# ugadiarov-la-phystech-edu/OCRL

Measured on AMD Instinct MI355X. Metric: images/sec (node) SLATE pretrain 128x128, 6 slots, 3 iters, higher is better.
Workload: dtype f32

## Files before the change

include/ocrl_hip.h:

```cpp
#ifndef OCRL_HIP_H
#define OCRL_HIP_H
#include <stddef.h>

#ifdef __cplusplus
extern "C" {
#endif

#define OCRL_ABI_VERSION 5

const char* ocrl_last_error(void);
int ocrl_abi_version(void);

typedef struct ocrl_slate ocrl_slate;
typedef struct ocrl_slate_config {
    int obs_size, obs_channels;
    int vocab_size, d_model;
    int cnn_hidden;
    int num_slots, num_iterations, slot_size, mlp_hidden;
    int num_dec_blocks, num_dec_heads;
    float dropout;
    int max_batch;
    int use_bcdec;
    int hard;
    int num_slot_heads;
// ... 2 lines not shown
size_t ocrl_slate_config_size(void);
int ocrl_slate_create(const ocrl_slate_config* cfg, ocrl_slate** out);
void ocrl_slate_destroy(ocrl_slate* h);

int ocrl_slate_param_count(const ocrl_slate* h);
int ocrl_slate_param_info(const ocrl_slate* h, int i, char* name, int name_cap, int shape[4], int* ndim,
                          long long* offset, long long* numel, int* group);
long long ocrl_slate_flat_size(const ocrl_slate* h);
long long ocrl_slate_group_begin(const ocrl_slate* h, int group);
size_t ocrl_slate_workspace_bytes(const ocrl_slate* h);

int ocrl_slate_bind(ocrl_slate* h, float* params, float* grads, float* adam_m, float* adam_v, void* workspace, size_t workspace_bytes);

int ocrl_slate_forward(ocrl_slate* h, const float* obs, int B, float tau, int train, unsigned long long seed,
                       const float* noise_z, const float* noise_zh, const float* noise_slots, void* stream);
int ocrl_slate_backward(ocrl_slate* h, void* stream);
int ocrl_slate_encode(ocrl_slate* h, const float* obs, int B, unsigned long long seed, const float* noise_slots, void* stream);
int ocrl_slate_encode_backward(ocrl_slate* h, const float* dslots, void* stream);
int ocrl_slate_freeze_weights(ocrl_slate* h, int on);
int ocrl_slate_generate(ocrl_slate* h, void* stream);
int ocrl_slate_clip_adam(ocrl_slate* h, const float lr[3], float clip, int step, float grad_scale, void* stream);
int ocrl_slate_grad_norm(ocrl_slate* h, void* stream);
float* ocrl_slate_metrics(const ocrl_slate* h);
int ocrl_slate_tensor(const ocrl_slate* h, const char* name, float** ptr, long long* count);
int ocrl_slate_soft_z(ocrl_slate* h, void* stream);
int ocrl_slate_dropout_mask(const ocrl_slate* h, unsigned site, long long n, float* out, void* stream);

int ocrl_gemm(const float* A, const float* B, float* C, int M, int N, int K, int lda, int ldb, int ldc, int akc, int bkc,
              float alpha, const float* bias, int relu, const float* mask, int ldmask, const float* resid, int ldr,
              int splitk, float* ws, void* stream);
typedef struct ocrl_gemm_desc {
    const float* A; const float* B; float* C;
    int M, N, K, lda, ldb, ldc;
    int akc, bkc;
    int batch, batch_inner;
    long long sA, sB, sC, sAi, sBi, sCi;
    int splitk; float alpha;
    const float* bias; int relu;
    float drop_p; unsigned long long drop_seed; unsigned drop_site;
    const float* mask; int ldmask; long long sMask; int mask_elu;
    const float* resid; int ldr; long long sR;
    float adrop_p; unsigned adrop_site; int adrop_ld;
    float* bias_out; long long sBias;
    int a_mode, b_mode; const float* x_lse; const int* x_tok; float x_scale;
    int epi_mode; float* stat; float* hstat; int* hidx; const float* e1; const float* e2; unsigned long long e_seed;
    const float* e_lse; const float* e_rowvec; float e_scale;
    int force_tile, force_sb;
} ocrl_gemm_desc;
size_t ocrl_gemm_desc_size(void);
int ocrl_gemm_ex(const ocrl_gemm_desc* d, float* ws, size_t ws_floats, void* stream);
int ocrl_gemm_plan(const ocrl_gemm_desc* d, int out[6]);
int ocrl_conv2d_fwd(const float* x, const float* w, const float* bias, float* y, int B, int H, int W, int cin, int cin_pad, int ks,
                    int relu, float* ws, void* stream);
int ocrl_conv2d_fwd_lowlat(const float* x, const float* w, const float* bias, float* y, int B, int H, int W, int cin, int cin_pad, int ks,
                           int relu, float* ws, void* stream);
size_t ocrl_conv2d_x3_ws_floats(void);
int ocrl_conv2d_fwd_x3(const float* x, const float* w, const float* bias, float* y, int B, int H, int W, int ks, int relu, float* ws, void* stream);
int ocrl_conv2d_bwd_data_x3(const float* dy, const float* w, const float* mask, float* dx, int B, int H, int W, int ks, float* ws, void* stream);
int ocrl_conv2d_bwd_weight_x3(const float* x, const float* dy, float* dw, int B, int H, int W, int ks, float* ws, size_t ws_floats, void* stream);
int ocrl_conv2d_bwd_data(const float* dy, const float* w, const float* mask, float* dx, int B, int H, int W, int ks, float* ws, void* stream);
size_t ocrl_conv2d_wgrad_ws_floats(int B, int H, int W, int ks, int cin_pad);
int ocrl_conv2d_bwd_weight(const float* x, const float* dy, float* dw, float* db, int B, int H, int W, int cin, int cin_pad, int ks,
                           float* ws, size_t ws_floats, void* stream);
typedef struct ocrl_conv_desc {
    const float* x; const float* w; float* y;
    int B, H, W, cin, cin_pad, ks;
    const float* bias; int relu;
    const float* posmap; const float* mask; int mask_elu;
    int transposed, low_latency;
} ocrl_conv_desc;
size_t ocrl_conv_desc_size(void);
int ocrl_conv2d_ex(const ocrl_conv_desc* d, float* ws, size_t ws_floats, void* stream);
typedef struct ocrl_conv_wgrad_desc {
    const float* x; const float* dy; float* dw; float* db;
    int B, H, W, cin, cin_pad, ks;
    int accumulate;
} ocrl_conv_wgrad_desc;
size_t ocrl_conv_wgrad_desc_size(void);
int ocrl_conv2d_bwd_weight_ex(const ocrl_conv_wgrad_desc* d, float* ws, size_t ws_floats, void* stream);
int ocrl_layernorm_fwd(const float* x, const float* gamma, const float* beta, float* y, float* mean, float* rstd, long long R, int F, void* stream);
int ocrl_layernorm_bwd(const float* dy, const float* x, const float* mean, const float* rstd, const float* gamma, float* dx, float* dgb,
                       long long R, int F, float* ws, size_t ws_floats, void* stream);

int ocrl_attention_fwd(const float* q, const float* k, const float* v, float* o, float* lse, int B, int T, int d, int h, int ld,
                       float p, unsigned long long seed, unsigned site, void* stream);
int ocrl_attention_bwd(const float* q, const float* k, const float* v, const float* o, const float* lse, const float* dO,
                       float* dq, float* dk, float* dv, float* delta, int B, int T, int d, int h, int ld,
                       float p, unsigned long long seed, unsigned site, void* stream);

int ocrl_obs_u8_to_f32(const unsigned char* obs_hwc, float* obs_chw, int B, int H, int W, int C, void* stream);

int ocrl_prof_enable(unsigned tag_mask);
int ocrl_prof_collect(double* ms, long long* count, int ntags);

size_t ocrl_slot_attention_ws_floats(int B, int K, int D, int H, int I);
int ocrl_slot_attention_fwd(const float* x, const float* slots0, const float* const* w, float* slots, float* attn, int B, int N, int K, int D,
                            int H, int I, float* ws, size_t ws_floats, void* stream);
int ocrl_slot_attention_bwd(const float* x, const float* dslots, float* dx, float* dslots0, float* const* dw, int B, int N, int K, int D, int H,
                            int I, float* ws, size_t ws_floats, void* stream);
size_t ocrl_slot_attention_mh_ws_floats(int B, int N, int K, int D, int H, int I, int heads);
int ocrl_slot_attention_mh_fwd(const float* x, const float* slots0, const float* const* w, float* slots, float* attn, int B, int N, int K, int D,
                               int H, int I, int heads, float* ws, size_t ws_floats, void* stream);
int ocrl_slot_attention_mh_bwd(const float* x, const float* dslots, float* dx, float* dslots0, float* const* dw, int B, int N, int K, int D, int H,
                               int I, int heads, float* ws, size_t ws_floats, void* stream);

#define OCRL_POOL_MAX_LAYERS 8
size_t ocrl_pool_transformer_ws_floats(int B, int K, int d, int nhead, int ff, int L);
int ocrl_pool_transformer_fwd(const float* slots, const float* const* w, const float* pos, float* out, int B, int K, int Din, int d, int nhead,
                              int ff, int L, float drop_p, unsigned long long seed, float* ws, size_t ws_floats, void* stream);
int ocrl_pool_transformer_bwd(const float* slots, const float* dout, const float* const* w, float* dslots, float* const* dw, int B, int K, int Din,
                              int d, int nhead, int ff, int L, float drop_p, unsigned long long seed, float* ws, size_t ws_floats, void* stream);
int ocrl_pool_transformer_dropout_mask(int layer, int which, long long n, float drop_p, unsigned long long seed, float* out, void* stream);
size_t ocrl_pool_transformer_long_ws_floats(int B, int K, int Din, int d, int nhead, int ff, int L);
int ocrl_pool_transformer_long_fwd(const float* slots, const float* const* w, const float* pos, float* out, int B, int K, int Din, int d, int nhead,
                                   int ff, int L, float drop_p, unsigned long long seed, float* ws, size_t ws_floats, void* stream);
int ocrl_pool_transformer_long_bwd(const float* slots, const float* dout, const float* const* w, float* dslots, float* const* dw, int B, int K,
                                   int Din, int d, int nhead, int ff, int L, float drop_p, unsigned long long seed, float* ws, size_t ws_floats,
                                   void* stream);

#define OCRL_POOL_RN_MAX_LAYERS 16
size_t ocrl_pool_rn_ws_floats(int B, int K, int D, int ng, const int* g_dims, int nf, const int* f_dims);
int ocrl_pool_rn_fwd(const float* slots, const float* const* w, float* out, int B, int K, int D, int ng, const int* g_dims, int nf, const int* f_dims,
                     float* ws, size_t ws_floats, void* stream);
int ocrl_pool_rn_bwd(const float* slots, const float* dout, const float* const* w, float* dslots, float* const* dw, int B, int K, int D, int ng,
                     const int* g_dims, int nf, const int* f_dims, float* ws, size_t ws_floats, void* stream);

#define OCRL_NATURECNN_MAX_GROUPS 16
#define OCRL_NATURECNN_MAX_CONVS 4
size_t ocrl_naturecnn_ws_floats(int B, int H, int W, int cin, int groups, int cnn_feat_size, int use_cnn_feat, int rep_dim);
int ocrl_naturecnn_fwd(const float* obs, const float* const* w, float* out, int B, int H, int W, int cin, int groups, int cnn_feat_size,
                       int use_cnn_feat, int rep_dim, int save, float* ws, size_t ws_floats, void* stream);
int ocrl_naturecnn_bwd(const float* obs, const float* dout, const float* const* w, float* const* dw, int B, int H, int W, int cin, int groups,
                       int cnn_feat_size, int use_cnn_feat, int rep_dim, float* ws, size_t ws_floats, void* stream);

size_t ocrl_pool_cnn_ws_floats(int B, int H, int W, int D, int rep_dim);
int ocrl_pool_cnn_fwd(const float* tokens, const float* const* w, float* out, int B, int H, int W, int D, int rep_dim, int save, float* ws,
                      size_t ws_floats, void* stream);
int ocrl_pool_cnn_bwd(const float* tokens, const float* dout, const float* const* w, float* dtokens, float* const* dw, int B, int H, int W, int D,
                      int rep_dim, float* ws, size_t ws_floats, void* stream);

#define OCRL_VAE_MAX_STAGES 6
size_t ocrl_vae_ws_floats(int B, int obs_size, int obs_channels, int cnn_feat_size, int latent_dim, int use_cnn_feat, int full);
int ocrl_vae_fwd(const float* obs, const float* const* w, const float* eps, float* rep, float* metrics, float* recon, int B, int obs_size,
                 int obs_channels, int cnn_feat_size, int latent_dim, int use_cnn_feat, float kld_weight, int full, float* ws, size_t ws_floats,
                 void* stream);
int ocrl_vae_bwd(const float* obs, const float* eps, const float* const* w, const float* dloss, const float* drep, float* const* dw, int B,
                 int obs_size, int obs_channels, int cnn_feat_size, int latent_dim, int use_cnn_feat, float kld_weight, int full, float* ws,
                 size_t ws_floats, void* stream);

#define OCRL_MAE_MAX_DEPTH 32
size_t ocrl_mae_ws_floats(int B, int obs_size, int patch, int D, int depth, int heads, int Dd, int ddepth, int dheads, int len_keep, int full);
int ocrl_mae_fwd(const float* obs, const float* const* w, const float* noise, float* rep, float* metrics, float* pred, float* mask,
                 int* ids_restore, int B, int obs_size, int patch, int D, int depth, int heads, int Dd, int ddepth, int dheads, int len_keep,
                 int full, float* ws, size_t ws_floats, void* stream);
int ocrl_mae_bwd(const float* obs, const float* const* w, const float* dloss, const float* drep, float* const* dw, int B, int obs_size,
                 int patch, int D, int depth, int heads, int Dd, int ddepth, int dheads, int len_keep, int full, float* ws, size_t ws_floats,
                 void* stream);
int ocrl_mae_rank(const float* noise, int* ids_restore, int* ids_keep, float* mask, int B, int L, int len_keep, void* stream);

#define OCRL_PROBE_MAX_SLOTS 12
#define OCRL_PROBE_MAX_PROPS 8
#define OCRL_PROBE_MAX_LAYERS 8
size_t ocrl_probe_ws_floats(int B, int K, int N, int D, int O, int slot_rows, int nl, const int* dims, int P);
int ocrl_probe_fwd(const float* rows, const float* const* w, const float* y, float* out, float* cost, int* col, float* metrics, int B, int K, int N,
                   int D, int T, int O, int slot_rows, int nl, const int* dims, float slope, int P, const int* tgt_range, const int* out_range,
                   const int* kind, float* ws, size_t ws_floats, void* stream);
// ... 74 lines not shown
```

ocrl_amd/csrc/capi.cpp:

```cpp
#include <stdarg.h>
#include <stdint.h>
#include <string.h>

#include <new>

#include "../../include/ocrl_hip.h"
#include "iodine_model.h"
#include "slate_model.h"

static thread_local char g_err[512] = "";

void ocrl_set_error(const char* fmt, ...) {
    va_list ap;
    va_start(ap, fmt);
    vsnprintf(g_err, sizeof g_err, fmt, ap);
    va_end(ap);
}

template <class M>
struct Handle {
    using Model = M;
    M* m = nullptr;
};
struct ocrl_slate : Handle<SlateModel> {};
// ... 183 lines not shown
}
size_t ocrl_conv2d_x3_ws_floats(void) { return 2 * conv_x3_pack_floats(5); }
int ocrl_conv2d_fwd_x3(const float* x, const float* w, const float* bias, float* y, int B, int H, int W, int ks, int relu, float* ws, void* stream) {
    if (ks != 3 && ks != 5) { ocrl_set_error("ocrl_conv2d_fwd_x3: ks must be 3 or 5"); return 1; }
    if (conv_pack_x3_launch(w, ws, nullptr, ST(stream), ks)) return 1;
    ConvArgs a;
    a.X = x; a.Y = y; a.B = B; a.H = H; a.W = W; a.bias = bias; a.relu = relu;
    return conv_x3_launch(a, ws, ST(stream), ks);
}
int ocrl_conv2d_bwd_data_x3(const float* dy, const float* w, const float* mask, float* dx, int B, int H, int W, int ks, float* ws, void* stream) {
    if (ks != 3 && ks != 5) { ocrl_set_error("ocrl_conv2d_bwd_data_x3: ks must be 3 or 5"); return 1; }
    if (conv_pack_x3_launch(w, ws, ws + conv_x3_pack_floats(5), ST(stream), ks)) return 1;
    ConvArgs a;
    a.X = dy; a.Y = dx; a.B = B; a.H = H; a.W = W; a.mask = mask;
    return conv_x3_launch(a, ws + conv_x3_pack_floats(5), ST(stream), ks);
}
int ocrl_conv2d_bwd_data(const float* dy, const float* w, const float* mask, float* dx, int B, int H, int W, int ks, float* ws, void* stream) {
    float* bw = ws + (size_t)ks * ks * 64 * 64;
    if (conv_pack_launch(w, ws, bw, ks, 64, 64, 64, ST(stream))) return 1;
    ConvArgs a;
    a.X = dy; a.Wp = bw; a.Y = dx; a.B = B; a.H = H; a.W = W; a.mask = mask;
    return conv_fwd_launch(a, ks, 64, 64, ST(stream));
}
size_t ocrl_conv2d_wgrad_ws_floats(int B, int H, int W, int ks, int cin_pad) { return conv_wgrad_ws_floats(B, H, W, ks, cin_pad) + (1 << 16); }
int ocrl_conv2d_bwd_weight(const float* x, const float* dy, float* dw, float* db, int B, int H, int W, int cin, int cin_pad, int ks, float* ws,
                           size_t ws_floats, void* stream) {
    if (ws_floats < ocrl_conv2d_wgrad_ws_floats(B, H, W, ks, cin_pad)) { ocrl_set_error("ocrl_conv2d_bwd_weight: workspace too small"); return 1; }
    WgradArgs a;
    a.X = x; a.dY = dy; a.part = ws; a.B = B; a.H = H; a.W = W;
    if (conv_wgrad_launch(a, ks, cin_pad, 64, cin, dw, 0, ST(stream), 0)) return 1;
    if (db) return colsum_launch(dy, 64, db, (long long)B * H * W, 64, 0, 1.f, ws, ws_floats, ST(stream));
    return 0;
}
int ocrl_conv2d_bwd_weight_x3(const float* x, const float* dy, float* dw, int B, int H, int W, int ks, float* ws, size_t ws_floats, void* stream) {
    if (ks != 3 && ks != 5) { ocrl_set_error("ocrl_conv2d_bwd_weight_x3: ks must be 3 or 5"); return 1; }
    if (ws_floats < ocrl_conv2d_wgrad_ws_floats(B, H, W, ks, 64)) { ocrl_set_error("ocrl_conv2d_bwd_weight_x3: workspace too small"); return 1; }
    WgradArgs a;
    a.X = x; a.dY = dy; a.part = ws; a.B = B; a.H = H; a.W = W;
    return conv_wgrad_launch(a, ks, 64, 64, 64, dw, 0, ST(stream), 1);
}
static bool conv_kernel_built(int ks, int cin_pad) { return (ks == 5 && (cin_pad == 64 || cin_pad == 8)) || (ks == 3 && cin_pad == 64); }
static bool aligned16(const void* p) { return ((uintptr_t)p & 15) == 0; }
size_t ocrl_conv_desc_size(void) { return sizeof(ocrl_conv_desc); }
int ocrl_conv2d_ex(const ocrl_conv_desc* d, float* ws, size_t ws_floats, void* stream) {
    if (!d) { ocrl_set_error("ocrl_conv2d_ex: null descriptor"); return 1; }
    if (!d->x || !d->w || !d->y || !ws || d->B < 1 || d->H < 1 || d->W < 1) { ocrl_set_error("ocrl_conv2d_ex: x, w, y, ws and a non-empty image are required"); return 1; }
    if (!conv_kernel_built(d->ks, d->cin_pad)) { ocrl_set_error("ocrl_conv2d_ex: no kernel for ks=%d cin_pad=%d (built: 5/64, 5/8, 3/64)", d->ks, d->cin_pad); return 1; }
    if (d->cin < 1 || d->cin > d->cin_pad) { ocrl_set_error("ocrl_conv2d_ex: cin %d outside 1 .. cin_pad %d", d->cin, d->cin_pad); return 1; }
    if (d->relu < 0 || d->relu > 2) { ocrl_set_error("ocrl_conv2d_ex: relu must be 0, 1 (ReLU) or 2 (ELU), got %d", d->relu); return 1; }
    if (d->mask_elu && !d->mask) { ocrl_set_error("ocrl_conv2d_ex: mask_elu needs a mask"); return 1; }
    if (d->transposed && (d->cin != 64 || d->cin_pad != 64)) { ocrl_set_error("ocrl_conv2d_ex: the transposed (backward-data) form needs cin = cin_pad = 64"); return 1; }
    if (!aligned16(d->x) || !aligned16(d->y) || !aligned16(ws) || !aligned16(d->bias) || !aligned16(d->posmap) || !aligned16(d->mask)) {
        ocrl_set_error("ocrl_conv2d_ex: x, y, ws, bias, posmap and mask must be 16-byte aligned");
        return 1;
    }
    const size_t pack = (size_t)d->ks * d->ks * d->cin_pad * 64, need = d->transposed ? 2 * pack : pack;
    if (ws_floats < need) { ocrl_set_error("ocrl_conv2d_ex: workspace of %zu floats, %zu needed", ws_floats, need); return 1; }
    float* bw = d->transposed ? ws + pack : nullptr;
    if (conv_pack_launch(d->w, ws, bw, d->ks, d->cin_pad, 64, d->cin, ST(stream))) return 1;
    ConvArgs a;
    a.X = d->x; a.Wp = bw ? bw : ws; a.Y = d->y; a.B = d->B; a.H = d->H; a.W = d->W; a.bias = d->bias; a.relu = d->relu;
    a.posmap = d->posmap; a.mask = d->mask; a.mask_elu = d->mask_elu ? 1 : 0;
    return conv_fwd_launch(a, d->ks, d->cin_pad, 64, ST(stream), d->low_latency ? 1 : 0);
}
size_t ocrl_conv_wgrad_desc_size(void) { return sizeof(ocrl_conv_wgrad_desc); }
int ocrl_conv2d_bwd_weight_ex(const ocrl_conv_wgrad_desc* d, float* ws, size_t ws_floats, void* stream) {
    if (!d) { ocrl_set_error("ocrl_conv2d_bwd_weight_ex: null descriptor"); return 1; }
    if (!d->x || !d->dy || !d->dw || !ws || d->B < 1 || d->H < 1 || d->W < 1) { ocrl_set_error("ocrl_conv2d_bwd_weight_ex: x, dy, dw, ws and a non-empty image are required"); return 1; }
    if (!conv_kernel_built(d->ks, d->cin_pad)) { ocrl_set_error("ocrl_conv2d_bwd_weight_ex: no kernel for ks=%d cin_pad=%d (built: 5/64, 5/8, 3/64)", d->ks, d->cin_pad); return 1; }
    if (d->cin < 1 || d->cin > d->cin_pad) { ocrl_set_error("ocrl_conv2d_bwd_weight_ex: cin %d outside 1 .. cin_pad %d", d->cin, d->cin_pad); return 1; }
    if (!aligned16(d->x) || !aligned16(d->dy) || !aligned16(ws)) { ocrl_set_error("ocrl_conv2d_bwd_weight_ex: x, dy and ws must be 16-byte aligned"); return 1; }
    const size_t need = ocrl_conv2d_wgrad_ws_floats(d->B, d->H, d->W, d->ks, d->cin_pad);
    if (ws_floats < need) { ocrl_set_error("ocrl_conv2d_bwd_weight_ex: workspace of %zu floats, %zu needed", ws_floats, need); return 1; }
    const int acc = d->accumulate ? 1 : 0;
    WgradArgs a;
    a.X = d->x; a.dY = d->dy; a.part = ws; a.B = d->B; a.H = d->H; a.W = d->W;
    if (conv_wgrad_launch(a, d->ks, d->cin_pad, 64, d->cin, d->dw, acc, ST(stream), 0)) return 1;
    if (d->db) return colsum_launch(d->dy, 64, d->db, (long long)d->B * d->H * d->W, 64, acc, 1.f, ws, ws_floats, ST(stream));
    return 0;
}
int ocrl_layernorm_fwd(const float* x, const float* g, const float* b, float* y, float* mean, float* rstd, long long R, int F, void* stream) {
    return layernorm_fwd_launch(x, g, b, y, mean, rstd, R, F, ST(stream));
}
int ocrl_layernorm_bwd(const float* dy, const float* x, const float* mean, const float* rstd, const float* g, float* dx, float* dgb, long long R,
                       int F, float* ws, size_t ws_floats, void* stream) {
    return layernorm_bwd_launch(dy, x, mean, rstd, g, dx, dgb, R, F, 0, 0, ws, ws_floats, ST(stream));
}

int ocrl_attention_fwd(const float* q, const float* k, const float* v, float* o, float* lse, int B, int T, int d, int h, int ld, float p,
                       unsigned long long seed, unsigned site, void* stream) {
    AttnArgs a;
    a.q = q; a.k = k; a.v = v; a.o = o; a.lse = lse; a.B = B; a.T = T; a.d = d; a.h = h; a.ld = ld; a.p = p; a.seed = seed; a.site = site;
    return attn_launch(a, 0, ST(stream));
}
int ocrl_attention_bwd(const float* q, const float* k, const float* v, const float* o, const float* lse, const float* dO, float* dq,
                       float* dk, float* dv, float* delta, int B, int T, int d, int h, int ld, float p, unsigned long long seed,
                       unsigned site, void* stream) {
    AttnArgs a;
    a.q = q; a.k = k; a.v = v; a.o = const_cast<float*>(o); a.lse = const_cast<float*>(lse); a.B = B; a.T = T; a.d = d; a.h = h; a.ld = ld;
    a.p = p; a.seed = seed; a.site = site; a.dO = dO; a.dq = dq; a.dk = dk; a.dv = dv; a.delta = delta;
    return attn_launch(a, 1, ST(stream));
}


int ocrl_iodine_create(const ocrl_iodine_config* c, ocrl_iodine** out) {
    if (!c || !out) { ocrl_set_error("ocrl_iodine_create: null argument"); return 1; }
    if (c->obs_size < 16 || c->obs_size % 16 || c->obs_channels != 3 || c->slot_size < 4 || c->slot_size % 4 || c->slot_size > 256 ||
        c->num_iterations < 1 || c->num_slots < 1 || c->num_slots > 16 || c->ref_mlp_hidden < 64 || c->ref_mlp_hidden % 64 || c->max_batch < 1 ||
        !(c->sigma > 0.f)) {
        ocrl_set_error("ocrl_iodine_create: invalid configuration");
        return 1;
    }
    IodineConfig k;
    k.obs_size = c->obs_size; k.obs_channels = c->obs_channels; k.slot_size = c->slot_size; k.num_iters = c->num_iterations;
    k.num_slots = c->num_slots; k.sigma = c->sigma; k.beta = c->beta; k.layer_norm = c->layer_norm; k.ref_mlp_hidden = c->ref_mlp_hidden;
    k.max_batch = c->max_batch;
    return h_create(k, out);
}
void ocrl_iodine_destroy(ocrl_iodine* h) { h_destroy(h); }
int ocrl_iodine_param_count(const ocrl_iodine* h) { return h_param_count(h); }
int ocrl_iodine_param_info(const ocrl_iodine* h, int i, char* name, int name_cap, int shape[4], int* ndim, long long* offset, long long* numel) {
    return h_param_info(h, i, name, name_cap, shape, ndim, offset, numel, nullptr);
}
long long ocrl_iodine_flat_size(const ocrl_iodine* h) { return h_flat_size(h); }
size_t ocrl_iodine_workspace_bytes(const ocrl_iodine* h) { return h_workspace_bytes(h); }
int ocrl_iodine_bind(ocrl_iodine* h, float* p, float* g, float* m, float* v, void* ws, size_t n) { return h_bind(h, p, g, m, v, ws, n); }
int ocrl_iodine_forward(ocrl_iodine* h, const float* obs, int B, unsigned long long seed, const float* noise, void* stream) {
    GUARD(h);
    return h->m->forward(obs, B, seed, noise, ST(stream));
}
int ocrl_iodine_backward(ocrl_iodine* h, void* stream) { GUARD(h); return h->m->backward(ST(stream)); }
int ocrl_iodine_clip_adam(ocrl_iodine* h, float lr, float clip, int step, float gscale, void* stream) {
    GUARD(h);
    return h->m->clip_adam(lr, clip, step, gscale, ST(stream));
}
int ocrl_iodine_grad_norm(ocrl_iodine* h, void* stream) { GUARD(h); return h->m->grad_norm(ST(stream)); }
float* ocrl_iodine_metrics(const ocrl_iodine* h) { return h_metrics(h); }
int ocrl_iodine_tensor(const ocrl_iodine* h, const char* name, float** ptr, long long* count) { return h_tensor(h, name, ptr, count); }
}
```

ocrl_amd/csrc/elementwise.hip:

```cpp
#include "common.h"
#include "kernels.h"

#define TINYF 1.17549435e-38f

__device__ inline float block_sum(float v, float* red) {
    v = wave_sum(v);
    const int w = threadIdx.x >> 6, nw = blockDim.x >> 6;
    __syncthreads();
    if ((threadIdx.x & 63) == 0) red[w] = v;
    __syncthreads();
    float s = 0.f;
    for (int i = 0; i < nw; ++i) s += red[i];
    return s;
}
__device__ inline float block_max(float v, float* red) {
    v = wave_max(v);
    const int w = threadIdx.x >> 6, nw = blockDim.x >> 6;
    __syncthreads();
    if ((threadIdx.x & 63) == 0) red[w] = v;
    __syncthreads();
    float s = red[0];
    for (int i = 1; i < nw; ++i) s = fmaxf(s, red[i]);
    return s;
}

__global__ void nchw_to_nhwc8_kernel(const float* __restrict__ in, float* __restrict__ out, int B, int C, int H, int W) {
    const long long n = (long long)B * H * W;
    const long long i = (long long)blockIdx.x * blockDim.x + threadIdx.x;
    if (i >= n) return;
    const long long hw = (long long)H * W;
    const long long b = i / hw, r = i % hw;
    float v[8];
#pragma unroll
    for (int c = 0; c < 8; ++c) v[c] = c < C ? in[(b * C + c) * hw + r] : 0.f;
    float4* o = reinterpret_cast<float4*>(out + i * 8);
    o[0] = make_float4(v[0], v[1], v[2], v[3]);
    o[1] = make_float4(v[4], v[5], v[6], v[7]);
}

__global__ void patchify4_kernel(const float* __restrict__ in, float* __restrict__ out, int B, int C, int S) {
    const int E = S / 4;
    const long long n = (long long)B * E * E * C * 4;
    const long long i = (long long)blockIdx.x * blockDim.x + threadIdx.x;
    if (i >= n) return;
    const int ky = i & 3;
    const int c = (i >> 2) % C;
    const long long row = (i >> 2) / C;
    const int ex = row % E, ey = (row / E) % E;
    const long long b = row / ((long long)E * E);
    const float4 v = *reinterpret_cast<const float4*>(in + ((b * C + c) * S + (ey * 4 + ky)) * S + ex * 4);
    *reinterpret_cast<float4*>(out + row * (C * 16) + c * 16 + ky * 4) = v;
}

__global__ void pixel_shuffle_kernel(const float* __restrict__ in, float* __restrict__ out, int B, int h, int w, int Cout, int forward,
                                     const float* __restrict__ mask) {
    const long long n = (long long)B * h * w * Cout;
    const long long i = (long long)blockIdx.x * blockDim.x + threadIdx.x;
    if (i >= n) return;
    const int c = i % Cout;
    long long r = i / Cout;
    const int x = r % w; r /= w;
    const int y = r % h;
    const long long b = r / h;
    const long long u = i * 4;
    const long long s00 = ((b * 2 * h + 2 * y) * (2 * w) + 2 * x) * Cout + c;
    const long long s01 = s00 + Cout, s10 = s00 + (long long)2 * w * Cout, s11 = s10 + Cout;
    if (forward) {
        const float4 v = *reinterpret_cast<const float4*>(in + u);
        out[s00] = v.x; out[s01] = v.y; out[s10] = v.z; out[s11] = v.w;
    } else {
        float4 v = make_float4(in[s00], in[s01], in[s10], in[s11]);
        if (mask) {
            const float4 m = *reinterpret_cast<const float4*>(mask + u);
            v.x = m.x > 0.f ? v.x : 0.f; v.y = m.y > 0.f ? v.y : 0.f; v.z = m.z > 0.f ? v.z : 0.f; v.w = m.w > 0.f ? v.w : 0.f;
        }
        *reinterpret_cast<float4*>(out + u) = v;
    }
}

template <int NPL>
__global__ void layernorm_fwd_kernel(const float* __restrict__ x, const float* __restrict__ g, const float* __restrict__ bta,
                                     float* __restrict__ y, float* __restrict__ mean, float* __restrict__ rstd, long long R) {
    constexpr int F = 64 * NPL;
    const int lane = threadIdx.x & 63;
// ... 166 lines not shown
        const float mu = group16_sum(s) * (1.0f / 192);
        float q = 0.f;
#pragma unroll
        for (int k = 0; k < 3; ++k) {
            v[i][k].x -= mu; v[i][k].y -= mu; v[i][k].z -= mu; v[i][k].w -= mu;
            q += (v[i][k].x * v[i][k].x + v[i][k].y * v[i][k].y) + (v[i][k].z * v[i][k].z + v[i][k].w * v[i][k].w);
        }
        const float rs = rsqrtf(group16_sum(q) * (1.0f / 192) + 1e-5f);
        if (row < R) {
#pragma unroll
            for (int k = 0; k < 3; ++k)
                *reinterpret_cast<float4*>(y + row * 192 + (k * 16 + c4) * 4) = make_float4(v[i][k].x * rs * gg[k].x + bb[k].x, v[i][k].y * rs * gg[k].y + bb[k].y,
                                                                                            v[i][k].z * rs * gg[k].z + bb[k].z, v[i][k].w * rs * gg[k].w + bb[k].w);
            if (c4 == 0) { if (mean) mean[row] = mu; if (rstd) rstd[row] = rs; }
        }
    }
}
__global__ __launch_bounds__(256) void layernorm_bwd192_kernel(const float* __restrict__ dy, const float* __restrict__ x, const float* __restrict__ mean,
                                                               const float* __restrict__ rstd, const float* __restrict__ g, float* __restrict__ dx,
                                                               float* __restrict__ part, long long R, int accumulate) {
    __shared__ float4 red[2][16][48];
    const int lane = threadIdx.x & 63, wv = threadIdx.x >> 6, c4 = lane & 15, rsub = lane >> 4;
    float4 gg[3], dg[3], db[3];
#pragma unroll
    for (int k = 0; k < 3; ++k) { gg[k] = *reinterpret_cast<const float4*>(g + (k * 16 + c4) * 4); dg[k] = make_float4(0.f, 0.f, 0.f, 0.f); db[k] = dg[k]; }
    for (long long grp = blockIdx.x; grp * 32 < R; grp += gridDim.x) {
        const long long row0 = (grp * 4 + wv) * 8 + rsub;
        float4 xv[2][3], yv[2][3];
        float mu[2], rs[2];
#pragma unroll
        for (int i = 0; i < 2; ++i) {
            const long long row = row0 + 4 * i;
            const bool ok = row < R;
#pragma unroll
            for (int k = 0; k < 3; ++k) {
                xv[i][k] = ok ? *reinterpret_cast<const float4*>(x + row * 192 + (k * 16 + c4) * 4) : make_float4(0.f, 0.f, 0.f, 0.f);
                yv[i][k] = ok ? *reinterpret_cast<const float4*>(dy + row * 192 + (k * 16 + c4) * 4) : make_float4(0.f, 0.f, 0.f, 0.f);
            }
            mu[i] = ok ? mean[row] : 0.f;
            rs[i] = ok ? rstd[row] : 0.f;
        }
#pragma unroll
        for (int i = 0; i < 2; ++i) {
            const long long row = row0 + 4 * i;
            float4 xh[3], d4[3];
            float s1 = 0.f, s2 = 0.f;
#pragma unroll
            for (int k = 0; k < 3; ++k) {
                xh[k] = make_float4((xv[i][k].x - mu[i]) * rs[i], (xv[i][k].y - mu[i]) * rs[i], (xv[i][k].z - mu[i]) * rs[i], (xv[i][k].w - mu[i]) * rs[i]);
                const float4 yy = yv[i][k];
                dg[k].x += yy.x * xh[k].x; dg[k].y += yy.y * xh[k].y; dg[k].z += yy.z * xh[k].z; dg[k].w += yy.w * xh[k].w;
                db[k].x += yy.x; db[k].y += yy.y; db[k].z += yy.z; db[k].w += yy.w;
                d4[k] = make_float4(yy.x * gg[k].x, yy.y * gg[k].y, yy.z * gg[k].z, yy.w * gg[k].w);
                s1 += (d4[k].x + d4[k].y) + (d4[k].z + d4[k].w);
                s2 += (d4[k].x * xh[k].x + d4[k].y * xh[k].y) + (d4[k].z * xh[k].z + d4[k].w * xh[k].w);
            }
            s1 = group16_sum(s1) * (1.0f / 192);
            s2 = group16_sum(s2) * (1.0f / 192);
            if (row < R) {
#pragma unroll
                for (int k = 0; k < 3; ++k) {
                    float4 o = make_float4(rs[i] * (d4[k].x - s1 - xh[k].x * s2), rs[i] * (d4[k].y - s1 - xh[k].y * s2), rs[i] * (d4[k].z - s1 - xh[k].z * s2),
                                           rs[i] * (d4[k].w - s1 - xh[k].w * s2));
                    float* dp = dx + row * 192 + (k * 16 + c4) * 4;
                    if (accumulate) { const float4 a = *reinterpret_cast<const float4*>(dp); o.x += a.x; o.y += a.y; o.z += a.z; o.w += a.w; }
                    *reinterpret_cast<float4*>(dp) = o;
                }
            }
        }
    }
#pragma unroll
    for (int k = 0; k < 3; ++k) { red[0][wv * 4 + rsub][k * 16 + c4] = dg[k]; red[1][wv * 4 + rsub][k * 16 + c4] = db[k]; }
    __syncthreads();
    if (threadIdx.x < 96) {
        const int which = threadIdx.x / 48, c = threadIdx.x % 48;
        float4 a = red[which][0][c];
#pragma unroll
        for (int k = 1; k < 16; ++k) { const float4 t = red[which][k][c]; a.x += t.x; a.y += t.y; a.z += t.z; a.w += t.w; }
        *reinterpret_cast<float4*>(part + (size_t)blockIdx.x * 384 + which * 192 + c * 4) = a;
    }
}

__global__ void colsum_kernel(const float* __restrict__ X, long long ld, float* __restrict__ part, long long R, int F, long long rows_per_chunk) {
    __shared__ float red[4][64];
    const int col = blockIdx.x * 64 + (threadIdx.x & 63), rl = threadIdx.x >> 6;
    const long long r0 = (long long)blockIdx.y * rows_per_chunk;
    const long long r1 = min(R, r0 + rows_per_chunk);
    float s = 0.f;
    if (col < F)
        for (long long r = r0 + rl; r < r1; r += 4) s += X[r * ld + col];
    red[rl][threadIdx.x & 63] = s;
    __syncthreads();
    if (rl == 0 && col < F) part[(size_t)blockIdx.y * F + col] = red[0][threadIdx.x] + red[1][threadIdx.x] + red[2][threadIdx.x] + red[3][threadIdx.x];
}
__global__ __launch_bounds__(256) void colsum4_kernel(const float* __restrict__ X, long long ld, float* __restrict__ part, long long R, int F,
                                                      long long rows_per_chunk) {
    __shared__ float4 red[256];
    const int F4 = F >> 2, RL = 256 / F4;
    const int c4 = threadIdx.x % F4, rl = threadIdx.x / F4;
    const long long r0 = (long long)blockIdx.x * rows_per_chunk;
    const long long r1 = min(R, r0 + rows_per_chunk);
    float4 s0 = make_float4(0.f, 0.f, 0.f, 0.f), s1 = s0, s2 = s0, s3 = s0;
    if (rl < RL) {
        const float* base = X + (size_t)c4 * 4;
        long long r = r0 + rl;
        for (; r + 3 * RL < r1; r += 4 * RL) {
            const float4 a = *reinterpret_cast<const float4*>(base + r * ld), b = *reinterpret_cast<const float4*>(base + (r + RL) * ld);
            const float4 c = *reinterpret_cast<const float4*>(base + (r + 2 * RL) * ld), d = *reinterpret_cast<const float4*>(base + (r + 3 * RL) * ld);
            s0.x += a.x; s0.y += a.y; s0.z += a.z; s0.w += a.w;
            s1.x += b.x; s1.y += b.y; s1.z += b.z; s1.w += b.w;
            s2.x += c.x; s2.y += c.y; s2.z += c.z; s2.w += c.w;
            s3.x += d.x; s3.y += d.y; s3.z += d.z; s3.w += d.w;
        }
        for (; r < r1; r += RL) {
            const float4 a = *reinterpret_cast<const float4*>(base + r * ld);
            s0.x += a.x; s0.y += a.y; s0.z += a.z; s0.w += a.w;
        }
    }
    red[threadIdx.x] = make_float4(s0.x + s1.x + s2.x + s3.x, s0.y + s1.y + s2.y + s3.y, s0.z + s1.z + s2.z + s3.z, s0.w + s1.w + s2.w + s3.w);
    __syncthreads();
    if (threadIdx.x < F4) {
        float4 t = red[threadIdx.x];
        for (int k = 1; k < RL; ++k) { const float4 v = red[k * F4 + threadIdx.x]; t.x += v.x; t.y += v.y; t.z += v.z; t.w += v.w; }
        *reinterpret_cast<float4*>(part + (size_t)blockIdx.x * F + threadIdx.x * 4) = t;
    }
}
__global__ __launch_bounds__(256) void colsum_final_kernel(const float* __restrict__ part, float* __restrict__ out, int nchunk, int F, int accumulate, float scale) {
    __shared__ float red[16][16];
    const int cl = threadIdx.x & 15, rl = threadIdx.x >> 4;
    const int c = blockIdx.x * 16 + cl;
    float s0 = 0.f, s1 = 0.f;
    if (c < F) {
        int k = rl;
        for (; k + 16 < nchunk; k += 32) { s0 += part[(size_t)k * F + c]; s1 += part[(size_t)(k + 16) * F + c]; }
        if (k < nchunk) s0 += part[(size_t)k * F + c];
    }
    red[rl][cl] = s0 + s1;
    __syncthreads();
    if (rl == 0 && c < F) {
        float t = 0.f;
#pragma unroll
        for (int k = 0; k < 16; ++k) t += red[k][cl];
        t *= scale;
        out[c] = accumulate ? out[c] + t : t;
    }
}

__global__ void reduce_partials_kernel(const float* __restrict__ part, int n, float* __restrict__ out, float scale, int accumulate) {
    __shared__ float red[4];
    float s = 0.f;
    for (int i = threadIdx.x; i < n; i += blockDim.x) s += part[i];
    s = block_sum(s, red);
    if (threadIdx.x == 0) out[0] = (accumulate ? out[0] : 0.f) + s * scale;
}

__global__ void mse_kernel(const float* __restrict__ obs, const float* __restrict__ recon, float* __restrict__ drecon,
                           float* __restrict__ part, int B, int C, int H, int W, float inv_b) {
    __shared__ float red[4];
    const long long n = (long long)B * H * W, hw = (long long)H * W;
    float s = 0.f;
    for (long long i = (long long)blockIdx.x * blockDim.x + threadIdx.x; i < n; i += (long long)gridDim.x * blockDim.x) {
        const long long b = i / hw, r = i % hw;
        const float4 rc = *reinterpret_cast<const float4*>(recon + i * 4);
        const float rv[4] = {rc.x, rc.y, rc.z, rc.w};
        float d[4] = {0.f, 0.f, 0.f, 0.f};
        for (int c = 0; c < C; ++c) {
            const float e = rv[c] - obs[(b * C + c) * hw + r];
            s += e * e;
            d[c] = 2.f * e * inv_b;
        }
        if (drecon) *reinterpret_cast<float4*>(drecon + i * 4) = make_float4(d[0], d[1], d[2], d[3]);
    }
    s = block_sum(s, red);
    if (threadIdx.x == 0) part[blockIdx.x] = s;
}

#define GS_MAXPT 16
template <int NPT>
__global__ __launch_bounds__(256) void gumbel_softmax_kernel(const float* __restrict__ raw, const float* __restrict__ e1,
                                                             const float* __restrict__ e2, float* __restrict__ z,
                                                             int* __restrict__ tokens, int V, float inv_tau,
                                                             unsigned long long seed, float* __restrict__ zst) {
    __shared__ float red[4];
    __shared__ float redv[4];
    __shared__ int redi[4];
    const long long row = blockIdx.x;
    const float* r = raw + row * V;
    const int npt = NPT ? NPT : V / 256;
    float x[GS_MAXPT];
    float mx = -INFINITY;
#pragma unroll
    for (int i = 0; i < GS_MAXPT; ++i)
        if (i < npt) { x[i] = r[i * 256 + threadIdx.x]; mx = fmaxf(mx, x[i]); }
    mx = block_max(mx, red);
    float s = 0.f;
#pragma unroll
    for (int i = 0; i < GS_MAXPT; ++i)
        if (i < npt) s += __expf(x[i] - mx);
    s = block_sum(s, red);
    const float lse = mx + __logf(s);
    float u[GS_MAXPT];
    float best = -INFINITY;
    int besti = 0;
    float m2 = -INFINITY;
#pragma unroll
    for (int i = 0; i < GS_MAXPT; ++i)
        if (i < npt) {
            const int v = i * 256 + threadIdx.x;
            const float lp = x[i] - lse;
            float ea, eb;
            if (e1) { ea = e1[row * V + v]; eb = e2[row * V + v]; }
            else {
                const uint64_t idx = (uint64_t)row * V + v;
                const uint2 ba = rng_bits4(seed, SITE_GUMBEL_Z, idx);
                ea = -__logf(u01_24(ba.x));
                eb = -__logf(u01_24(ba.y));
            }
            const float g1 = -__logf(ea + TINYF), g2 = -__logf(eb + TINYF);
            u[i] = (lp + g1) * inv_tau;
            m2 = fmaxf(m2, u[i]);
            const float h = (lp + g2) * inv_tau;
            if (h > best) { best = h; besti = v; }
        }
    m2 = block_max(m2, red);
    float s2 = 0.f;
#pragma unroll
    for (int i = 0; i < GS_MAXPT; ++i)
        if (i < npt) { u[i] = __expf(u[i] - m2); s2 += u[i]; }
// ... 805 lines not shown
    float mx = -INFINITY;
    for (int j = tid; j < nk; j += 256) {
        const float* kr = base + (size_t)j * ld + d;
        float a = 0.f;
        for (int c = 0; c < dh; c += 4) {
            const float4 kv = *reinterpret_cast<const float4*>(kr + c);
            a += qs[c] * kv.x + qs[c + 1] * kv.y + qs[c + 2] * kv.z + qs[c + 3] * kv.w;
        }
        sc[j] = a;
        mx = fmaxf(mx, a);
    }
    red[tid] = mx;
    __syncthreads();
    for (int o = 128; o > 0; o >>= 1) { if (tid < o) red[tid] = fmaxf(red[tid], red[tid + o]); __syncthreads(); }
    mx = red[0];
    __syncthreads();
    float sum = 0.f;
    for (int j = tid; j < nk; j += 256) { const float e = __expf(sc[j] - mx); sc[j] = e; sum += e; }
    red[tid] = sum;
    __syncthreads();
    for (int o = 128; o > 0; o >>= 1) { if (tid < o) red[tid] += red[tid + o]; __syncthreads(); }
    const float inv = 1.0f / red[0];
    __syncthreads();
    const int nsl = 256 / dh, c = tid % dh, sl = tid / dh;
    float acc = 0.f;
    if (sl < nsl)
        for (int j = sl; j < nk; j += nsl) acc += sc[j] * base[(size_t)j * ld + 2 * d + c];
    red[tid] = sl < nsl ? acc : 0.f;
    __syncthreads();
    if (tid < dh) {
        float a = 0.f;
        for (int k = 0; k < nsl; ++k) a += red[k * dh + tid];
        out[(size_t)b * d + hd * dh + tid] = a * inv;
    }
}

__global__ void onehot_kernel(const int* __restrict__ tokens, float* __restrict__ z, long long n, int V) {
    const long long i = (long long)blockIdx.x * blockDim.x + threadIdx.x;
    if (i >= n) return;
    z[i] = (int)(i % V) == tokens[i / V] ? 1.f : 0.f;
}

#define GRID1D(n) dim3(cdiv((n), 256)), dim3(256)

int nchw_to_nhwc8_launch(const float* in, float* out, int B, int C, int H, int W, hipStream_t st) {
    OCRL_REQUIRE(C <= 8, "nchw_to_nhwc8: C must be <= 8");
    const long long n = (long long)B * H * W;
    hipLaunchKernelGGL(nchw_to_nhwc8_kernel, GRID1D(n), 0, st, in, out, B, C, H, W);
    OCRL_CHECK_LAUNCH("nchw_to_nhwc8");
    return 0;
}
int patchify4_launch(const float* in, float* out, int B, int C, int S, hipStream_t st) {
    OCRL_REQUIRE(S % 4 == 0, "patchify4: S %% 4 != 0");
    const long long n = (long long)B * (S / 4) * (S / 4) * C * 4;
    hipLaunchKernelGGL(patchify4_kernel, GRID1D(n), 0, st, in, out, B, C, S);
    OCRL_CHECK_LAUNCH("patchify4");
    return 0;
}
int pixel_shuffle_launch(const float* in, float* out, int B, int h, int w, int Cout, int forward, const float* mask, hipStream_t st) {
    const long long n = (long long)B * h * w * Cout;
    hipLaunchKernelGGL(pixel_shuffle_kernel, GRID1D(n), 0, st, in, out, B, h, w, Cout, forward, mask);
    OCRL_CHECK_LAUNCH("pixel_shuffle");
    return 0;
}
int layernorm_fwd_launch(const float* x, const float* g, const float* b, float* y, float* mean, float* rstd, long long R, int F, hipStream_t st) {
    OCRL_REQUIRE(F % 64 == 0 && F >= 64 && F <= 256, "layernorm: F must be 64..256, multiple of 64 (got %d)", F);
    dim3 grid(cdiv(R, 4)), blk(256);
    const bool al16 = (((uintptr_t)x | (uintptr_t)y | (uintptr_t)g | (uintptr_t)b) & 15) == 0;
    switch (F / 64) {
        case 1:
            if (al16) hipLaunchKernelGGL(layernorm_fwd64_kernel, dim3((unsigned)cdiv(R, 64)), blk, 0, st, x, g, b, y, mean, rstd, R);
            else hipLaunchKernelGGL(layernorm_fwd_kernel<1>, grid, blk, 0, st, x, g, b, y, mean, rstd, R);
            break;
        case 2: hipLaunchKernelGGL(layernorm_fwd_kernel<2>, grid, blk, 0, st, x, g, b, y, mean, rstd, R); break;
        case 3:
            if (al16) hipLaunchKernelGGL(layernorm_fwd192_kernel, dim3((unsigned)cdiv(R, 32)), blk, 0, st, x, g, b, y, mean, rstd, R);
            else hipLaunchKernelGGL(layernorm_fwd_kernel<3>, grid, blk, 0, st, x, g, b, y, mean, rstd, R);
            break;
        default: hipLaunchKernelGGL(layernorm_fwd_kernel<4>, grid, blk, 0, st, x, g, b, y, mean, rstd, R); break;
    }
    OCRL_CHECK_LAUNCH("layernorm_fwd");
    return 0;
}
int colsum_launch(const float* X, long long ld, float* out, long long R, int F, int accumulate, float scale, float* ws, size_t ws_floats, hipStream_t st) {
    if (F % 4 == 0 && ld % 4 == 0 && F <= 1024 && F >= 4 && (((uintptr_t)X) & 15) == 0 && R >= 1024) {
        long long nchunk = 2048;
        if (nchunk > R / 8) nchunk = R / 8;
        if ((size_t)nchunk * F > ws_floats) nchunk = (long long)(ws_floats / F);
        if (nchunk >= 16) {
            const long long rpc = (R + nchunk - 1) / nchunk;
            nchunk = (R + rpc - 1) / rpc;
            hipLaunchKernelGGL(colsum4_kernel, dim3((unsigned)nchunk), dim3(256), 0, st, X, ld, ws, R, F, rpc);
            OCRL_CHECK_LAUNCH("colsum4");
            hipLaunchKernelGGL(colsum_final_kernel, dim3(cdiv(F, 16)), dim3(256), 0, st, ws, out, (int)nchunk, F, accumulate, scale);
            OCRL_CHECK_LAUNCH("colsum_final");
            return 0;
        }
    }
    const int cb = cdiv(F, 64);
    long long nchunk = 1024 / cb;
    if (nchunk < 1) nchunk = 1;
    if (nchunk > (R + 63) / 64) nchunk = (R + 63) / 64;
    if (nchunk < 1) nchunk = 1;
    OCRL_REQUIRE((size_t)nchunk * F <= ws_floats, "colsum: workspace too small (%lld x %d)", nchunk, F);
    const long long rpc = (R + nchunk - 1) / nchunk;
    hipLaunchKernelGGL(colsum_kernel, dim3(cb, (int)nchunk), dim3(256), 0, st, X, ld, ws, R, F, rpc);
    OCRL_CHECK_LAUNCH("colsum");
    hipLaunchKernelGGL(colsum_final_kernel, dim3(cdiv(F, 16)), dim3(256), 0, st, ws, out, (int)nchunk, F, accumulate, scale);
    OCRL_CHECK_LAUNCH("colsum_final");
    return 0;
}
int layernorm_bwd_launch(const float* dy, const float* x, const float* mean, const float* rstd, const float* g, float* dx,
                         float* dgb, long long R, int F, int accumulate_dx, int accumulate_dgb, float* ws, size_t ws_floats, hipStream_t st) {
    OCRL_REQUIRE(F % 64 == 0 && F >= 64 && F <= 256, "layernorm bwd: F must be 64..256, multiple of 64 (got %d)", F);
    int nblk = (int)((R + 3) / 4);
    if (nblk > 2048) nblk = 2048;
    while (nblk > 64 && (size_t)nblk * 2 * F * 2 + (size_t)8 * 2 * F > ws_floats) nblk /= 2;
    const size_t need = (size_t)nblk * 2 * F;
    OCRL_REQUIRE(need + (size_t)8 * 2 * F <= ws_floats, "layernorm bwd: workspace too small");
    dim3 grid(nblk), blk(256);
    switch (F / 64) {
        case 1:
            if (((((uintptr_t)x | (uintptr_t)dy | (uintptr_t)dx | (uintptr_t)g) & 15) == 0) && (((uintptr_t)ws) & 15) == 0)
                hipLaunchKernelGGL(layernorm_bwd64_kernel, grid, blk, 0, st, dy, x, mean, rstd, g, dx, ws, R, accumulate_dx);
            else hipLaunchKernelGGL(layernorm_bwd_kernel<1>, grid, blk, 0, st, dy, x, mean, rstd, g, dx, ws, R, accumulate_dx);
            break;
        case 2: hipLaunchKernelGGL(layernorm_bwd_kernel<2>, grid, blk, 0, st, dy, x, mean, rstd, g, dx, ws, R, accumulate_dx); break;
        case 3:
            if (((((uintptr_t)x | (uintptr_t)dy | (uintptr_t)dx | (uintptr_t)g) & 15) == 0) && (((uintptr_t)ws) & 15) == 0)
                hipLaunchKernelGGL(layernorm_bwd192_kernel, grid, blk, 0, st, dy, x, mean, rstd, g, dx, ws, R, accumulate_dx);
            else hipLaunchKernelGGL(layernorm_bwd_kernel<3>, grid, blk, 0, st, dy, x, mean, rstd, g, dx, ws, R, accumulate_dx);
            break;
        default: hipLaunchKernelGGL(layernorm_bwd_kernel<4>, grid, blk, 0, st, dy, x, mean, rstd, g, dx, ws, R, accumulate_dx); break;
    }
    OCRL_CHECK_LAUNCH("layernorm_bwd");
    return colsum_launch(ws, 2 * F, dgb, nblk, 2 * F, accumulate_dgb, 1.f, ws + need, ws_floats - need, st);
}
int reduce_partials_launch(const float* part, int n, float* out, float scale, int accumulate, hipStream_t st) {
    hipLaunchKernelGGL(reduce_partials_kernel, dim3(1), dim3(256), 0, st, part, n, out, scale, accumulate);
    OCRL_CHECK_LAUNCH("reduce_partials");
    return 0;
}
int mse_launch(const float* obs, const float* recon, float* drecon, float* out, int B, int C, int H, int W, float* ws, size_t ws_floats, hipStream_t st) {
    OCRL_REQUIRE(C <= 4, "mse: C must be <= 4");
    const int nblk = 1024;
    OCRL_REQUIRE(ws_floats >= (size_t)nblk, "mse: workspace too small");
    hipLaunchKernelGGL(mse_kernel, dim3(nblk), dim3(256), 0, st, obs, recon, drecon, ws, B, C, H, W, 1.0f / B);
    OCRL_CHECK_LAUNCH("mse");
    return reduce_partials_launch(ws, nblk, out, 1.0f / B, 0, st);
}
int gumbel_softmax_launch(const float* raw, const float* e1, const float* e2, float* z, int* tokens, long long R, int V, float tau,
                          unsigned long long seed, hipStream_t st, float* zst) {
    OCRL_REQUIRE(V % 256 == 0 && V <= 256 * GS_MAXPT, "gumbel_softmax: V must be a multiple of 256, <= %d", 256 * GS_MAXPT);
    OCRL_REQUIRE((e1 == nullptr) == (e2 == nullptr), "gumbel_softmax: give both noise tensors or none");
    switch (V / 256) {
        case 16: hipLaunchKernelGGL(gumbel_softmax_kernel<16>, dim3((unsigned)R), dim3(256), 0, st, raw, e1, e2, z, tokens, V, 1.0f / tau, seed, zst); break;
        case 8: hipLaunchKernelGGL(gumbel_softmax_kernel<8>, dim3((unsigned)R), dim3(256), 0, st, raw, e1, e2, z, tokens, V, 1.0f / tau, seed, zst); break;
        default: hipLaunchKernelGGL(gumbel_softmax_kernel<0>, dim3((unsigned)R), dim3(256), 0, st, raw, e1, e2, z, tokens, V, 1.0f / tau, seed, zst); break;
    }
    OCRL_CHECK_LAUNCH("gumbel_softmax");
    return 0;
}
int softmax_bwd_rows_launch(const float* z, float* d, long long R, int V, float scale, hipStream_t st) {
    OCRL_REQUIRE(V % 256 == 0 && V <= 256 * GS_MAXPT, "softmax_bwd_rows: V must be a multiple of 256, <= %d", 256 * GS_MAXPT);
    if (V == 4096) hipLaunchKernelGGL(softmax_bwd_rows_kernel<16>, dim3((unsigned)R), dim3(256), 0, st, z, d, V, scale);
    else hipLaunchKernelGGL(softmax_bwd_rows_kernel<0>, dim3((unsigned)R), dim3(256), 0, st, z, d, V, scale);
    OCRL_CHECK_LAUNCH("softmax_bwd_rows");
    return 0;
}
int ce_launch(float* pred, const int* tokens, float* out, long long R, int V, int B, int write_grad, float* ws, size_t ws_floats, hipStream_t st) {
    OCRL_REQUIRE(ws_floats >= (size_t)R, "ce: workspace too small");
    OCRL_REQUIRE(V % 256 == 0 && V <= 256 * GS_MAXPT, "ce: V must be a multiple of 256, <= %d", 256 * GS_MAXPT);
    if (V == 4096) hipLaunchKernelGGL(ce_kernel<16>, dim3((unsigned)R), dim3(256), 0, st, pred, tokens, ws, V, 1.0f / B, write_grad);
    else hipLaunchKernelGGL(ce_kernel<0>, dim3((unsigned)R), dim3(256), 0, st, pred, tokens, ws, V, 1.0f / B, write_grad);
    OCRL_CHECK_LAUNCH("ce");
    return reduce_partials_launch(ws, (int)R, out, 1.0f / B, 0, st);
}
int softmax_stat_combine_launch(const float* stat, int nseg, long long R, float* lse, const float* hstat, const int* hidx, int* tokens,
                                const float* pred, int ldp, const int* tok, float* out, float scale, float* ws, size_t ws_floats, hipStream_t st,
                                const float* cdf_scores, int cdf_V, float cdf_tau, unsigned long long cdf_seed) {
    OCRL_REQUIRE(nseg >= 1 && nseg <= 64, "softmax_stat_combine: 1..64 segments (got %d)", nseg);
    const long long nblk = (R + 15) / 16;
    OCRL_REQUIRE(!pred || (tok && out && ws && ws_floats >= (size_t)nblk), "softmax_stat_combine: cross-entropy needs tokens, an output and %lld workspace floats", nblk);
    CdfArgs cdf;
    cdf.scores = cdf_scores; cdf.V = cdf_V; cdf.tau = cdf_tau; cdf.seed = cdf_seed;
    OCRL_REQUIRE(!cdf_scores || (hstat && hidx && tokens && cdf_V > 0 && cdf_V <= nseg * 64), "softmax_stat_combine: inverse-CDF sampling arguments");
    hipLaunchKernelGGL(softmax_stat_combine_kernel, dim3((unsigned)nblk), dim3(1024), 0, st, stat, nseg, R, lse, hstat, hidx, tokens, pred, ldp, tok,
                       pred ? ws : nullptr, cdf);
    OCRL_CHECK_LAUNCH("softmax_stat_combine");
    if (pred) return reduce_partials_launch(ws, (int)nblk, out, scale, 0, st);
    return 0;
}
int exp_rows_launch(const float* y, const float* lse, float* z, long long R, int V, hipStream_t st) {
    OCRL_REQUIRE(V % 4 == 0, "exp_rows: V %% 4 != 0");
    const long long n4 = R * (V / 4);
    hipLaunchKernelGGL(exp_rows_kernel, dim3((unsigned)((n4 + 255) / 256)), dim3(256), 0, st, y, lse, z, n4, V / 4);
    OCRL_CHECK_LAUNCH("exp_rows");
    return 0;
}
int rowdot_bias64_launch(const float* g, const float* act, const float* bias, long long R, float* out, hipStream_t st) {
    OCRL_REQUIRE(((((uintptr_t)g) | ((uintptr_t)act) | ((uintptr_t)bias)) & 15) == 0, "rowdot: operands must be 16-byte aligned");
    hipLaunchKernelGGL(rowdot_bias64_kernel, dim3((unsigned)((R + 15) / 16)), dim3(256), 0, st, g, act, bias, R, out);
    OCRL_CHECK_LAUNCH("rowdot_bias64");
    return 0;
}
int embed_fwd_launch(const int* tokens, const float* dict, const float* bos, const float* pe, float* out, int B, int T, int d, float p,
                     unsigned long long seed, hipStream_t st) {
    OCRL_REQUIRE(d % 4 == 0, "embed: d %% 4 != 0");
    const long long n = (long long)B * T * (d / 4);
    hipLaunchKernelGGL(embed_fwd_kernel, dim3((unsigned)cdiv(n, 1024)), dim3(256), 0, st, tokens, dict, bos, pe, out, B, T, d, p, seed);
    OCRL_CHECK_LAUNCH("embed_fwd");
    return 0;
}
static size_t eb_align(size_t n) { return (n + 63) & ~(size_t)63; }
size_t embed_bwd_ws_floats(long long BT, int V, int d) {
    const size_t nchunk = (size_t)cdiv(BT, EB_CHUNK), nunit = (size_t)cdiv(BT, EB_UNIT);
    return eb_align(nchunk * (V + 1)) + 2 * eb_align((size_t)V + 2) + eb_align((size_t)BT) + eb_align(nunit * 2 * d);
}
// ... 188 lines not shown
```

ocrl_amd/csrc/gemm.hip:

```cpp
#include "common.h"
#include "kernels.h"
#include <stdlib.h>

int gemm_launch_tt(const GemmArgs& a, const GemmPlan& p, hipStream_t st);
int gemm_launch_tn(const GemmArgs& a, const GemmPlan& p, hipStream_t st);
int gemm_launch_nn(const GemmArgs& a, const GemmPlan& p, hipStream_t st);

__global__ __launch_bounds__(256) void splitk_reduce_kernel(const float* __restrict__ part, float* __restrict__ out, long long n4,
                                                            int splits, long long stride, int accumulate) {
    __shared__ float4 red[16][16];
    const int cl = threadIdx.x & 15, sl = threadIdx.x >> 4;
    const long long i = (long long)blockIdx.x * 16 + cl;
    float4 s = make_float4(0.f, 0.f, 0.f, 0.f);
    if (i < n4) {
        int k = sl;
        for (; k + 48 < splits; k += 64) {
            const float4 v0 = *reinterpret_cast<const float4*>(part + (size_t)k * stride + i * 4);
            const float4 v1 = *reinterpret_cast<const float4*>(part + (size_t)(k + 16) * stride + i * 4);
            const float4 v2 = *reinterpret_cast<const float4*>(part + (size_t)(k + 32) * stride + i * 4);
            const float4 v3 = *reinterpret_cast<const float4*>(part + (size_t)(k + 48) * stride + i * 4);
            s.x += (v0.x + v1.x) + (v2.x + v3.x); s.y += (v0.y + v1.y) + (v2.y + v3.y);
            s.z += (v0.z + v1.z) + (v2.z + v3.z); s.w += (v0.w + v1.w) + (v2.w + v3.w);
        }
        for (; k < splits; k += 16) {
            const float4 v = *reinterpret_cast<const float4*>(part + (size_t)k * stride + i * 4);
            s.x += v.x; s.y += v.y; s.z += v.z; s.w += v.w;
        }
    }
    red[sl][cl] = s;
    __syncthreads();
    if (sl == 0 && i < n4) {
        float4 t = accumulate ? *reinterpret_cast<const float4*>(out + i * 4) : make_float4(0.f, 0.f, 0.f, 0.f);
#pragma unroll
        for (int k = 0; k < 16; ++k) { t.x += red[k][cl].x; t.y += red[k][cl].y; t.z += red[k][cl].z; t.w += red[k][cl].w; }
        *reinterpret_cast<float4*>(out + i * 4) = t;
    }
}

static int env_tile() {
    static int v = -1;
    if (v < 0) {
        const char* e = getenv("OCRL_GEMM_TILE");
        v = 0;
        if (e) { int bm = 0, bn = 0; if (sscanf(e, "%dx%d", &bm, &bn) == 2) v = bm * 1000 + bn; }
    }
    return v;
}
static int env_sb() {
    static int v = -1;
    if (v < 0) { const char* e = getenv("OCRL_GEMM_SB"); v = e ? atoi(e) : 0; }
    return v;
}
static bool tile_built(int tile, int akc, int bkc) {
    return tile == 128128 || tile == 128064 || tile == 64128 || tile == 64064 || (tile == 128192 && (akc || !bkc));
}

int gemm_plan(const GemmArgs& a, GemmPlan* plan) {
    OCRL_REQUIRE(a.M > 0 && a.N > 0 && a.K > 0, "gemm: empty problem %d %d %d", a.M, a.N, a.K);
    OCRL_REQUIRE(a.batch >= 1 && a.splitk >= 1, "gemm: bad batch/splitk");
    if (a.akc) OCRL_REQUIRE(a.K % 4 == 0 && a.lda % 4 == 0, "gemm: A k-contiguous needs K,lda %% 4 == 0 (K=%d lda=%d)", a.K, a.lda);
    else OCRL_REQUIRE(a.M % 4 == 0 && a.lda % 4 == 0, "gemm: A m-contiguous needs M,lda %% 4 == 0 (M=%d lda=%d)", a.M, a.lda);
    if (a.bkc) OCRL_REQUIRE(a.K % 4 == 0 && a.ldb % 4 == 0, "gemm: B k-contiguous needs K,ldb %% 4 == 0 (K=%d ldb=%d)", a.K, a.ldb);
    else OCRL_REQUIRE(a.N % 4 == 0 && a.ldb % 4 == 0, "gemm: B n-contiguous needs N,ldb %% 4 == 0 (N=%d ldb=%d)", a.N, a.ldb);
    OCRL_REQUIRE(((uintptr_t)a.A & 15) == 0 && ((uintptr_t)a.B & 15) == 0, "gemm: operands must be 16-byte aligned");
    OCRL_REQUIRE((a.sA % 4) == 0 && (a.sB % 4) == 0 && (a.sAi % 4) == 0 && (a.sBi % 4) == 0, "gemm: batch strides must be multiples of 4");
    OCRL_REQUIRE(a.batch_inner >= 1 && a.batch % a.batch_inner == 0, "gemm: batch must be a multiple of batch_inner");
    OCRL_REQUIRE(a.splitk == 1 || a.batch == 1, "gemm: split-k with batches is not supported");
    if (a.splitk > 1) OCRL_REQUIRE(a.sCsplit >= (long long)(a.M - 1) * a.ldc + a.N, "gemm: split-k slab stride too small");
    if (a.adrop_p > 0.f) OCRL_REQUIRE(a.adrop_ld > 0 && a.adrop_ld % 4 == 0 && a.batch == 1, "gemm: A-dropout needs adrop_ld %% 4 == 0 and no batching");
    if (a.bias_out) OCRL_REQUIRE(!a.akc && (a.splitk == 1 || a.sBias >= a.M), "gemm: fused bias gradient needs the dW form");
    OCRL_REQUIRE(!(a.a_mode || a.b_mode) || (a.batch == 1 && a.adrop_p == 0.f && a.x_lse && (a.a_mode != 3 || a.x_tok) &&
                 (a.a_mode == 0 || a.a_mode == 2 || a.a_mode == 3) && (a.b_mode == 0 || a.b_mode == 2)), "gemm: bad operand transform arguments");
    OCRL_REQUIRE(a.force_sb >= -1 && a.force_sb <= 1, "gemm: force_sb must be -1, 0 or 1 (got %d)", a.force_sb);
    GemmPlan p;
    p.layout = 2 * (a.akc ? 1 : 0) + (a.bkc ? 1 : 0);
    if (a.epi_mode) {
        OCRL_REQUIRE(a.akc && a.batch == 1 && a.splitk == 1 && !a.a_mode && !a.b_mode && a.adrop_p == 0.f && a.relu == 0 && a.drop_p == 0.f && !a.resid,
                     "gemm: soft-max epilogue needs a plain k-contiguous A, no split-k / batches / activation");
        OCRL_REQUIRE((a.N & 3) == 0 && (a.ldc & 3) == 0 && (((uintptr_t)a.C) & 15) == 0 && (!a.bias || (((uintptr_t)a.bias) & 15) == 0),
                     "gemm: soft-max epilogue needs N, ldc multiples of 4 and 16-byte aligned C / bias");
        if (a.epi_mode == 1 || a.epi_mode == 2) {
            OCRL_REQUIRE(a.bkc && a.stat && !a.mask && gemm_stat_segments(a.N) <= 64, "gemm: soft-max statistics need a k-contiguous B, a stat buffer and N <= 4096");
            if (a.epi_mode == 2) {
                OCRL_REQUIRE(a.hstat && a.hidx && (a.e1 == nullptr) == (a.e2 == nullptr) && a.ldc == a.N, "gemm: Gumbel head arguments");
                OCRL_REQUIRE(!a.e1 || ((((uintptr_t)a.e1) | ((uintptr_t)a.e2)) & 15) == 0, "gemm: Gumbel noise must be 16-byte aligned");
            }
        } else {
            OCRL_REQUIRE(a.epi_mode == 3 && !a.bkc && a.mask && a.e_lse && a.e_rowvec && !a.bias && (a.ldmask & 3) == 0 && (((uintptr_t)a.mask) & 15) == 0,
                         "gemm: soft-max backward epilogue arguments");
        }
        OCRL_REQUIRE((a.force_tile == 0 || a.force_tile == 128128) && a.force_sb != 0,
                     "gemm: soft-max epilogue %d is built for single-buffered 128x128 tiles only", a.epi_mode);
        p.bm = 128; p.bn = 128; p.sb = 1; p.epi = a.epi_mode;
        *plan = p;
        return 0;
    }
    if (a.a_mode || a.b_mode) {
        OCRL_REQUIRE(a.akc || !a.bkc, "gemm: operand transforms are not built for akc=0 bkc=1");
        p.xf = 2;
    } else if (a.adrop_p > 0.f) {
        p.xf = 1;
    }
    int tile = 0, sb = -1;
    if (a.force_tile) {
        OCRL_REQUIRE(tile_built(a.force_tile, a.akc, a.bkc), "gemm: tile %dx%d is not built for akc=%d bkc=%d", a.force_tile / 1000,
                     a.force_tile % 1000, a.akc, a.bkc);
        tile = a.force_tile;
    } else if (env_tile() && tile_built(env_tile(), a.akc, a.bkc)) {
        tile = env_tile();
    } else if (a.akc && a.N == 192 && a.K >= 1024 && a.M >= 4096) {
        tile = 128192;
    } else if (!a.akc && !a.bkc && a.N == 192 && a.K >= 4096) {
        tile = 128192;
        sb = 1;
    } else if (a.N % 128 == 0) {
        tile = a.M > 64 ? 128128 : 64128;
    } else {
        tile = a.M > 64 ? 128064 : 64064;
    }
    if (a.force_sb >= 0) {
        sb = a.force_sb;
    } else if (sb < 0) {
        const int mode = env_sb();
        sb = (mode == 1 || (mode == 0 && a.akc)) ? 1 : 0;
    }
    p.bm = tile / 1000; p.bn = tile % 1000; p.sb = sb;
    *plan = p;
    return 0;
}

int gemm_launch(const GemmArgs& a, hipStream_t st) {
    GemmPlan p;
    if (gemm_plan(a, &p)) return 1;
    if (a.akc && a.bkc) return gemm_launch_tt(a, p, st);
    if (a.akc) return gemm_launch_tn(a, p, st);
    return gemm_launch_nn(a, p, st);
}

int splitk_reduce_launch(const float* part, float* out, long long n, int splits, long long stride,
                         int accumulate, hipStream_t st) {
    OCRL_REQUIRE(n % 4 == 0 && stride % 4 == 0, "splitk_reduce: n and stride must be multiples of 4");
    const long long n4 = n / 4;
    hipLaunchKernelGGL(splitk_reduce_kernel, dim3(cdiv(n4, 16)), dim3(256), 0, st, part, out, n4, splits, stride, accumulate);
    OCRL_CHECK_LAUNCH("splitk_reduce");
    return 0;
}

void gemm_splitk_layout(GemmArgs& a, float* ws, long long bslab) {
    const long long slab = (long long)a.M * a.N;
    a.C = ws; a.sCsplit = slab;
    if (a.bias_out) { a.bias_out = ws + a.splitk * slab; a.sBias = bslab; }
}

int gemm_splitk_launch(GemmArgs a, float* ws, long long bslab, int accumulate, hipStream_t st) {
    float* const C = a.C;
    float* const db = a.bias_out;
    gemm_splitk_layout(a, ws, bslab);
    RC(gemm_launch(a, st));
    RC(splitk_reduce_launch(ws, C, a.sCsplit, a.splitk, a.sCsplit, accumulate, st));
    if (db) RC(splitk_reduce_launch(a.bias_out, db, a.M, a.splitk, bslab, 0, st));
    return 0;
}

static void set_xf(GemmArgs& a, const Xf& xf) {
    a.a_mode = xf.a_mode; a.b_mode = xf.b_mode; a.x_lse = xf.lse; a.x_tok = xf.tok; a.x_scale = xf.scale;
}
static void set_adrop(GemmArgs& a, const Drop& dr, int ld) {
    if (dr.p > 0.f) { a.adrop_p = dr.p; a.adrop_site = dr.site; a.adrop_ld = ld; a.drop_seed = dr.seed; }
}

int lin_fwd(const float* x, int ldx, const float* W, const float* b, float* y, int ldy, long long M, int N, int K, int relu, const float* resid,
            int ldr, hipStream_t st, Drop dr) {
    GemmArgs a;
    a.A = x; a.B = W; a.C = y; a.M = (int)M; a.N = N; a.K = K; a.lda = ldx; a.ldb = K; a.ldc = ldy; a.akc = 1; a.bkc = 1;
    a.bias = b; a.relu = relu; a.resid = resid; a.ldr = ldr; a.drop_p = dr.p; a.drop_seed = dr.seed; a.drop_site = dr.site;
    return gemm_launch(a, st);
}

int lin_bwd_x(const float* dy, int ld_dy, const float* W, float* dx, int ldx, long long M, int N_out, int K_in, const float* mask, int ldmask,
              const float* resid, int ldr, hipStream_t st, Drop dr, Xf xf, float alpha) {
    GemmArgs a;
    a.A = dy; a.B = W; a.C = dx; a.M = (int)M; a.N = K_in; a.K = N_out; a.lda = ld_dy; a.ldb = K_in; a.ldc = ldx; a.akc = 1; a.bkc = 0;
    a.alpha = alpha; a.mask = mask; a.ldmask = ldmask; a.resid = resid; a.ldr = ldr;
    set_adrop(a, dr, N_out);
    set_xf(a, xf);
    return gemm_launch(a, st);
}

static int lin_splitk_count(const GemmArgs& a, size_t sk_floats, int max_splits, int* splits) {
    GemmPlan p;
    RC(gemm_plan(a, &p));
    long long s = 1024 / ((long long)cdiv(a.M, p.bm) * cdiv(a.N, p.bn));
    if (s > a.K / 256) s = a.K / 256;
    if (max_splits > 0 && s > max_splits) s = max_splits;
    const long long per = (long long)a.M * a.N + ((a.M + 3) & ~3);
    if (s * per > (long long)sk_floats) s = (long long)sk_floats / per;
    *splits = s > 1 ? (int)s : 1;
    return 0;
}

int lin_bwd_w(const float* dy, int ld_dy, const float* x, int ldx, float* dW, float* db, long long M, int N_out, int K_in, float alpha, float* sk,
              size_t sk_floats, hipStream_t st, Drop dr, Xf xf, int accumulate, int max_splits) {
    OCRL_REQUIRE(!(db && accumulate), "lin_bwd_w: a fused bias gradient is written, not accumulated");
    GemmArgs a;
    a.A = dy; a.B = x; a.C = dW; a.M = N_out; a.N = K_in; a.K = (int)M; a.lda = ld_dy; a.ldb = ldx; a.ldc = K_in; a.akc = 0; a.bkc = 0;
    a.alpha = alpha; a.bias_out = db;
    set_adrop(a, dr, N_out);
    set_xf(a, xf);
    int splits;
    RC(lin_splitk_count(a, sk_floats, max_splits, &splits));
    if (splits > 1) {
        a.splitk = splits;
        return gemm_splitk_launch(a, sk, (N_out + 3) & ~3, accumulate, st);
    }
    if (accumulate) { a.resid = dW; a.ldr = K_in; }
    return gemm_launch(a, st);
}
```

ocrl_amd/csrc/kernels.h:

```cpp
#pragma once
#include "common.h"
#include "../../include/ocrl_hip.h"

enum { PROF_CONV5 = 0, PROF_CONV_OTHER = 1, PROF_WGRAD = 2, PROF_GEMM = 3, PROF_SA_FWD = 4, PROF_SA_BWD = 5, PROF_ATTN_FWD = 6, PROF_ATTN_BWD = 7, PROF_NTAGS = 8 };
int prof_begin(int tag, hipStream_t st);
void prof_end(int idx, hipStream_t st);

struct GemmArgs {
    const float* A = nullptr;
    const float* B = nullptr;
    float* C = nullptr;
    int M = 0, N = 0, K = 0;
    int lda = 0, ldb = 0, ldc = 0;
    int akc = 1, bkc = 1;
    int batch = 1;
    int batch_inner = 1;
    long long sA = 0, sB = 0, sC = 0;
    long long sAi = 0, sBi = 0, sCi = 0;
    int splitk = 1;
    long long sCsplit = 0;
    float alpha = 1.f;
    const float* bias = nullptr;
    int relu = 0;
    float drop_p = 0.f;
    unsigned long long drop_seed = 0;
    unsigned drop_site = 0;
    const float* mask = nullptr; int ldmask = 0; long long sMask = 0;
    int mask_elu = 0;
    const float* resid = nullptr; int ldr = 0; long long sR = 0;
    float adrop_p = 0.f; unsigned adrop_site = 0; int adrop_ld = 0;
    float* bias_out = nullptr; long long sBias = 0;
    int a_mode = 0, b_mode = 0;
    const float* x_lse = nullptr; const int* x_tok = nullptr; float x_scale = 1.f;
    int epi_mode = 0;
    float* stat = nullptr; float* hstat = nullptr; int* hidx = nullptr;
    const float* e1 = nullptr; const float* e2 = nullptr; unsigned long long e_seed = 0;
    const float* e_lse = nullptr; const float* e_rowvec = nullptr; float e_scale = 1.f;
    int force_tile = 0;
    int force_sb = -1;
};
inline int gemm_stat_segments(int N) { return 2 * ((N + 127) / 128); }
struct GemmPlan { int bm = 0, bn = 0, sb = 0, xf = 0, epi = 0, layout = 0; };
int gemm_plan(const GemmArgs& a, GemmPlan* plan);
int gemm_launch(const GemmArgs& a, hipStream_t st);
int splitk_reduce_launch(const float* part, float* out, long long n, int splits, long long stride,
                         int accumulate, hipStream_t st);
void gemm_splitk_layout(GemmArgs& a, float* ws, long long bslab);
int gemm_splitk_launch(GemmArgs a, float* ws, long long bslab, int accumulate, hipStream_t st);

struct Drop { float p = 0.f; unsigned long long seed = 0; unsigned site = 0; };
struct Xf { int a_mode = 0, b_mode = 0; const float* lse = nullptr; const int* tok = nullptr; float scale = 1.f; };
int lin_fwd(const float* x, int ldx, const float* W, const float* b, float* y, int ldy, long long M, int N, int K, int relu, const float* resid,
            int ldr, hipStream_t st, Drop dr = Drop());
int lin_bwd_x(const float* dy, int ld_dy, const float* W, float* dx, int ldx, long long M, int N_out, int K_in, const float* mask, int ldmask,
              const float* resid, int ldr, hipStream_t st, Drop dr = Drop(), Xf xf = Xf(), float alpha = 1.f);
int lin_bwd_w(const float* dy, int ld_dy, const float* x, int ldx, float* dW, float* db, long long M, int N_out, int K_in, float alpha, float* sk,
              size_t sk_floats, hipStream_t st, Drop dr = Drop(), Xf xf = Xf(), int accumulate = 0, int max_splits = 0);

int pool_embed_launch(const float* lin, const float* cls, const float* pos, float* x0, int B, int K, int d, hipStream_t st);
int pool_rows_launch(const float* in, float* out, int B, int K, int d, int mode, hipStream_t st);
int pool_attn_launch(const float* qkv, float* P, float* O, const float* dO, float* dqkv, int B, int S, int d, int h, float p, unsigned long long seed,
                     unsigned site, int backward, hipStream_t st);

int pool_cols_launch(const float* src, int lds, float* dst, int ldd, long long rows, int ncols, int ncopy, hipStream_t st);
int pool_cls_drop_launch(const float* x, const float* resid, int ldr, float* out, int B, int N, int S, float p, unsigned long long seed, unsigned site,
                         hipStream_t st);
int pool_cls_add_launch(float* dX, const float* v, int B, int d, int S, hipStream_t st);
int pool_cls_nchunk(int B, int S, int* chunk);
struct PoolClsArgs {
    const float* X = nullptr;
    const float* Win = nullptr; const float* bin = nullptr;
    const float* q = nullptr;
    float* U = nullptr;
    float* part = nullptr;
    float* z = nullptr;
    float* stat = nullptr;
    float* o = nullptr;
    const float* dO = nullptr;
    float* G = nullptr; float* gD = nullptr;
    float* dX = nullptr;
    float* w = nullptr; float* dq = nullptr;
    const float* x0 = nullptr;
    float* dW = nullptr; float* db = nullptr;
    int B = 0, S = 0, d = 0, h = 0;
    float p = 0.f; unsigned long long seed = 0; unsigned site = 0;
};
int pool_cls_attn_fwd_launch(const PoolClsArgs& a, hipStream_t st);
int pool_cls_attn_bwd_launch(const PoolClsArgs& a, hipStream_t st);
int pool_flash_launch(const float* qkv, float* O, float* lse, const float* dO, float* Dd, float* dqkv, int B, int S, int d, int h, float p,
                      unsigned long long seed, unsigned site, int backward, hipStream_t st);

int rn_pair_fwd_launch(const float* AB, const float* b1, float* h1, int B, int K, int g, hipStream_t st);
int rn_pair_bwd_launch(const float* dh1, float* dAB, int B, int K, int g, hipStream_t st);
int rn_pairsum_fwd_launch(const float* gL, float* y, int B, int P, int g, hipStream_t st);
int rn_pairsum_bwd_launch(const float* dy, const float* gL, float* dgL, int B, int P, int g, hipStream_t st);

struct NcMap { long long sN = 0, sG = 0, sC = 0, sH = 0, sW = 0; };
struct NcFwdArgs {
    const float* X = nullptr; NcMap x;
    float* Y = nullptr; float* Y2 = nullptr; NcMap y;
    const float* w[OCRL_NATURECNN_MAX_GROUPS] = {}; const float* bias[OCRL_NATURECNN_MAX_GROUPS] = {};
    int B = 0, G = 1, cin = 0, cout = 0, H = 0, W = 0, OH = 0, OW = 0, ks = 0, stride = 0;
    int pad = 0;
};
struct NcBwdArgs {
    const float* X = nullptr; NcMap x;
    const float* dY = nullptr; NcMap dy;
    float* dX = nullptr;
    float* part = nullptr;
    int slabs = 1, slab_rows = 0;
    const float* w[OCRL_NATURECNN_MAX_GROUPS] = {};
    int B = 0, G = 1, cin = 0, cout = 0, H = 0, W = 0, OH = 0, OW = 0, ks = 0, stride = 0;
    int pad = 0;
    long long dw_tiles = 0, dx_tiles = 0; int dw_blocks = 0;
};
struct NcReduceLayer { const float* part = nullptr; int slabs = 0, G = 0, cout = 0, K = 0; long long n = 0; };
struct NcReduceArgs {
    NcReduceLayer L[OCRL_NATURECNN_MAX_CONVS];
    float* dw[OCRL_NATURECNN_MAX_CONVS][OCRL_NATURECNN_MAX_GROUPS] = {};
    float* db[OCRL_NATURECNN_MAX_CONVS][OCRL_NATURECNN_MAX_GROUPS] = {};
    int nlayers = 0;
};
int nc_conv_fwd_launch(const NcFwdArgs& a, hipStream_t st);
int nc_conv_bwd_launch(NcBwdArgs a, hipStream_t st);
int nc_dw_reduce_launch(const NcReduceArgs& a, hipStream_t st);
int nc_relu_mask_launch(const float* d, const float* act, float* out, long long n, hipStream_t st);

struct PcGeom {
    int OH = 0, OW = 0, OWT = 0;
    int NG = 0, nchunk = 0;
    size_t wp_floats = 0;
    long long units = 0; int slab_units = 0, slabs = 0; size_t part_floats = 0;
    int passes = 0, nbg = 0, Dp = 0; size_t wd_floats = 0;
    int HB = 0, WB = 0, WT = 0; long long dx_units = 0; int upw = 0;
};
PcGeom pc_geom(int B, int H, int W, int D);
struct PcFwdArgs {
    const float* X = nullptr; const float* Wp = nullptr; const float* bias = nullptr; float* Y = nullptr;
    int B = 0, H = 0, W = 0, D = 0, OH = 0, OW = 0, OWT = 0, nchunk = 0, NG = 0;
};
// ... 5 lines not shown
struct PcDxArgs {
    const float* dY = nullptr; const float* Wd = nullptr; float* dX = nullptr;
    int H = 0, W = 0, D = 0, OH = 0, OW = 0, HB = 0, WT = 0, Dp = 0, passes = 0, upw = 0;
    long long units = 0, groups = 0;
};
int pc_conv1_fwd_launch(const float* X, const float* w, const float* bias, float* Wp, float* Y, int B, int H, int W, int D, hipStream_t st);
int pc_conv1_dw_launch(const float* X, const float* dY, float* part, int B, int H, int W, int D, hipStream_t st);
int pc_conv1_dw_reduce_launch(const float* part, float* dw, float* db, int B, int H, int W, int D, hipStream_t st);
int pc_conv1_dx_launch(const float* dY, const float* w, float* Wd, float* dX, int B, int H, int W, int D, hipStream_t st);

#define PROBE_MAX_SLOTS 12
#define PROBE_MAX_PROPS 8
#define PROBE_MAX_WIDTH 256
struct ProbeSchema { int P; int t[PROBE_MAX_PROPS], a[PROBE_MAX_PROPS], b[PROBE_MAX_PROPS], kind[PROBE_MAX_PROPS]; };
int probe_schema_check(const ProbeSchema& sc, int T, int O);
int probe_match_check(int B, int K, int N, int T, int O);
int probe_match_launch(const float* out, int ld_row, long long ld_img, const float* y, const float* dloss, float* cost, int* col, float* part,
                       float* metrics, float* dout, int B, int K, int N, int T, int O, const ProbeSchema& sc, hipStream_t st);
int probe_leaky_fwd_launch(float* x, long long n, float slope, hipStream_t st);
int probe_leaky_bwd_launch(float* dx, const float* h, long long n, float slope, hipStream_t st);

int vae_permute_launch(const float* src, float* dst, long long R, int C, int HW, int rows, int pack, hipStream_t st);
int vae_pad_rows_launch(const float* src, float* dst, int rows, int rows_pad, int K, hipStream_t st);
int vae_kl_fwd_launch(const float* ml, const float* eps, float* latent, float* part, float* rep, int B, int L, hipStream_t st);
int vae_loss_launch(const float* part, float* metrics, int B, float kld_weight, hipStream_t st);
int vae_kl_bwd_launch(const float* ml, const float* eps, const float* dlat, const float* drep, const float* dloss, float* dml, int B, int L,
                      float kld_weight, hipStream_t st);
int vae_scale_launch(const float* x, float* y, const float* g, long long n, hipStream_t st);
int vae_recon_nchw_launch(const float* r4, float* out, int B, int C, int HW, hipStream_t st);

#define MAE_MAX_PATCHES 1024
int mae_rank_launch(const float* noise, int* restore, int* keep, float* mask, int* restore_out, float* mask_out, int B, int L, int len_keep,
                    hipStream_t st);
int mae_patch_gather_launch(const float* obs, const int* ids, float* out, int B, int n, int S, int p, hipStream_t st);
int mae_tokens_fwd_launch(const float* embed, const float* cls, const float* pos, const int* ids, float* x0, int B, int n, int D, hipStream_t st);
int mae_tokens_bwd_launch(const float* dx0, float* dembed, float* dcls, int B, int n, int D, hipStream_t st);
int mae_unshuffle_fwd_launch(const float* e, const float* mtok, const float* dpos, const int* restore, float* xd, int B, int L, int len_keep, int Dd,
                             hipStream_t st);
int mae_unshuffle_bwd_launch(const float* dxd, const int* keep, const float* mask, float* de, float* dmtok, float* part, int B, int L, int len_keep,
                             int Dd, hipStream_t st);
int mae_gelu_fwd_launch(const float* pre, float* y, long long n, hipStream_t st);
int mae_gelu_bwd_launch(const float* dy, const float* pre, float* dpre, long long n, hipStream_t st);
int mae_ln_fwd_launch(const float* x, const float* g, const float* b, float* y, float* mean, float* rstd, long long R, int F, float eps, hipStream_t st);
int mae_ln_chunks(long long R);
int mae_ln_bwd_launch(const float* dy, const float* x, const float* mean, const float* rstd, const float* g, const float* resid, float* dx, float* dg,
                      float* db, float* part, long long R, int F, hipStream_t st);
int mae_loss_launch(const float* pred, const float* obs, const float* mask, const float* dloss, float* part, float* loss, float* dpred, int B, int L,
                    int len_keep, int S, int p, hipStream_t st);

struct ConvArgs {
    const float* X = nullptr;
    const float* Wp = nullptr;
    float* Y = nullptr;
    int B = 0, H = 0, W = 0;
    const float* bias = nullptr;
    int relu = 0;
    const float* posmap = nullptr;
    const float* mask = nullptr;
    int mask_elu = 0;
};
size_t conv_x3_pack_floats(int KS = 5);
int conv_pack_x3_launch(const float* W, float* fwd3, float* bwd3, hipStream_t st, int KS = 5);
int conv_x3_launch(const ConvArgs& a, const float* pack3, hipStream_t st, int KS = 5);
struct WgradArgs;
int conv_wgrad_x3_stage(const WgradArgs& a, int nchunk, hipStream_t st, int KS = 5);
struct WgradArgs {
    const float* X = nullptr;
    const float* dY = nullptr;
    float* part = nullptr;
    int B = 0, H = 0, W = 0;
};
int conv_fwd_launch(const ConvArgs& a, int KS, int CIN, int COUT, hipStream_t st, int low_latency = 0);
int conv_wgrad_launch(const WgradArgs& a, int KS, int CIN, int COUT, int cin_real, float* dW, int accumulate, hipStream_t st, int x3 = -1);
size_t conv_wgrad_ws_floats(int B, int H, int W, int KS, int CIN);
int conv_pack_launch(const float* W, float* fwd, float* bwd, int KS, int CIN, int COUT, int cin_real, hipStream_t st);

int nchw_to_nhwc8_launch(const float* in, float* out, int B, int C, int H, int W, hipStream_t st);
int patchify4_launch(const float* in, float* out, int B, int C, int S, hipStream_t st);
int pixel_shuffle_launch(const float* in, float* out, int B, int h, int w, int Cout, int forward, const float* mask, hipStream_t st);
int layernorm_fwd_launch(const float* x, const float* g, const float* b, float* y, float* mean, float* rstd, long long R, int F, hipStream_t st);
int layernorm_bwd_launch(const float* dy, const float* x, const float* mean, const float* rstd, const float* g, float* dx,
                         float* dgb, long long R, int F, int accumulate_dx, int accumulate_dgb, float* ws, size_t ws_floats, hipStream_t st);
int colsum_launch(const float* X, long long ld, float* out, long long R, int F, int accumulate, float scale, float* ws, size_t ws_floats, hipStream_t st);
int reduce_partials_launch(const float* part, int n, float* out, float scale, int accumulate, hipStream_t st);
int mse_launch(const float* obs, const float* recon, float* drecon, float* out, int B, int C, int H, int W, float* ws, size_t ws_floats, hipStream_t st);
int gumbel_softmax_launch(const float* raw, const float* e1, const float* e2, float* z, int* tokens, long long R, int V, float tau,
                          unsigned long long seed, hipStream_t st, float* zst = nullptr);
int softmax_bwd_rows_launch(const float* z, float* d, long long R, int V, float scale, hipStream_t st);
int softmax_stat_combine_launch(const float* stat, int nseg, long long R, float* lse, const float* hstat, const int* hidx, int* tokens,
                                const float* pred, int ldp, const int* tok, float* out, float scale, float* ws, size_t ws_floats, hipStream_t st,
                                const float* cdf_scores = nullptr, int cdf_V = 0, float cdf_tau = 1.f, unsigned long long cdf_seed = 0);
int exp_rows_launch(const float* y, const float* lse, float* z, long long R, int V, hipStream_t st);
int rowdot_bias64_launch(const float* g, const float* act, const float* bias, long long R, float* out, hipStream_t st);
int ce_launch(float* pred, const int* tokens, float* out, long long R, int V, int B, int write_grad, float* ws, size_t ws_floats, hipStream_t st);
int embed_fwd_launch(const int* tokens, const float* dict, const float* bos, const float* pe, float* out, int B, int T, int d, float p,
                     unsigned long long seed, hipStream_t st);
size_t embed_bwd_ws_floats(long long BT, int V, int d);
int embed_bwd_launch(float* g, const int* tokens, float* ddict, int B, int T, int V, int d, float p, unsigned long long seed, float* ws,
                     size_t ws_floats, hipStream_t st);
int dropout_apply_launch(const float* x, float* y, long long n, float p, unsigned long long seed, unsigned site, hipStream_t st);
int dropout_mask_launch(float* y, long long n, float p, unsigned long long seed, unsigned site, hipStream_t st);
int cross_attn_fwd_launch(const float* Q, const float* Km, const float* Vm, float* O, float* P, int B, int T, int K, int d, int h, float p,
                          unsigned long long seed, unsigned site, hipStream_t st);
size_t cross_attn_bwd_ws_floats(int B, int T, int K, int d, int h);
int cross_attn_bwd_launch(const float* dO, const float* Q, const float* Km, const float* Vm, const float* P, float* dQ, float* dKm, float* dVm,
                          int B, int T, int K, int d, int h, float p, unsigned long long seed, unsigned site, float* part, size_t part_floats,
                          hipStream_t st);
int obs_u8_to_f32_launch(const unsigned char* in, float* out, int B, int H, int W, int C, hipStream_t st);
int fill_launch(float* x, long long n, float v, hipStream_t st);
int axpy_launch(const float* x, float* y, long long n, float a, hipStream_t st);
int posmap_launch(const float* Wpos, const float* bpos, float* out, int S, int C, hipStream_t st);
int posgrid_launch(float* out, int S, hipStream_t st);
int im2col5_launch(const float* x8, float* col, long long npix, int H, int W, int C, int ldc, hipStream_t st);
int unpack5_launch(const float* dWp, float* dW, int C, int ldc, hipStream_t st);
int pad_cols_launch(const float* in, int ldi, float* out, int ldo, long long R, int C, int Cout, hipStream_t st);

bool xattn_supported(int K, int d, int h);
int xattn_kp(int K, int h);
struct XaFoldHost {
    const float* mem = nullptr;
    const float* Wq[8]; const float* Wk[8]; const float* Wv[8]; const float* Wo[8];
    float* ck[8]; float* cv[8];
    float* Ab[8]; float* AbT[8]; float* Vo[8]; float* VoT[8];
    int B = 0, K = 0, d = 0, h = 0, nblk = 0;
};
int xattn_fold_fwd_launch(const XaFoldHost& f, hipStream_t st);
struct XaHost {
    const float* x = nullptr;
    const float* resid = nullptr;
    float* y = nullptr;
    float* P = nullptr;
    const float *Ab = nullptr, *AbT = nullptr, *Vo = nullptr, *VoT = nullptr;
    const float* gd = nullptr;
    float *Pd = nullptr, *dS = nullptr;
    int B = 0, T = 0, K = 0, d = 0, h = 0;
    float p = 0.f; unsigned long long seed = 0; unsigned site_p = 0, site_o = 0;
};
int xattn_launch(const XaHost& h, int backward, hipStream_t st);


struct SaWts {
    int ln_in_g, ln_in_b, ln_s_g, ln_s_b, ln_m_g, ln_m_b;
    int Wq, WqT, Wk, WkT, Wv, WvT, Wih, WihT, Whh, WhhT, bih, bhh, W0, W0T, b0, W2, W2T, b2;
    int total;
};
static inline SaWts sa_wts_layout(int C, int D, int H) {
    SaWts o; int a = 0;
    auto take = [&](int n) { int r = a; a += (n + 3) & ~3; return r; };
    o.ln_in_g = take(C); o.ln_in_b = take(C); o.ln_s_g = take(D); o.ln_s_b = take(D); o.ln_m_g = take(D); o.ln_m_b = take(D);
    o.Wq = take(D * D); o.WqT = take(D * D); o.Wk = take(D * C); o.WkT = take(C * D); o.Wv = take(D * C); o.WvT = take(C * D);
    o.Wih = take(3 * D * D); o.WihT = take(3 * D * D); o.Whh = take(3 * D * D); o.WhhT = take(3 * D * D);
    o.bih = take(3 * D); o.bhh = take(3 * D);
    o.W0 = take(H * D); o.W0T = take(H * D); o.b0 = take(H); o.W2 = take(D * H); o.W2T = take(D * H); o.b2 = take(D);
    o.total = a;
    return o;
}
struct SaSave { int sprev, sn, q, u, r, z, n, hn, sg, m, hid, qp, up, upn, csum, ld; };
static inline SaSave sa_save_layout(int C, int D, int H, int NH = 1) {
    SaSave o;
    o.sprev = 0; o.sn = D; o.q = 2 * D; o.u = 3 * D; o.r = 4 * D; o.z = 5 * D; o.n = 6 * D; o.hn = 7 * D; o.sg = 8 * D; o.m = 9 * D;
    o.hid = 10 * D; o.qp = 10 * D + H; o.up = o.qp + NH * C; o.upn = o.up + NH * C; o.csum = o.upn + NH * C; o.ld = o.csum + ((NH + 3) & ~3);
    return o;
}
struct SaGrad { int out, hid, gi, gh, u, q, qp, ld; };
static inline SaGrad sa_grad_layout(int C, int D, int H, int NH = 1) {
    SaGrad o;
// ... 105 lines not shown
```

ocrl_amd/csrc/slate_model.cpp:

```cpp
#include "slate_model.h"

#include <stdlib.h>
#include <functional>
#include <utility>

#include <math.h>
#include <stdarg.h>
#include <string.h>

static std::string fmt(const char* f, ...) {
    char buf[256];
    va_list ap;
    va_start(ap, f);
    vsnprintf(buf, sizeof buf, f, ap);
    va_end(ap);
    return buf;
}

SlateModel::SlateModel(const SlateConfig& c) : cfg(c) {
    S = c.obs_size; E = S / 4; T = E * E; N = S * S; V = c.vocab; d = c.d_model; C = c.cnn_hidden;
    K = c.num_slots; I = c.num_iters; D = c.slot_size; H = c.mlp_hidden; NB = c.num_blocks; NH = c.num_heads;
    DH = d / NH; Bmax = c.max_batch; SH = c.slot_heads > 0 ? c.slot_heads : 1;
    const int ch = c.obs_channels;
    add_param("_dvae._encoder.0.m.weight", {64, ch, 4, 4}, 0); add_param("_dvae._encoder.0.m.bias", {64}, 0);
// ... 121 lines not shown
    if (cfg.use_bcdec) {
        const size_t BKN = BK * (size_t)N;
        bc_Wc_ = carve(nullptr, 25 * 64 * 5 + 64); bc_W1r_ = carve(nullptr, (size_t)25 * 64 * D); bc_P1_ = carve(nullptr, (size_t)N * 64);
        bc_M_ = carve(nullptr, BK * 1600); bc_T_ = carve(nullptr, BK * 1600);
        bc_c1_ = carve("bc_c1", BKN * 64); bc_c2_ = carve("bc_c2", BKN * 64); bc_c3_ = carve("bc_c3", BKN * 64);
        bc_out4_ = carve(nullptr, BKN * 4); bc_dout4_ = carve(nullptr, BKN * 4);
        bc_gA_ = carve(nullptr, BKN * 64); bc_gB_ = carve(nullptr, BKN * 64);
        for (int i = 0; i < 2; ++i) {
            bc_pk_[i] = carve(nullptr, 25 * 64 * 64); bc_pkb_[i] = carve(nullptr, 25 * 64 * 64);
            if (conv_x3_ > 0) {
                float* f3 = carve(nullptr, conv_x3_pack_floats());
                float* b3 = carve(nullptr, conv_x3_pack_floats());
                if (ws_commit_) { x3_of_[bc_pk_[i]] = f3; x3_of_[bc_pkb_[i]] = b3; }
            }
        }
        bc_Wk4_ = carve(nullptr, 9 * 64 * 4); bc_Wb4_ = carve(nullptr, 9 * 64 * 4);
        bc_dW1r_ = carve(nullptr, (size_t)25 * 64 * D); bc_dWc_ = carve(nullptr, 25 * 64 * 5 + 64);
        bc_dT_ = carve(nullptr, BK * 1600); bc_dM_ = carve(nullptr, BK * 1600); bc_G1_ = carve(nullptr, (size_t)N * 64);
        recon_ = carve("recon", BN * 4);
    } else {
    patches_ = carve("patches", BT * 16 * cfg.obs_channels);
    for (int i = 0; i < 7; ++i) de_[i] = carve(fmt("dvae_enc%d", i).c_str(), BT * 64);
    zraw_ = carve("zraw", BT * V);
    z_ = carve("z", BT * V);
    zdec_ = cfg.hard ? carve("z_st", BT * V) : z_;
    tokens_ = reinterpret_cast<int*>(carve("tokens", BT));
    {
        const size_t nseg = (size_t)gemm_stat_segments(V);
        zstat_ = carve(nullptr, BT * nseg * 2); zhstat_ = carve(nullptr, BT * nseg); zhidx_ = reinterpret_cast<int*>(carve(nullptr, BT * nseg));
        zlse_ = carve("z_lse", BT); zdot_ = carve(nullptr, BT);
        cestat_ = carve(nullptr, BT * nseg * 2); celse_ = carve("ce_lse", BT); cepart_ = carve(nullptr, BT / 16 + 16);
    }
    dd0_ = carve("dvae_dec0", BT * 64); dd1_ = carve("dvae_dec1", BT * 64); dd2_ = carve("dvae_dec2", BT * 64); dd3_ = carve("dvae_dec3", BT * 64);
    dd4_ = carve("dvae_dec4", BT * 256); ps1_ = carve(nullptr, BT * 256);
    dd6_ = carve("dvae_dec6", BT * 256); dd7_ = carve("dvae_dec7", BT * 256); dd8_ = carve("dvae_dec8", BT * 256);
    dd9_ = carve("dvae_dec9", BT * 1024); ps2_ = carve(nullptr, BN * 64);
    recon_ = carve("recon", BN * 4); drecon_ = carve(nullptr, BN * 4);
    for (int i = 0; i < 2; ++i) {
        dw_fwd_[i] = carve(nullptr, 9 * 64 * 64); dw_bwd_[i] = carve(nullptr, 9 * 64 * 64);
        if (conv_x3_ > 0) {
            float* f3 = carve(nullptr, conv_x3_pack_floats(3));
            float* b3 = carve(nullptr, conv_x3_pack_floats(3));
            if (ws_commit_) { x3_of_[dw_fwd_[i]] = f3; x3_of_[dw_bwd_[i]] = b3; }
        }
    }
    w11p_ = carve(nullptr, 4 * 64);
    mem_ = carve("mem", BK * d); emb_ = carve("emb", BT * d);
    for (int b = 0; b < NB; ++b) {
        Blk& k = blk_[b];
        k.ln1 = carve(nullptr, BT * d); k.ln1_mean = carve(nullptr, BT); k.ln1_rstd = carve(nullptr, BT);
        k.q = carve(nullptr, BT * 3 * d); k.k = k.q + d; k.v = k.q + 2 * d;
        k.lse = carve(nullptr, B * NH * (size_t)T); k.ao = carve(nullptr, BT * d); k.x1 = carve(nullptr, BT * d);
        k.ln2 = carve(nullptr, BT * d); k.ln2_mean = carve(nullptr, BT); k.ln2_rstd = carve(nullptr, BT);
        k.cq = carve(nullptr, BT * d); k.ck = carve(nullptr, BK * d); k.cv = carve(nullptr, BK * d);
        k.cP = carve(nullptr, B * NH * (size_t)T * K); k.cao = carve(nullptr, BT * d); k.x2 = carve(nullptr, BT * d);
        k.ln3 = carve(nullptr, BT * d); k.ln3_mean = carve(nullptr, BT); k.ln3_rstd = carve(nullptr, BT);
        k.f1 = carve(fmt("blk%d.ffn_hidden", b).c_str(), BT * 4 * d); k.x3 = carve(nullptr, BT * d);
    }
    bg_.resize(NB);
    {
        const size_t NC = xattn_supported(K, d, NH) ? (size_t)NH * xattn_kp(K, NH) : 16;
        xa_zero_base_ = carve_pos();
        for (int b = 0; b < NB; ++b) {
            Blk& k = blk_[b];
            k.xaAb = carve(nullptr, B * NC * d); k.xaAbT = carve(nullptr, B * NC * d); k.xaVo = carve(nullptr, B * NC * d); k.xaVoT = carve(nullptr, B * NC * d);
        }
        xa_zero_floats_ = (size_t)(carve_pos() - xa_zero_base_);
        for (int b = 0; b < NB; ++b) { bg_[b].xaPd = carve(nullptr, BT * NC); bg_[b].xaDs = carve(nullptr, BT * NC); }
        xa_dAb_ = carve(nullptr, B * NC * d); xa_dVo_ = carve(nullptr, B * NC * d);
        xa_pq_ = carve(nullptr, B * (size_t)d * d); xa_po_ = carve(nullptr, B * (size_t)d * d);
    }
    attn_delta_ = carve(nullptr, B * NH * (size_t)T);
    lnf_ = carve("dec_out", BT * d); lnf_mean_ = carve(nullptr, BT); lnf_rstd_ = carve(nullptr, BT);
    pred_ = carve("pred", BT * V);
    gx_ = carve(nullptr, BT * d); gbr_ = carve(nullptr, BT * d); gt1_ = carve(nullptr, BT * d); gt2_ = carve(nullptr, BT * d);
    gt3_ = carve(nullptr, BT * d); gf1_ = carve(nullptr, BT * 4 * d); gqkv_ = carve(nullptr, BT * 3 * d);
    for (int b = 0; b < NB; ++b) {
        BlkG& q = bg_[b];
        if (b == 0) { q.gbr[0] = gbr_; q.gf1 = gf1_; q.gt2 = gt2_; q.gqkv = gqkv_; }
        else { q.gbr[0] = carve(nullptr, BT * d); q.gf1 = carve(nullptr, BT * 4 * d); q.gt2 = carve(nullptr, BT * d); q.gqkv = carve(nullptr, BT * 3 * d); }
        q.gbr[1] = carve(nullptr, BT * d); q.gbr[2] = carve(nullptr, BT * d);
    }
    scratch3_ = carve(nullptr, scratch_floats_);
    gmem_ = carve(nullptr, BK * d); gck_ = carve(nullptr, BK * d); gcv_ = carve(nullptr, BK * d);
    gdA_ = carve(nullptr, BN * 64); gdB_ = carve(nullptr, BN * 64);
    }
    {
        const int ldc0 = (25 * cfg.obs_channels + 3) & ~3;
        col0_ = carve(nullptr, BN * ldc0); dw0p_ = carve(nullptr, (size_t)64 * ldc0);
    }
    end_layout();
}

int SlateModel::bind(float* p, float* g, float* m, float* v, void* ws, size_t ws_bytes) {
    RC(check_buffers(p, g, ws, ws_bytes));
    OCRL_REQUIRE(d % 64 == 0 && d <= 256 && D % 64 == 0 && C == 64 && V % 256 == 0 && S % 4 == 0 && d % NH == 0 && DH % 4 == 0 && DH <= 64,
                 "unsupported configuration (d_model/slot_size multiples of 64 <= 256, cnn hidden 64, vocab %% 256, obs_size %% 4)");
    OCRL_REQUIRE(cfg.obs_channels == 3, "obs_channels must be 3");
    OCRL_REQUIRE(T % 4 == 0, "obs_size/4 squared must be a multiple of 4");
    adopt_buffers(p, g, m, v, ws);
    clear_encode_graphs();
    packs_valid_ = false;
    layout_workspace(true);
    if (!side_) {
        const char* e = getenv("OCRL_OVERLAP");
        overlap_mode_ = e ? atoi(e) : 5;
        if (overlap_mode_) {
            OCRL_HIP(hipStreamCreateWithFlags(&side_, hipStreamNonBlocking));
            OCRL_HIP(hipEventCreateWithFlags(&ev_fork_, hipEventDisableTiming));
            OCRL_HIP(hipEventCreateWithFlags(&ev_join_, hipEventDisableTiming));
            OCRL_HIP(hipEventCreateWithFlags(&ev_tokens_, hipEventDisableTiming));
            const char* w = getenv("OCRL_DW_SIDE");
            dw_mode_ = (overlap_mode_ >= 3 && !cfg.use_bcdec) ? (w ? atoi(w) : 2) : 0;
            if (dw_mode_) {
                for (hipEvent_t& ev : ev_dw_) OCRL_HIP(hipEventCreateWithFlags(&ev, hipEventDisableTiming));
                OCRL_HIP(hipEventCreateWithFlags(&ev_join2_, hipEventDisableTiming));
                if (dw_mode_ == 2) OCRL_HIP(hipStreamCreateWithFlags(&side2_, hipStreamNonBlocking));
            }
        }
    }
    {
        const char* e = getenv("OCRL_XATTN");
        xattn_ = !cfg.use_bcdec && xattn_supported(K, d, NH) && (e ? atoi(e) != 0 : true);
        if (!cfg.use_bcdec && xa_zero_floats_) OCRL_HIP(hipMemset(xa_zero_base_, 0, xa_zero_floats_ * sizeof(float)));
    }
    RC(posgrid_launch(gridT_, S, 0));
    RC(fill_launch(recon_, (long long)Bmax * N * 4, 0.f, 0));
    const SaWts wo = sa_wts_layout(C, D, H);
    const std::string sa = "_slotattn.slot_attention.";
    std::vector<PackEntry> ent;
    auto e = [&](const std::string& name, int rows, int cols, int off, int tr) {
        PackEntry x; x.src = P(name); x.rows = rows; x.cols = cols; x.dst_off = off; x.transpose = tr;
        ent.push_back(x);
    };
    e(sa + "norm_inputs.weight", 1, C, wo.ln_in_g, 0); e(sa + "norm_inputs.bias", 1, C, wo.ln_in_b, 0);
    e(sa + "norm_slots.weight", 1, D, wo.ln_s_g, 0); e(sa + "norm_slots.bias", 1, D, wo.ln_s_b, 0);
    e(sa + "norm_mlp.weight", 1, D, wo.ln_m_g, 0); e(sa + "norm_mlp.bias", 1, D, wo.ln_m_b, 0);
    e(sa + "project_q.weight", D, D, wo.Wq, 2); e(sa + "project_q.weight", D, D, wo.WqT, 3);
    e(sa + "project_k.weight", D, C, wo.Wk, 2); e(sa + "project_k.weight", D, C, wo.WkT, 3);
    e(sa + "project_v.weight", D, C, wo.Wv, 2); e(sa + "project_v.weight", D, C, wo.WvT, 3);
    e(sa + "gru.weight_ih", 3 * D, D, wo.Wih, 2); e(sa + "gru.weight_ih", 3 * D, D, wo.WihT, 3);
    e(sa + "gru.weight_hh", 3 * D, D, wo.Whh, 2); e(sa + "gru.weight_hh", 3 * D, D, wo.WhhT, 3);
    e(sa + "gru.bias_ih", 1, 3 * D, wo.bih, 0); e(sa + "gru.bias_hh", 1, 3 * D, wo.bhh, 0);
    e(sa + "mlp.0.weight", H, D, wo.W0, 2); e(sa + "mlp.0.weight", H, D, wo.W0T, 3); e(sa + "mlp.0.bias", 1, H, wo.b0, 0);
    e(sa + "mlp.2.weight", D, H, wo.W2, 2); e(sa + "mlp.2.weight", D, H, wo.W2T, 3); e(sa + "mlp.2.bias", 1, D, wo.b2, 0);
    sa_pack_n_ = (int)ent.size();
    sa_pack_max_ = 3 * D * D;
    OCRL_REQUIRE(sa_pack_n_ <= 64, "pack table overflow");
    OCRL_HIP(hipMemcpy(sa_pack_dev_, ent.data(), ent.size() * sizeof(PackEntry), hipMemcpyHostToDevice));
    OCRL_HIP(hipDeviceSynchronize());
    have_fwd_ = false;
    return 0;
}

int SlateModel::soft_z(hipStream_t st) {
    if (!fused_heads() || cfg.use_bcdec) return 0;
    OCRL_REQUIRE(have_scores_, "soft_z: no forward since the last backward (the scores have been overwritten by their gradient)");
    return exp_rows_launch(zraw_, zlse_, z_, (long long)last_.B * T, V, st);
}
int SlateModel::dropout_mask(unsigned site, long long n, float* out, hipStream_t st) const {
    return dropout_mask_launch(out, n, pdrop_, last_.seed, site, st);
}

int SlateModel::conv_layer_fwd(const float* x, const float* pack, const float* bias, float* y, int Bn, int Hh, int Ww, int KS, int CIN,
                               int relu, const float* posmap, const float* mask, hipStream_t st) {
    ConvArgs a;
    a.X = x; a.Wp = pack; a.Y = y; a.B = Bn; a.H = Hh; a.W = Ww; a.bias = bias; a.relu = relu; a.posmap = posmap; a.mask = mask;
    if (conv_x3_ > 0 && (KS == 5 || KS == 3) && CIN == 64 && !conv_lowlat_) {
        auto it = x3_of_.find(pack);
        if (it != x3_of_.end()) return conv_x3_launch(a, it->second, st, KS);
    }
    return conv_fwd_launch(a, KS, CIN, 64, st, conv_lowlat_);
}
int SlateModel::conv_layer_wgrad(const float* x, const float* dy, float* dW, float* db, int Bn, int Hh, int Ww, int KS, int CIN,
                                 int cin_real, hipStream_t st) {
    WgradArgs a;
    a.X = x; a.dY = dy; a.part = scratch_; a.B = Bn; a.H = Hh; a.W = Ww;
    OCRL_REQUIRE(conv_wgrad_ws_floats(Bn, Hh, Ww, KS, CIN) <= scratch_floats_, "conv wgrad: scratch too small");
    RC(conv_wgrad_launch(a, KS, CIN, 64, cin_real, dW, 0, st, conv_x3_ > 0 ? 1 : 0));
    if (db) RC(colsum_launch(dy, 64, db, (long long)Bn * Hh * Ww, 64, 0, 1.f, scratch_, scratch_floats_, st));
    return 0;
}

int SlateModel::pack_weights(hipStream_t st, bool encoder_only) {
    RC(conv_pack_launch(P("_enc._encoder.0.m.weight"), cw_fwd_[0], nullptr, 5, 8, 64, cfg.obs_channels, st));
    RC(conv_pack_launch(P("_enc._encoder.1.m.weight"), cw_fwd_[1], cw_bwd_[1], 5, 64, 64, 64, st));
    RC(conv_pack_launch(P("_enc._encoder.2.m.weight"), cw_fwd_[2], cw_bwd_[2], 5, 64, 64, 64, st));
    RC(conv_pack_launch(P("_enc._encoder.3.weight"), cw_fwd_[3], cw_bwd_[3], 5, 64, 64, 64, st));
    if (conv_x3_ > 0) {
        const char* names[4] = {nullptr, "_enc._encoder.1.m.weight", "_enc._encoder.2.m.weight", "_enc._encoder.3.weight"};
        for (int i = 1; i < 4; ++i) {
            auto f = x3_of_.find(cw_fwd_[i]), b = x3_of_.find(cw_bwd_[i]);
            if (f != x3_of_.end()) RC(conv_pack_x3_launch(P(names[i]), const_cast<float*>(f->second), b != x3_of_.end() ? const_cast<float*>(b->second) : nullptr, st));
        }
    }
    if (!cfg.use_bcdec && !encoder_only) {
        RC(conv_pack_launch(P("_dvae._decoder.1.m.weight"), dw_fwd_[0], dw_bwd_[0], 3, 64, 64, 64, st));
        RC(conv_pack_launch(P("_dvae._decoder.6.m.weight"), dw_fwd_[1], dw_bwd_[1], 3, 64, 64, 64, st));
        if (conv_x3_ > 0) {
            const char* names[2] = {"_dvae._decoder.1.m.weight", "_dvae._decoder.6.m.weight"};
            for (int i = 0; i < 2; ++i) {
                auto f = x3_of_.find(dw_fwd_[i]), b = x3_of_.find(dw_bwd_[i]);
// ... 242 lines not shown
    const size_t bytes = (size_t)in.B * cfg.obs_channels * N * sizeof(float);
    OCRL_HIP(hipMemcpyAsync(obs_stage_, in.obs, bytes, hipMemcpyDeviceToDevice, st));
    RC(store_u64_launch(seed_dev_, in.seed, st));
    if (!eg.exec) {
        StepInputs gi = in;
        gi.obs = obs_stage_; gi.seed_dev = seed_dev_;
        hipGraph_t g = nullptr;
        if (!cap_) OCRL_HIP(hipStreamCreateWithFlags(&cap_, hipStreamNonBlocking));
        OCRL_HIP(hipStreamBeginCapture(cap_, hipStreamCaptureModeThreadLocal));
        int rc = frozen_ ? 0 : pack_weights(cap_, true);
        if (!rc) rc = fwd_encoder(gi, cap_);
        const hipError_t ce = hipStreamEndCapture(cap_, &g);
        if (rc) { if (g) (void)hipGraphDestroy(g); return rc; }
        OCRL_HIP(ce);
        OCRL_HIP(hipGraphInstantiate(&eg.exec, g, nullptr, nullptr, 0));
        OCRL_HIP(hipGraphDestroy(g));
    }
    OCRL_HIP(hipGraphLaunch(eg.exec, st));
    return 0;
}

void SlateModel::clear_encode_graphs() {
    for (auto& kv : enc_graphs_) if (kv.second.exec) (void)hipGraphExecDestroy(kv.second.exec);
    enc_graphs_.clear();
}

int SlateModel::encode_backward(const float* dslots, hipStream_t st) {
    OCRL_REQUIRE(have_enc_, "encode_backward: call encode first (its activations are what is differentiated)");
    OCRL_REQUIRE(!frozen_, "encode_backward: the weights are frozen (ocrl_slate_freeze_weights): encode() kept no activations");
    OCRL_REQUIRE(g_ && dslots, "encode_backward: no gradient buffer bound / null dslots");
    RC(fill_launch(g_, flat_size_, 0.f, st));
    RC(copy_launch(dslots, gslots_, (long long)last_.B * K * D, st));
    RC(bwd_encoder(st));
    have_enc_ = false;
    enc_only_grads_ = true;
    return 0;
}

int SlateModel::generate(hipStream_t st) {
    OCRL_REQUIRE(!cfg.use_bcdec, "generate: the autoregressive decoder is not part of the use_bcdec configuration");
    OCRL_REQUIRE(last_.B > 0 && last_.obs, "generate: run forward or encode first");
    have_enc_ = false;
    const int B = last_.B;
    const long long BK = (long long)B * K;
    pdrop_ = 0.f;
    have_fwd_ = false;
    OCRL_HIP(hipMemsetAsync(tokens_, 0, sizeof(int) * (size_t)B * T, st));
    RC(lin_fwd(slots_, D, P("_slotproj.weight"), nullptr, mem_, d, BK, d, D, 0, nullptr, 0, 0.f, 0, st));
    for (int b = 0; b < NB; ++b) {
        const std::string pre = fmt("_tfdec.blocks.%d.", b);
        RC(lin_fwd(mem_, d, P(pre + "encoder_decoder_attn.proj_k.weight"), nullptr, blk_[b].ck, d, BK, d, d, 0, nullptr, 0, 0.f, 0, st));
        RC(lin_fwd(mem_, d, P(pre + "encoder_decoder_attn.proj_v.weight"), nullptr, blk_[b].cv, d, BK, d, d, 0, nullptr, 0, 0.f, 0, st));
    }
    float* x0 = emb_;
    for (int t = 0; t < T; ++t) {
        RC(embed_step_launch(tokens_, P("_dict.dictionary.weight"), P("_bos_token._bos_token"), P("_z_pos.pe"), x0, B, T, d, t, st));
        const float* xin = x0;
        for (int b = 0; b < NB; ++b) {
            Blk& k = blk_[b];
            const std::string pre = fmt("_tfdec.blocks.%d.", b);
            RC(layernorm_fwd_launch(xin, P(pre + "self_attn_layer_norm.weight"), P(pre + "self_attn_layer_norm.bias"), k.ln1, k.ln1_mean, k.ln1_rstd, B, d, st));
            const float* res = (b == 0) ? k.ln1 : xin;
            RC(lin_fwd(k.ln1, d, P(pre + "self_attn.proj_q.weight"), nullptr, k.q + (size_t)t * 3 * d, T * 3 * d, B, 3 * d, d, 0, nullptr, 0, 0.f, 0, st));
            RC(decode_attn_launch(k.q, k.ao, B, T, t, d, NH, 3 * d, st));
            RC(lin_fwd(k.ao, d, P(pre + "self_attn.proj_o.weight"), nullptr, k.x1, d, B, d, d, 0, res, d, 0.f, 0, st));
            RC(layernorm_fwd_launch(k.x1, P(pre + "encoder_decoder_attn_layer_norm.weight"), P(pre + "encoder_decoder_attn_layer_norm.bias"), k.ln2, k.ln2_mean, k.ln2_rstd, B, d, st));
            RC(lin_fwd(k.ln2, d, P(pre + "encoder_decoder_attn.proj_q.weight"), nullptr, k.cq, d, B, d, d, 0, nullptr, 0, 0.f, 0, st));
            RC(cross_attn_fwd_launch(k.cq, k.ck, k.cv, k.cao, k.cP, B, 1, K, d, NH, 0.f, 0, 0, st));
            RC(lin_fwd(k.cao, d, P(pre + "encoder_decoder_attn.proj_o.weight"), nullptr, k.x2, d, B, d, d, 0, k.x1, d, 0.f, 0, st));
            RC(layernorm_fwd_launch(k.x2, P(pre + "ffn_layer_norm.weight"), P(pre + "ffn_layer_norm.bias"), k.ln3, k.ln3_mean, k.ln3_rstd, B, d, st));
            RC(lin_fwd(k.ln3, d, P(pre + "ffn.0.weight"), P(pre + "ffn.0.bias"), k.f1, 4 * d, B, 4 * d, d, 1, nullptr, 0, 0.f, 0, st));
            RC(lin_fwd(k.f1, 4 * d, P(pre + "ffn.2.weight"), P(pre + "ffn.2.bias"), k.x3, d, B, d, 4 * d, 0, k.x2, d, 0.f, 0, st));
            xin = k.x3;
        }
        RC(layernorm_fwd_launch(xin, P("_tfdec.layer_norm.weight"), P("_tfdec.layer_norm.bias"), lnf_, lnf_mean_, lnf_rstd_, B, d, st));
        RC(lin_fwd(lnf_, d, P("_out.weight"), nullptr, pred_, V, B, V, d, 0, nullptr, 0, 0.f, 0, st));
        RC(argmax_pos_launch(pred_, tokens_, B, T, V, t, st, 1));
    }
    RC(onehot_launch(tokens_, z_, (long long)B * T, V, st));
    RC(dvae_decode(B, nullptr, st, z_));
    return 0;
}

int SlateModel::bwd_decoder(hipStream_t st) {
    const int B = last_.B;
    const long long BT = (long long)B * T, BK = (long long)B * K;
    const float p = pdrop_;
    const float scale = 1.0f / sqrtf((float)DH);
    const bool dws = dw_mode_ != 0 && side_ != nullptr;
    hipStream_t sw = dws ? (dw_mode_ == 2 ? side2_ : side_) : st;
    float* const sw_scratch = dw_mode_ == 2 ? scratch3_ : scratch2_;
    auto dw_sync = [&]() -> int {
        if (!dws) return 0;
        hipEvent_t ev = ev_dw_[ev_dw_next_++ & 7];
        OCRL_HIP(hipEventRecord(ev, st));
        OCRL_HIP(hipStreamWaitEvent(sw, ev, 0));
        return 0;
    };
    auto dw = [&](const float* dy, int ld_dy, const float* x, int ldx, float* dW, float* db, long long M, int N_out, int K_in, Xf xf = Xf()) -> int {
        float* keep = scratch_;
        if (dws) scratch_ = sw_scratch;
        const int rc = lin_bwd_w(dy, ld_dy, x, ldx, dW, db, M, N_out, K_in, 1.f, sw, xf);
        scratch_ = keep;
        return rc;
    };
    auto on_sw = [&](const std::function<int()>& body) -> int {
        float* keep = scratch_;
        if (dws) scratch_ = sw_scratch;
        const int rc = body();
        scratch_ = keep;
        return rc;
    };
    Xf ce; ce.a_mode = 3; ce.lse = celse_; ce.tok = tokens_; ce.scale = 1.0f / last_.B;
    RC(dw_sync());
    RC(dw(pred_, V, lnf_, d, G("_out.weight"), nullptr, BT, V, d, ce));
    RC(lin_bwd_x(pred_, V, P("_out.weight"), gt1_, d, BT, V, d, nullptr, 0, nullptr, 0, st, Drop(), ce));
    const float* xlast = blk_[NB - 1].x3;
    RC(layernorm_bwd_launch(gt1_, xlast, lnf_mean_, lnf_rstd_, P("_tfdec.layer_norm.weight"), gx_, G("_tfdec.layer_norm.weight"), BT, d, 0, 0,
                            scratch_, scratch_floats_, st));
    RC(fill_launch(gmem_, BK * d, 0.f, st));
    for (int b = NB - 1; b >= 0; --b) {
        Blk& k = blk_[b];
        const BlkG& q = bg_[dws ? b : 0];
        const std::string pre = fmt("_tfdec.blocks.%d.", b);
        const unsigned site = SITE_BLK_BASE + 8 * b;
        const float* xin = (b == 0) ? emb_ : blk_[b - 1].x3;
        const float* gd = gx_;
        auto drop_gx = [&](unsigned s_, float* into) -> int {
            gd = gx_;
            if (p > 0.f || dws) { RC(dropout_apply_launch(gx_, into, BT * d, p, last_.seed, s_, st)); gd = into; }
            return 0;
        };
        RC(drop_gx(site + 4, q.gbr[0]));
        RC(lin_bwd_x(gd, d, P(pre + "ffn.2.weight"), q.gf1, 4 * d, BT, d, 4 * d, k.f1, 4 * d, nullptr, 0, st));
        RC(dw_sync());
        RC(dw(gd, d, k.f1, 4 * d, G(pre + "ffn.2.weight"), G(pre + "ffn.2.bias"), BT, d, 4 * d));
        RC(dw(q.gf1, 4 * d, k.ln3, d, G(pre + "ffn.0.weight"), G(pre + "ffn.0.bias"), BT, 4 * d, d));
        RC(lin_bwd_x(q.gf1, 4 * d, P(pre + "ffn.0.weight"), gt1_, d, BT, 4 * d, d, nullptr, 0, nullptr, 0, st));
        RC(layernorm_bwd_launch(gt1_, k.x2, k.ln3_mean, k.ln3_rstd, P(pre + "ffn_layer_norm.weight"), gx_, G(pre + "ffn_layer_norm.weight"), BT, d, 1, 0,
                                scratch_, scratch_floats_, st));
        RC(drop_gx(site + 3, q.gbr[1]));
        const float* gd_co = gd;
        if (xattn_) {
            const int NC = NH * xattn_kp(K, NH);
            XaHost hx;
            hx.x = k.ln2; hx.y = gt1_; hx.P = k.cP; hx.Ab = k.xaAb; hx.AbT = k.xaAbT; hx.Vo = k.xaVo; hx.VoT = k.xaVoT; hx.gd = gd_co; hx.Pd = q.xaPd; hx.dS = q.xaDs;
            hx.B = B; hx.T = T; hx.K = K; hx.d = d; hx.h = NH; hx.p = p; hx.seed = last_.seed; hx.site_p = site + 2; hx.site_o = site + 3;
            RC(xattn_launch(hx, 1, st));
            RC(dw_sync());
            RC(on_sw([&]() -> int {
                const int KP = xattn_kp(K, NH), dh = DH;
                const float* Wq = P(pre + "encoder_decoder_attn.proj_q.weight");
                const float* Wo = P(pre + "encoder_decoder_attn.proj_o.weight");
                GemmArgs ga;
                ga.M = NC; ga.N = d; ga.K = T; ga.lda = NC; ga.ldb = d; ga.ldc = d; ga.akc = 0; ga.bkc = 0; ga.batch = B;
                ga.sA = (long long)T * NC; ga.sB = (long long)T * d; ga.sC = (long long)NC * d;
                ga.A = q.xaPd; ga.B = gd_co; ga.C = xa_dVo_;
                RC(gemm_launch(ga, sw));
                ga.A = q.xaDs; ga.B = k.ln2; ga.C = xa_dAb_;
                RC(gemm_launch(ga, sw));
                GemmArgs gb;
                gb.M = K; gb.N = dh; gb.K = d; gb.akc = 1; gb.bkc = 1; gb.lda = d; gb.ldb = d; gb.ldc = d; gb.batch = B * NH; gb.batch_inner = NH; gb.alpha = scale;
                gb.A = xa_dAb_; gb.sA = (long long)NC * d; gb.sAi = (long long)KP * d;
                gb.B = Wq; gb.sB = 0; gb.sBi = (long long)dh * d;
                gb.C = gck_; gb.sC = (long long)K * d; gb.sCi = dh;
                RC(gemm_launch(gb, sw));
                GemmArgs gc;
                gc.M = K; gc.N = dh; gc.K = d; gc.akc = 1; gc.bkc = 0; gc.lda = d; gc.ldb = d; gc.ldc = d; gc.batch = B * NH; gc.batch_inner = NH;
                gc.A = xa_dVo_; gc.sA = (long long)NC * d; gc.sAi = (long long)KP * d;
                gc.B = Wo; gc.sB = 0; gc.sBi = dh;
                gc.C = gcv_; gc.sC = (long long)K * d; gc.sCi = dh;
                RC(gemm_launch(gc, sw));
                GemmArgs gq;
                gq.M = dh; gq.N = d; gq.K = K; gq.akc = 0; gq.bkc = 0; gq.lda = d; gq.ldb = d; gq.ldc = d; gq.batch = B * NH; gq.batch_inner = NH; gq.alpha = scale;
                gq.A = k.ck; gq.sA = (long long)K * d; gq.sAi = dh;
                gq.B = xa_dAb_; gq.sB = (long long)NC * d; gq.sBi = (long long)KP * d;
                gq.C = xa_pq_; gq.sC = (long long)d * d; gq.sCi = (long long)dh * d;
                RC(gemm_launch(gq, sw));
                GemmArgs go;
                go.M = d; go.N = dh; go.K = K; go.akc = 0; go.bkc = 0; go.lda = d; go.ldb = d; go.ldc = d; go.batch = B * NH; go.batch_inner = NH;
                go.A = xa_dVo_; go.sA = (long long)NC * d; go.sAi = (long long)KP * d;
                go.B = k.cv; go.sB = (long long)K * d; go.sBi = dh;
                go.C = xa_po_; go.sC = (long long)d * d; go.sCi = dh;
                RC(gemm_launch(go, sw));
                RC(colsum_launch(xa_pq_, (long long)d * d, G(pre + "encoder_decoder_attn.proj_q.weight"), B, d * d, 0, 1.f, scratch_, scratch_floats_, sw));
                RC(colsum_launch(xa_po_, (long long)d * d, G(pre + "encoder_decoder_attn.proj_o.weight"), B, d * d, 0, 1.f, scratch_, scratch_floats_, sw));
                return 0;
            }));
        } else {
        RC(lin_bwd_x(gd, d, P(pre + "encoder_decoder_attn.proj_o.weight"), gt1_, d, BT, d, d, nullptr, 0, nullptr, 0, st));
        RC(cross_attn_bwd_launch(gt1_, k.cq, k.ck, k.cv, k.cP, q.gt2, gck_, gcv_, B, T, K, d, NH, p, last_.seed, site + 2, scratch_, scratch_floats_, st));
        RC(dw_sync());
        RC(dw(gd_co, d, k.cao, d, G(pre + "encoder_decoder_attn.proj_o.weight"), nullptr, BT, d, d));
        RC(dw(q.gt2, d, k.ln2, d, G(pre + "encoder_decoder_attn.proj_q.weight"), nullptr, BT, d, d));
        RC(lin_bwd_x(q.gt2, d, P(pre + "encoder_decoder_attn.proj_q.weight"), gt1_, d, BT, d, d, nullptr, 0, nullptr, 0, st));
        }
        {
            hipStream_t sx = xattn_ ? sw : st;
            auto body = [&]() -> int {
                RC(lin_bwd_w(gck_, d, mem_, d, G(pre + "encoder_decoder_attn.proj_k.weight"), nullptr, BK, d, d, 1.f, sx));
                RC(lin_bwd_w(gcv_, d, mem_, d, G(pre + "encoder_decoder_attn.proj_v.weight"), nullptr, BK, d, d, 1.f, sx));
                RC(lin_bwd_x(gck_, d, P(pre + "encoder_decoder_attn.proj_k.weight"), gmem_, d, BK, d, d, nullptr, 0, gmem_, d, sx));
                RC(lin_bwd_x(gcv_, d, P(pre + "encoder_decoder_attn.proj_v.weight"), gmem_, d, BK, d, d, nullptr, 0, gmem_, d, sx));
                return 0;
            };
            if (xattn_) RC(on_sw(body)); else RC(body());
        }
        RC(layernorm_bwd_launch(gt1_, k.x1, k.ln2_mean, k.ln2_rstd, P(pre + "encoder_decoder_attn_layer_norm.weight"), gx_,
                                G(pre + "encoder_decoder_attn_layer_norm.weight"), BT, d, 1, 0, scratch_, scratch_floats_, st));
        RC(drop_gx(site + 1, q.gbr[2]));
        const float* gd_o = gd;
        RC(lin_bwd_x(gd, d, P(pre + "self_attn.proj_o.weight"), gt1_, d, BT, d, d, nullptr, 0, nullptr, 0, st));
        {
            AttnArgs a;
            a.q = k.q; a.k = k.k; a.v = k.v; a.o = k.ao; a.lse = k.lse; a.B = B; a.T = T; a.d = d; a.h = NH; a.ld = 3 * d;
            a.p = p; a.seed = last_.seed; a.site = site + 0;
            a.dO = gt1_; a.dq = q.gqkv; a.dk = q.gqkv + d; a.dv = q.gqkv + 2 * d; a.delta = attn_delta_;
            RC(attn_launch(a, 1, st));
        }
        RC(dw_sync());
        RC(dw(gd_o, d, k.ao, d, G(pre + "self_attn.proj_o.weight"), nullptr, BT, d, d));
        RC(dw(q.gqkv, 3 * d, k.ln1, d, G(pre + "self_attn.proj_q.weight"), nullptr, BT, 3 * d, d));
        RC(lin_bwd_x(q.gqkv, 3 * d, P(pre + "self_attn.proj_q.weight"), gt1_, d, BT, 3 * d, d, nullptr, 0, nullptr, 0, st));
        if (b == 0) {
            RC(axpy_launch(gx_, gt1_, BT * d, 1.f, st));
            RC(layernorm_bwd_launch(gt1_, xin, k.ln1_mean, k.ln1_rstd, P(pre + "self_attn_layer_norm.weight"), gx_,
                                    G(pre + "self_attn_layer_norm.weight"), BT, d, 0, 0, scratch_, scratch_floats_, st));
        } else {
            RC(layernorm_bwd_launch(gt1_, xin, k.ln1_mean, k.ln1_rstd, P(pre + "self_attn_layer_norm.weight"), gx_,
                                    G(pre + "self_attn_layer_norm.weight"), BT, d, 1, 0, scratch_, scratch_floats_, st));
        }
    }
    RC(embed_bwd_launch(gx_, tokens_, G("_dict.dictionary.weight"), B, T, V, d, p, last_.seed, scratch_, scratch_floats_, st));
    RC(fill_launch(G("_z_pos.pe"), (long long)(T + 1) * d, 0.f, st));
    RC(colsum_launch(gx_, (long long)T * d, G("_z_pos.pe"), B, T * d, 0, 1.f, scratch_, scratch_floats_, st));
    RC(copy_launch(G("_z_pos.pe"), G("_bos_token._bos_token"), d, st));
    if (dws && xattn_) {
        hipEvent_t ev = ev_dw_[ev_dw_next_++ & 7];
        OCRL_HIP(hipEventRecord(ev, sw));
        OCRL_HIP(hipStreamWaitEvent(st, ev, 0));
    }
    RC(lin_bwd_w(gmem_, d, slots_, D, G("_slotproj.weight"), nullptr, BK, d, D, 1.f, st));
    RC(lin_bwd_x(gmem_, d, P("_slotproj.weight"), gslots_, D, BK, d, D, nullptr, 0, nullptr, 0, st));
    return 0;
}

int SlateModel::bwd_encoder(hipStream_t st, bool fork_dvae) {
    const int B = last_.B;
    const long long BN = (long long)B * N, R = (long long)B * I * K;
    const SaSave so = sa_save_layout(C, D, H, SH);
    const SaGrad go = sa_grad_layout(C, D, H, SH);
    const std::string sa = "_slotattn.slot_attention.";
    SlotAttnArgs a;
    a.B = B; a.N = N; a.C = C; a.K = K; a.D = D; a.H = H; a.I = I; a.NH = SH; a.eps = 1e-8f; a.scale = 1.0f / sqrtf((float)(D / SH));
    a.x = x_; a.wts = sa_wts_; a.save = sa_save_; a.dslots = gslots_; a.dx = gA_; a.dslots0 = gslots0_; a.grows = sa_grows_; a.g_small = sa_small_;
    a.xchg = sa_xchg_; a.parts = sa_parts_;
    if (fork_dvae) {
        RC(fork_side(st));
        std::swap(scratch_, scratch2_);
        const int rc = bwd_dvae(side_);
        std::swap(scratch_, scratch2_);
        RC(rc);
    }
    RC(slot_attn_launch(a, 1, st));
    const bool side_w = side_ && overlap_mode_ >= 3 && !cfg.use_bcdec && !fork_dvae;
    hipStream_t sw = side_w ? side_ : st;
    if (side_w) { RC(fork_side(st)); std::swap(scratch_, scratch2_); }
    auto sa_weight_grads = [&]() -> int {
    RC(lin_bwd_w(sa_grows_ + go.out, go.ld, sa_save_ + so.hid, so.ld, G(sa + "mlp.2.weight"), G(sa + "mlp.2.bias"), R, D, H, 1.f, sw));
    RC(lin_bwd_w(sa_grows_ + go.hid, go.ld, sa_save_ + so.m, so.ld, G(sa + "mlp.0.weight"), G(sa + "mlp.0.bias"), R, H, D, 1.f, sw));
    RC(lin_bwd_w(sa_grows_ + go.gi, go.ld, sa_save_ + so.u, so.ld, G(sa + "gru.weight_ih"), G(sa + "gru.bias_ih"), R, 3 * D, D, 1.f, sw));
    RC(lin_bwd_w(sa_grows_ + go.gh, go.ld, sa_save_ + so.sprev, so.ld, G(sa + "gru.weight_hh"), G(sa + "gru.bias_hh"), R, 3 * D, D, 1.f, sw));
    RC(lin_bwd_w(sa_grows_ + go.q, go.ld, sa_save_ + so.sn, so.ld, G(sa + "project_q.weight"), nullptr, R, D, D, 1.f, sw));
    for (int h = 0, dh = D / SH; h < SH; ++h) {
        RC(lin_bwd_w(sa_grows_ + go.u + h * dh, go.ld, sa_save_ + so.up + h * C, so.ld, G(sa + "project_v.weight") + (size_t)h * dh * C, nullptr, R, dh, C, 1.f, sw));
        RC(lin_bwd_w(sa_save_ + so.q + h * dh, so.ld, sa_grows_ + go.qp + h * C, go.ld, G(sa + "project_k.weight") + (size_t)h * dh * C, nullptr, R, dh, C, a.scale, sw));
    }
    const int SM = 4 * D + 2 * C;
    RC(colsum_launch(sa_small_ + 0, SM, G(sa + "norm_slots.weight"), B, 2 * D, 0, 1.f, scratch_, scratch_floats_, sw));
    RC(colsum_launch(sa_small_ + 2 * D, SM, G(sa + "norm_mlp.weight"), B, 2 * D, 0, 1.f, scratch_, scratch_floats_, sw));
    RC(colsum_launch(sa_small_ + 4 * D, SM, G(sa + "norm_inputs.weight"), B, 2 * C, 0, 1.f, scratch_, scratch_floats_, sw));
    RC(slot_init_bwd_launch(gslots0_, P("_slotattn.slot_log_sigma"), last_.noise_slots, G("_slotattn.slot_mu"), G("_slotattn.slot_log_sigma"),
                            B * K, D, last_.seed, sw));
    RC(lin_bwd_w(gA_, C, h1_, C, G("_slotattn.mlp.2.weight"), G("_slotattn.mlp.2.bias"), BN, C, C, 1.f, sw));
    if (side_w) RC(im2col5_launch(obs8_, col0_, BN, S, S, cfg.obs_channels, (25 * cfg.obs_channels + 3) & ~3, sw));
    return 0;
    };
    {
        const int rc = sa_weight_grads();
        if (side_w) std::swap(scratch_, scratch2_);
        RC(rc);
    }
    RC(lin_bwd_x(gA_, C, P("_slotattn.mlp.2.weight"), gB_, C, BN, C, C, h1_, C, nullptr, 0, st));
    RC(lin_bwd_w(gB_, C, ln0_, C, G("_slotattn.mlp.0.weight"), G("_slotattn.mlp.0.bias"), BN, C, C, 1.f, st));
    float* gL = side_w ? gC_ : gA_;
    RC(lin_bwd_x(gB_, C, P("_slotattn.mlp.0.weight"), gL, C, BN, C, C, nullptr, 0, nullptr, 0, st));
    RC(layernorm_bwd_launch(gL, e4_, ln0_mean_, ln0_rstd_, P("_slotattn.layer_norm.weight"), gB_, G("_slotattn.layer_norm.weight"), BN, C, 0, 0,
                            scratch_, scratch_floats_, st));
    RC(colsum_launch(gB_, (long long)N * C, gmap_, B, N * C, 0, 1.f, scratch_, scratch_floats_, st));
    RC(lin_bwd_w(gmap_, C, gridT_, 4, G("_enc_pos.channels_map.weight"), G("_enc_pos.channels_map.bias"), N, C, 4, 1.f, st));
    if (fork_dvae || side_w) RC(join_side(st));
    if (dw_mode_ == 2 && side2_) {
        OCRL_HIP(hipEventRecord(ev_join2_, side2_));
        OCRL_HIP(hipStreamWaitEvent(st, ev_join2_, 0));
    }
    RC(colsum_launch(gmap_, C, G("_enc._encoder.3.bias"), N, C, 0, 1.f, scratch_, scratch_floats_, st));
    RC(conv_layer_wgrad(e3_, gB_, G("_enc._encoder.3.weight"), nullptr, B, S, S, 5, 64, 64, st));
    RC(conv_layer_fwd(gB_, cw_bwd_[3], nullptr, gA_, B, S, S, 5, 64, 0, nullptr, e3_, st));
    RC(conv_layer_wgrad(e2_, gA_, G("_enc._encoder.2.m.weight"), G("_enc._encoder.2.m.bias"), B, S, S, 5, 64, 64, st));
    RC(conv_layer_fwd(gA_, cw_bwd_[2], nullptr, gB_, B, S, S, 5, 64, 0, nullptr, e2_, st));
    RC(conv_layer_wgrad(e1_, gB_, G("_enc._encoder.1.m.weight"), G("_enc._encoder.1.m.bias"), B, S, S, 5, 64, 64, st));
    RC(conv_layer_fwd(gB_, cw_bwd_[1], nullptr, gA_, B, S, S, 5, 64, 0, nullptr, e1_, st));
    {
        const int ch = cfg.obs_channels, ldc0 = (25 * ch + 3) & ~3;
        if (!side_w) RC(im2col5_launch(obs8_, col0_, BN, S, S, ch, ldc0, st));
        RC(lin_bwd_w(gA_, 64, col0_, ldc0, dw0p_, G("_enc._encoder.0.m.bias"), BN, 64, ldc0, 1.f, st));
        RC(unpack5_launch(dw0p_, G("_enc._encoder.0.m.weight"), ch, ldc0, st));
    }
    return 0;
}

int SlateModel::bwd_dvae(hipStream_t st) {
    const int B = last_.B;
    const long long BT = (long long)B * T, BN = (long long)B * N;
// ... 190 lines not shown
```

ocrl_amd/csrc/slate_model.h:

```cpp
#pragma once
#include <map>
#include <string>
#include <vector>

#include "kernels.h"
#include "model_base.h"

struct SlateConfig {
    int obs_size = 64, obs_channels = 3, vocab = 4096, d_model = 192, cnn_hidden = 64;
    int num_slots = 5, num_iters = 3, slot_size = 192, mlp_hidden = 192;
    int num_blocks = 4, num_heads = 4;
    float dropout = 0.1f;
    int max_batch = 1;
    int use_bcdec = 0;
    int hard = 0;
    int slot_heads = 1;
};

struct StepInputs {
    const float* obs = nullptr;
    int B = 0;
    float tau = 1.f;
    int train = 1;
    unsigned long long seed = 0;
    const float* noise_z = nullptr;
    const float* noise_zh = nullptr;
    const float* noise_slots = nullptr;
    const unsigned long long* seed_dev = nullptr;
};

class SlateModel : public ModelBase {
public:
    explicit SlateModel(const SlateConfig& c);
    ~SlateModel();
    long long group_begin(int g) const { return group_begin_[g]; }
    int bind(float* p, float* g, float* m, float* v, void* ws, size_t ws_bytes);
    int forward(const StepInputs& in, hipStream_t st);
    int backward(hipStream_t st);
    int encode(const StepInputs& in, hipStream_t st);
    void freeze_weights(bool on) { frozen_ = on; packs_valid_ = false; clear_encode_graphs(); }
    void clear_encode_graphs();
    int encode_backward(const float* dslots, hipStream_t st);
    int generate(hipStream_t st);
    int clip_adam(const float lr[3], float clip, int step, float gscale, hipStream_t st);
    int grad_norm(hipStream_t st);
    int dropout_mask(unsigned site, long long n, float* out, hipStream_t st) const;
    int soft_z(hipStream_t st);
    const SlateConfig cfg;

private:
    void layout_workspace(bool commit);
    int lin_fwd(const float* x, int ldx, const float* W, const float* b, float* y, int ldy, long long M, int N, int K, int relu,
                const float* resid, int ldr, float drop_p, unsigned site, hipStream_t st) {
        return ::lin_fwd(x, ldx, W, b, y, ldy, M, N, K, relu, resid, ldr, st, Drop{drop_p, last_.seed, site});
    }
    int lin_bwd_w(const float* dy, int ld_dy, const float* x, int ldx, float* dW, float* db, long long M, int N_out, int K_in,
                  float alpha, hipStream_t st, Xf xf = Xf()) {
        return ::lin_bwd_w(dy, ld_dy, x, ldx, dW, db, M, N_out, K_in, alpha, scratch_, scratch_floats_, st, Drop(), xf);
    }
    bool fused_heads() const { return !cfg.hard; }
    int conv_layer_fwd(const float* x, const float* pack, const float* bias, float* y, int Bn, int Hh, int Ww, int KS, int CIN, int relu,
                       const float* posmap, const float* mask, hipStream_t st);
    int conv_layer_wgrad(const float* x, const float* dy, float* dW, float* db, int Bn, int Hh, int Ww, int KS, int CIN, int cin_real,
                         hipStream_t st);
    int pack_weights(hipStream_t st, bool encoder_only = false);
    int fwd_encoder(const StepInputs& in, hipStream_t st, int fork_dvae = 0);
    int fwd_dvae(const StepInputs& in, hipStream_t st);
    int fwd_decoder(hipStream_t st, bool with_ce = true);
    int dvae_decode(int B, float* drecon, hipStream_t st, const float* zin = nullptr);
    int bwd_decoder(hipStream_t st);
    int bwd_encoder(hipStream_t st, bool fork_dvae = false);
    int bwd_dvae(hipStream_t st);
    int pack_bcdec(hipStream_t st);
    int fwd_bcdec(hipStream_t st);
    int bwd_bcdec(hipStream_t st);

    long long group_begin_[4] = {0, 0, 0, 0};

    int S, E, T, N, V, d, C, K, I, D, H, NB, NH, DH, Bmax;
    int SH = 1;
    StepInputs last_;
    float pdrop_ = 0.f;
    bool have_fwd_ = false;
    int conv_lowlat_ = 0;
    bool frozen_ = false, packs_valid_ = false;
    bool have_enc_ = false;
    bool enc_only_grads_ = false;
    bool have_scores_ = false;

    float *scratch_ = nullptr;
    size_t scratch_floats_ = 0;
    float* scratch2_ = nullptr;
    int overlap_mode_ = 0;
    hipStream_t side_ = nullptr;
    hipEvent_t ev_fork_ = nullptr, ev_join_ = nullptr, ev_tokens_ = nullptr;
    int fork_side(hipStream_t st);
    int join_side(hipStream_t st);
    float *zstat_ = nullptr, *zhstat_ = nullptr, *zlse_ = nullptr, *zdot_ = nullptr, *cestat_ = nullptr, *celse_ = nullptr, *cepart_ = nullptr;
    int* zhidx_ = nullptr;
    float *obs8_, *patches_, *de_[7], *zraw_, *z_, *zdec_;
    int* tokens_;
    float *dd0_, *dd1_, *dd2_, *dd3_, *dd4_, *ps1_, *dd6_, *dd7_, *dd8_, *dd9_, *ps2_, *recon_, *drecon_;
    float *e1_, *e2_, *e3_, *e4_, *posmap_, *gridT_, *ln0_, *ln0_mean_, *ln0_rstd_, *h1_, *x_;
    float *slots0_, *slot_noise_, *slots_, *attn_, *sa_save_, *sa_wts_, *sa_grows_, *sa_small_, *sa_xchg_;
    float* attn_heads_ = nullptr;
    float* sa_parts_;
    PackEntry* sa_pack_dev_ = nullptr;
    int sa_pack_n_ = 0, sa_pack_max_ = 0;
    float *cw_fwd_[4], *cw_bwd_[4];
    int conv_x3_ = -1;
    std::map<const float*, const float*> x3_of_;
    float *dw_fwd_[2], *dw_bwd_[2];
    float *w11p_;
    float *mem_, *emb_;
    struct Blk {
        float *ln1, *ln1_mean, *ln1_rstd, *q, *k, *v, *lse, *ao, *x1;
        float *ln2, *ln2_mean, *ln2_rstd, *cq, *ck, *cv, *cP, *cao, *x2;
        float *ln3, *ln3_mean, *ln3_rstd, *f1, *x3;
        float *xaAb, *xaAbT, *xaVo, *xaVoT;
    };
    bool xattn_ = false;
    float *xa_dAb_ = nullptr, *xa_dVo_ = nullptr, *xa_pq_ = nullptr, *xa_po_ = nullptr;
    size_t xa_zero_floats_ = 0;
    float* xa_zero_base_ = nullptr;
    std::vector<Blk> blk_;
    struct BlkG { float *gbr[3], *gf1, *gt2, *gqkv, *xaPd, *xaDs; };
    std::vector<BlkG> bg_;
    struct EncGraph { hipGraphExec_t exec = nullptr; int warm = 0; };
    std::map<int, EncGraph> enc_graphs_;
    int enc_graph_mode_ = -1;
    hipStream_t cap_ = nullptr;
    float* obs_stage_ = nullptr;
    unsigned long long* seed_dev_ = nullptr;
    int dw_mode_ = 0;
    hipStream_t side2_ = nullptr;
    float* scratch3_ = nullptr;
    hipEvent_t ev_dw_[8] = {nullptr, nullptr, nullptr, nullptr, nullptr, nullptr, nullptr, nullptr};
    hipEvent_t ev_join2_ = nullptr;
    int ev_dw_next_ = 0;
    float *attn_delta_;
    float *lnf_, *lnf_mean_, *lnf_rstd_, *pred_;
    float *gqkv_;
    float *gx_, *gbr_, *gt1_, *gt2_, *gt3_, *gf1_, *gmem_, *gck_, *gcv_, *gslots_, *gslots0_;
    float *gA_, *gB_, *gC_;
    float *gdA_, *gdB_;
    float *gmap_;
    float *col0_, *dw0p_;
    float *bc_Wc_, *bc_W1r_, *bc_P1_, *bc_M_, *bc_T_, *bc_c1_, *bc_c2_, *bc_c3_, *bc_out4_, *bc_dout4_, *bc_gA_, *bc_gB_;
    float *bc_pk_[2], *bc_pkb_[2], *bc_Wk4_, *bc_Wb4_, *bc_dW1r_, *bc_dWc_, *bc_dT_, *bc_dM_, *bc_G1_;
};
```

Before: 1703.

## Defer split-K and column-sum reductions into batched table-driven reduce launches

Split-K weight-gradient reductions, LayerNorm gamma/beta column sums and cross-attention colsums in the decoder backward pass are no longer launched one by one. They are recorded as jobs in a per-step table, with partials kept in dedicated arena slabs, and flushed per block through a single table-driven reduce kernel on the side stream. The goal is fewer small kernel launches and less serialization on the shared scratch buffer. The cost is extra workspace for the arena and LayerNorm slots, host-to-device job-table uploads, and extra dw_sync points before each flush.

```diff
diff --git a/include/ocrl_hip.h b/include/ocrl_hip.h
--- a/include/ocrl_hip.h
+++ b/include/ocrl_hip.h
@@ -108,6 +108,19 @@
 int ocrl_layernorm_bwd(const float* dy, const float* x, const float* mean, const float* rstd, const float* gamma, float* dx, float* dgb,
                        long long R, int F, float* ws, size_t ws_floats, void* stream);
 
+int ocrl_splitk_reduce(const float* part, float* out, long long n, int splits, long long stride, int accumulate, void* stream);
+int ocrl_colsum(const float* X, long long ld, float* out, long long R, int F, int accumulate, float scale, float* ws, size_t ws_floats, void* stream);
+enum { OCRL_REDUCE_SPLITK = 0, OCRL_REDUCE_COLSUM = 1, OCRL_REDUCE_COLSUM4 = 2, OCRL_REDUCE_COLSUM_FINAL = 3 };
+typedef struct ocrl_reduce_job {
+    const float* src; float* dst;
+    long long part_stride, rows, ld;
+    int parts, cols, accumulate, kind;
+    float scale;
+    int chain;
+} ocrl_reduce_job;
+size_t ocrl_reduce_job_size(void);
+int ocrl_reduce_table(const ocrl_reduce_job* jobs, int njobs, void* stream);
+
 int ocrl_attention_fwd(const float* q, const float* k, const float* v, float* o, float* lse, int B, int T, int d, int h, int ld,
                        float p, unsigned long long seed, unsigned site, void* stream);
 int ocrl_attention_bwd(const float* q, const float* k, const float* v, const float* o, const float* lse, const float* dO,
diff --git a/ocrl_amd/csrc/capi.cpp b/ocrl_amd/csrc/capi.cpp
--- a/ocrl_amd/csrc/capi.cpp
+++ b/ocrl_amd/csrc/capi.cpp
@@ -289,6 +289,32 @@
 int ocrl_layernorm_fwd(const float* x, const float* g, const float* b, float* y, float* mean, float* rstd, long long R, int F, void* stream) {
     return layernorm_fwd_launch(x, g, b, y, mean, rstd, R, F, ST(stream));
 }
+int ocrl_splitk_reduce(const float* part, float* out, long long n, int splits, long long stride, int accumulate, void* stream) {
+    return splitk_reduce_launch(part, out, n, splits, stride, accumulate, ST(stream));
+}
+int ocrl_colsum(const float* X, long long ld, float* out, long long R, int F, int accumulate, float scale, float* ws, size_t ws_floats, void* stream) {
+    return colsum_launch(X, ld, out, R, F, accumulate, scale, ws, ws_floats, ST(stream));
+}
+size_t ocrl_reduce_job_size(void) { return sizeof(ocrl_reduce_job); }
+int ocrl_reduce_table(const ocrl_reduce_job* jobs, int njobs, void* stream) {
+    OCRL_REQUIRE(jobs && njobs >= 1 && njobs <= 4096, "reduce table: 1..4096 jobs");
+    std::vector<ReduceJob> host(jobs, jobs + njobs);
+    std::vector<int> prefix(njobs + 1);
+    RC(reduce_table_prepare(host.data(), njobs, prefix.data()));
+    const size_t jb = (size_t)njobs * sizeof(ReduceJob), pb = (size_t)(njobs + 1) * sizeof(int);
+    char* dev = nullptr;
+    OCRL_HIP(hipMalloc(&dev, jb + pb));
+    int rc = 0;
+    if (hipMemcpy(dev, host.data(), jb, hipMemcpyHostToDevice) != hipSuccess || hipMemcpy(dev + jb, prefix.data(), pb, hipMemcpyHostToDevice) != hipSuccess) {
+        rc = 1;
+    } else {
+        rc = reduce_table_launch(reinterpret_cast<const ReduceJob*>(dev), reinterpret_cast<const int*>(dev + jb), njobs, prefix[njobs], ST(stream));
+        if (hipStreamSynchronize(ST(stream)) != hipSuccess) rc = 1;
+    }
+    (void)hipFree(dev);
+    OCRL_REQUIRE(rc == 0, "reduce table: upload or launch failed");
+    return 0;
+}
 int ocrl_layernorm_bwd(const float* dy, const float* x, const float* mean, const float* rstd, const float* g, float* dx, float* dgb, long long R,
                        int F, float* ws, size_t ws_floats, void* stream) {
     return layernorm_bwd_launch(dy, x, mean, rstd, g, dx, dgb, R, F, 0, 0, ws, ws_floats, ST(stream));
diff --git a/ocrl_amd/csrc/elementwise.hip b/ocrl_amd/csrc/elementwise.hip
--- a/ocrl_amd/csrc/elementwise.hip
+++ b/ocrl_amd/csrc/elementwise.hip
@@ -1,5 +1,6 @@
 #include "common.h"
 #include "kernels.h"
+#include "reduce_impl.h"
 
 #define TINYF 1.17549435e-38f
 
@@ -332,68 +333,17 @@
 }
 
 __global__ void colsum_kernel(const float* __restrict__ X, long long ld, float* __restrict__ part, long long R, int F, long long rows_per_chunk) {
-    __shared__ float red[4][64];
-    const int col = blockIdx.x * 64 + (threadIdx.x & 63), rl = threadIdx.x >> 6;
-    const long long r0 = (long long)blockIdx.y * rows_per_chunk;
-    const long long r1 = min(R, r0 + rows_per_chunk);
-    float s = 0.f;
-    if (col < F)
-        for (long long r = r0 + rl; r < r1; r += 4) s += X[r * ld + col];
-    red[rl][threadIdx.x & 63] = s;
-    __syncthreads();
-    if (rl == 0 && col < F) part[(size_t)blockIdx.y * F + col] = red[0][threadIdx.x] + red[1][threadIdx.x] + red[2][threadIdx.x] + red[3][threadIdx.x];
+    __shared__ float4 red[256];
+    colsum_body(X, ld, part, R, F, rows_per_chunk, blockIdx.x, blockIdx.y, red);
 }
 __global__ __launch_bounds__(256) void colsum4_kernel(const float* __restrict__ X, long long ld, float* __restrict__ part, long long R, int F,
                                                       long long rows_per_chunk) {
     __shared__ float4 red[256];
-    const int F4 = F >> 2, RL = 256 / F4;
-    const int c4 = threadIdx.x % F4, rl = threadIdx.x / F4;
-    const long long r0 = (long long)blockIdx.x * rows_per_chunk;
-    const long long r1 = min(R, r0 + rows_per_chunk);
-    float4 s0 = make_float4(0.f, 0.f, 0.f, 0.f), s1 = s0, s2 = s0, s3 = s0;
-    if (rl < RL) {
-        const float* base = X + (size_t)c4 * 4;
-        long long r = r0 + rl;
-        for (; r + 3 * RL < r1; r += 4 * RL) {
-            const float4 a = *reinterpret_cast<const float4*>(base + r * ld), b = *reinterpret_cast<const float4*>(base + (r + RL) * ld);
-            const float4 c = *reinterpret_cast<const float4*>(base + (r + 2 * RL) * ld), d = *reinterpret_cast<const float4*>(base + (r + 3 * RL) * ld);
-            s0.x += a.x; s0.y += a.y; s0.z += a.z; s0.w += a.w;
-            s1.x += b.x; s1.y += b.y; s1.z += b.z; s1.w += b.w;
-            s2.x += c.x; s2.y += c.y; s2.z += c.z; s2.w += c.w;
-            s3.x += d.x; s3.y += d.y; s3.z += d.z; s3.w += d.w;
-        }
-        for (; r < r1; r += RL) {
-            const float4 a = *reinterpret_cast<const float4*>(base + r * ld);
-            s0.x += a.x; s0.y += a.y; s0.z += a.z; s0.w += a.w;
-        }
-    }
-    red[threadIdx.x] = make_float4(s0.x + s1.x + s2.x + s3.x, s0.y + s1.y + s2.y + s3.y, s0.z + s1.z + s2.z + s3.z, s0.w + s1.w + s2.w + s3.w);
-    __syncthreads();
-    if (threadIdx.x < F4) {
-        float4 t = red[threadIdx.x];
-        for (int k = 1; k < RL; ++k) { const float4 v = red[k * F4 + threadIdx.x]; t.x += v.x; t.y += v.y; t.z += v.z; t.w += v.w; }
-        *reinterpret_cast<float4*>(part + (size_t)blockIdx.x * F + threadIdx.x * 4) = t;
-    }
+    colsum4_body(X, ld, part, R, F, rows_per_chunk, blockIdx.x, red);
 }
 __global__ __launch_bounds__(256) void colsum_final_kernel(const float* __restrict__ part, float* __restrict__ out, int nchunk, int F, int accumulate, float scale) {
-    __shared__ float red[16][16];
-    const int cl = threadIdx.x & 15, rl = threadIdx.x >> 4;
-    const int c = blockIdx.x * 16 + cl;
-    float s0 = 0.f, s1 = 0.f;
-    if (c < F) {
-        int k = rl;
-        for (; k + 16 < nchunk; k += 32) { s0 += part[(size_t)k * F + c]; s1 += part[(size_t)(k + 16) * F + c]; }
-        if (k < nchunk) s0 += part[(size_t)k * F + c];
-    }
-    red[rl][cl] = s0 + s1;
-    __syncthreads();
-    if (rl == 0 && c < F) {
-        float t = 0.f;
-#pragma unroll
-        for (int k = 0; k < 16; ++k) t += red[k][cl];
-        t *= scale;
-        out[c] = accumulate ? out[c] + t : t;
-    }
+    __shared__ float4 red[256];
+    colsum_final_body(part, out, nchunk, F, accumulate, scale, blockIdx.x, red);
 }
 
 __global__ void reduce_partials_kernel(const float* __restrict__ part, int n, float* __restrict__ out, float scale, int accumulate) {
@@ -1365,36 +1315,56 @@
     OCRL_CHECK_LAUNCH("layernorm_fwd");
     return 0;
 }
-int colsum_launch(const float* X, long long ld, float* out, long long R, int F, int accumulate, float scale, float* ws, size_t ws_floats, hipStream_t st) {
+int colsum_jobs(const float* X, long long ld, float* out, long long R, int F, int accumulate, float scale, float* ws, size_t ws_floats, ReduceJob* jobs,
+                size_t* ws_used) {
+    ReduceJob s1 = {}, fin = {};
+    s1.src = X; s1.dst = ws; s1.rows = R; s1.ld = ld; s1.cols = F; s1.scale = 1.f;
+    fin.src = ws; fin.dst = out; fin.cols = F; fin.accumulate = accumulate; fin.scale = scale; fin.kind = OCRL_REDUCE_COLSUM_FINAL;
+    long long nchunk = 0;
     if (F % 4 == 0 && ld % 4 == 0 && F <= 1024 && F >= 4 && (((uintptr_t)X) & 15) == 0 && R >= 1024) {
-        long long nchunk = 2048;
+        nchunk = 2048;
         if (nchunk > R / 8) nchunk = R / 8;
         if ((size_t)nchunk * F > ws_floats) nchunk = (long long)(ws_floats / F);
         if (nchunk >= 16) {
             const long long rpc = (R + nchunk - 1) / nchunk;
             nchunk = (R + rpc - 1) / rpc;
-            hipLaunchKernelGGL(colsum4_kernel, dim3((unsigned)nchunk), dim3(256), 0, st, X, ld, ws, R, F, rpc);
-            OCRL_CHECK_LAUNCH("colsum4");
-            hipLaunchKernelGGL(colsum_final_kernel, dim3(cdiv(F, 16)), dim3(256), 0, st, ws, out, (int)nchunk, F, accumulate, scale);
-            OCRL_CHECK_LAUNCH("colsum_final");
-            return 0;
-        }
-    }
-    const int cb = cdiv(F, 64);
-    long long nchunk = 1024 / cb;
-    if (nchunk < 1) nchunk = 1;
-    if (nchunk > (R + 63) / 64) nchunk = (R + 63) / 64;
-    if (nchunk < 1) nchunk = 1;
-    OCRL_REQUIRE((size_t)nchunk * F <= ws_floats, "colsum: workspace too small (%lld x %d)", nchunk, F);
-    const long long rpc = (R + nchunk - 1) / nchunk;
-    hipLaunchKernelGGL(colsum_kernel, dim3(cb, (int)nchunk), dim3(256), 0, st, X, ld, ws, R, F, rpc);
-    OCRL_CHECK_LAUNCH("colsum");
-    hipLaunchKernelGGL(colsum_final_kernel, dim3(cdiv(F, 16)), dim3(256), 0, st, ws, out, (int)nchunk, F, accumulate, scale);
+            s1.kind = OCRL_REDUCE_COLSUM4; s1.part_stride = rpc;
+        } else {
+            nchunk = 0;
+        }
+    }
+    if (!nchunk) {
+        const int cb = cdiv(F, 64);
+        nchunk = 1024 / cb;
+        if (nchunk < 1) nchunk = 1;
+        if (nchunk > (R + 63) / 64) nchunk = (R + 63) / 64;
+        if (nchunk < 1) nchunk = 1;
+        OCRL_REQUIRE((size_t)nchunk * F <= ws_floats, "colsum: workspace too small (%lld x %d)", nchunk, F);
+        s1.kind = OCRL_REDUCE_COLSUM; s1.part_stride = (R + nchunk - 1) / nchunk;
+    }
+    s1.parts = fin.parts = (int)nchunk;
+    jobs[0] = s1; jobs[1] = fin;
+    if (ws_used) *ws_used = (size_t)nchunk * F;
+    return 0;
+}
+int colsum_launch(const float* X, long long ld, float* out, long long R, int F, int accumulate, float scale, float* ws, size_t ws_floats, hipStream_t st) {
+    ReduceJob j[2];
+    RC(colsum_jobs(X, ld, out, R, F, accumulate, scale, ws, ws_floats, j, nullptr));
+    const long long rpc = j[0].part_stride;
+    const int nchunk = j[0].parts;
+    if (j[0].kind == OCRL_REDUCE_COLSUM4) {
+        hipLaunchKernelGGL(colsum4_kernel, dim3((unsigned)nchunk), dim3(256), 0, st, X, ld, ws, R, F, rpc);
+        OCRL_CHECK_LAUNCH("colsum4");
+    } else {
+        hipLaunchKernelGGL(colsum_kernel, dim3(cdiv(F, 64), nchunk), dim3(256), 0, st, X, ld, ws, R, F, rpc);
+        OCRL_CHECK_LAUNCH("colsum");
+    }
+    hipLaunchKernelGGL(colsum_final_kernel, dim3(cdiv(F, 16)), dim3(256), 0, st, ws, out, nchunk, F, accumulate, scale);
     OCRL_CHECK_LAUNCH("colsum_final");
     return 0;
 }
-int layernorm_bwd_launch(const float* dy, const float* x, const float* mean, const float* rstd, const float* g, float* dx,
-                         float* dgb, long long R, int F, int accumulate_dx, int accumulate_dgb, float* ws, size_t ws_floats, hipStream_t st) {
+int layernorm_bwd_partials_launch(const float* dy, const float* x, const float* mean, const float* rstd, const float* g, float* dx, long long R, int F,
+                                  int accumulate_dx, float* ws, size_t ws_floats, int* nblk_out, hipStream_t st) {
     OCRL_REQUIRE(F % 64 == 0 && F >= 64 && F <= 256, "layernorm bwd: F must be 64..256, multiple of 64 (got %d)", F);
     int nblk = (int)((R + 3) / 4);
     if (nblk > 2048) nblk = 2048;
@@ -1417,6 +1387,14 @@
         default: hipLaunchKernelGGL(layernorm_bwd_kernel<4>, grid, blk, 0, st, dy, x, mean, rstd, g, dx, ws, R, accumulate_dx); break;
     }
     OCRL_CHECK_LAUNCH("layernorm_bwd");
+    *nblk_out = nblk;
+    return 0;
+}
+int layernorm_bwd_launch(const float* dy, const float* x, const float* mean, const float* rstd, const float* g, float* dx,
+                         float* dgb, long long R, int F, int accumulate_dx, int accumulate_dgb, float* ws, size_t ws_floats, hipStream_t st) {
+    int nblk;
+    RC(layernorm_bwd_partials_launch(dy, x, mean, rstd, g, dx, R, F, accumulate_dx, ws, ws_floats, &nblk, st));
+    const size_t need = (size_t)nblk * 2 * F;
     return colsum_launch(ws, 2 * F, dgb, nblk, 2 * F, accumulate_dgb, 1.f, ws + need, ws_floats - need, st);
 }
 int reduce_partials_launch(const float* part, int n, float* out, float scale, int accumulate, hipStream_t st) {
diff --git a/ocrl_amd/csrc/gemm.hip b/ocrl_amd/csrc/gemm.hip
--- a/ocrl_amd/csrc/gemm.hip
+++ b/ocrl_amd/csrc/gemm.hip
@@ -1,5 +1,6 @@
 #include "common.h"
 #include "kernels.h"
+#include "reduce_impl.h"
 #include <stdlib.h>
 
 int gemm_launch_tt(const GemmArgs& a, const GemmPlan& p, hipStream_t st);
@@ -8,33 +9,8 @@
 
 __global__ __launch_bounds__(256) void splitk_reduce_kernel(const float* __restrict__ part, float* __restrict__ out, long long n4,
                                                             int splits, long long stride, int accumulate) {
-    __shared__ float4 red[16][16];
-    const int cl = threadIdx.x & 15, sl = threadIdx.x >> 4;
-    const long long i = (long long)blockIdx.x * 16 + cl;
-    float4 s = make_float4(0.f, 0.f, 0.f, 0.f);
-    if (i < n4) {
-        int k = sl;
-        for (; k + 48 < splits; k += 64) {
-            const float4 v0 = *reinterpret_cast<const float4*>(part + (size_t)k * stride + i * 4);
-            const float4 v1 = *reinterpret_cast<const float4*>(part + (size_t)(k + 16) * stride + i * 4);
-            const float4 v2 = *reinterpret_cast<const float4*>(part + (size_t)(k + 32) * stride + i * 4);
-            const float4 v3 = *reinterpret_cast<const float4*>(part + (size_t)(k + 48) * stride + i * 4);
-            s.x += (v0.x + v1.x) + (v2.x + v3.x); s.y += (v0.y + v1.y) + (v2.y + v3.y);
-            s.z += (v0.z + v1.z) + (v2.z + v3.z); s.w += (v0.w + v1.w) + (v2.w + v3.w);
-        }
-        for (; k < splits; k += 16) {
-            const float4 v = *reinterpret_cast<const float4*>(part + (size_t)k * stride + i * 4);
-            s.x += v.x; s.y += v.y; s.z += v.z; s.w += v.w;
-        }
-    }
-    red[sl][cl] = s;
-    __syncthreads();
-    if (sl == 0 && i < n4) {
-        float4 t = accumulate ? *reinterpret_cast<const float4*>(out + i * 4) : make_float4(0.f, 0.f, 0.f, 0.f);
-#pragma unroll
-        for (int k = 0; k < 16; ++k) { t.x += red[k][cl].x; t.y += red[k][cl].y; t.z += red[k][cl].z; t.w += red[k][cl].w; }
-        *reinterpret_cast<float4*>(out + i * 4) = t;
-    }
+    __shared__ float4 red[256];
+    splitk_reduce_body(part, out, n4, splits, stride, accumulate, blockIdx.x, red);
 }
 
 static int env_tile() {
@@ -199,20 +175,44 @@
     return 0;
 }
 
-int lin_bwd_w(const float* dy, int ld_dy, const float* x, int ldx, float* dW, float* db, long long M, int N_out, int K_in, float alpha, float* sk,
-              size_t sk_floats, hipStream_t st, Drop dr, Xf xf, int accumulate, int max_splits) {
-    OCRL_REQUIRE(!(db && accumulate), "lin_bwd_w: a fused bias gradient is written, not accumulated");
+static GemmArgs lin_bwd_w_args(const float* dy, int ld_dy, const float* x, int ldx, float* dW, float* db, long long M, int N_out, int K_in, float alpha) {
     GemmArgs a;
     a.A = dy; a.B = x; a.C = dW; a.M = N_out; a.N = K_in; a.K = (int)M; a.lda = ld_dy; a.ldb = ldx; a.ldc = K_in; a.akc = 0; a.bkc = 0;
     a.alpha = alpha; a.bias_out = db;
+    return a;
+}
+
+int lin_bwd_w(const float* dy, int ld_dy, const float* x, int ldx, float* dW, float* db, long long M, int N_out, int K_in, float alpha, float* sk,
+              size_t sk_floats, hipStream_t st, Drop dr, Xf xf, int accumulate, int max_splits, ReduceJob* defer) {
+    OCRL_REQUIRE(!(db && accumulate), "lin_bwd_w: a fused bias gradient is written, not accumulated");
+    GemmArgs a = lin_bwd_w_args(dy, ld_dy, x, ldx, dW, db, M, N_out, K_in, alpha);
     set_adrop(a, dr, N_out);
     set_xf(a, xf);
+    if (defer) { defer[0] = ReduceJob(); defer[1] = ReduceJob(); }
     int splits;
     RC(lin_splitk_count(a, sk_floats, max_splits, &splits));
     if (splits > 1) {
         a.splitk = splits;
-        return gemm_splitk_launch(a, sk, (N_out + 3) & ~3, accumulate, st);
+        const long long bslab = (N_out + 3) & ~3;
+        if (!defer) return gemm_splitk_launch(a, sk, bslab, accumulate, st);
+        gemm_splitk_layout(a, sk, bslab);
+        RC(gemm_launch(a, st));
+        ReduceJob& w = defer[0];
+        w.kind = OCRL_REDUCE_SPLITK; w.src = sk; w.dst = dW; w.cols = (int)a.sCsplit; w.parts = splits; w.part_stride = a.sCsplit; w.accumulate = accumulate; w.scale = 1.f;
+        if (db) {
+            ReduceJob& b = defer[1];
+            b.kind = OCRL_REDUCE_SPLITK; b.src = a.bias_out; b.dst = db; b.cols = a.M; b.parts = splits; b.part_stride = bslab; b.scale = 1.f;
+        }
+        return 0;
     }
     if (accumulate) { a.resid = dW; a.ldr = K_in; }
     return gemm_launch(a, st);
 }
+
+int lin_bwd_w_sk_floats(long long M, int N_out, int K_in, size_t sk_floats, int max_splits, size_t* need) {
+    const GemmArgs a = lin_bwd_w_args(nullptr, 4, nullptr, 4, nullptr, nullptr, M, N_out, K_in, 1.f);
+    int splits;
+    RC(lin_splitk_count(a, sk_floats, max_splits, &splits));
+    *need = splits > 1 ? (size_t)splits * ((size_t)N_out * K_in + ((N_out + 3) & ~3)) : 0;
+    return 0;
+}
diff --git a/ocrl_amd/csrc/kernels.h b/ocrl_amd/csrc/kernels.h
--- a/ocrl_amd/csrc/kernels.h
+++ b/ocrl_amd/csrc/kernels.h
@@ -48,6 +48,10 @@
 void gemm_splitk_layout(GemmArgs& a, float* ws, long long bslab);
 int gemm_splitk_launch(GemmArgs a, float* ws, long long bslab, int accumulate, hipStream_t st);
 
+typedef ocrl_reduce_job ReduceJob;
+int reduce_table_prepare(ReduceJob* jobs, int njobs, int* prefix);
+int reduce_table_launch(const ReduceJob* jobs_dev, const int* prefix_dev, int njobs, int workgroups, hipStream_t st);
+
 struct Drop { float p = 0.f; unsigned long long seed = 0; unsigned site = 0; };
 struct Xf { int a_mode = 0, b_mode = 0; const float* lse = nullptr; const int* tok = nullptr; float scale = 1.f; };
 int lin_fwd(const float* x, int ldx, const float* W, const float* b, float* y, int ldy, long long M, int N, int K, int relu, const float* resid,
@@ -55,7 +59,8 @@
 int lin_bwd_x(const float* dy, int ld_dy, const float* W, float* dx, int ldx, long long M, int N_out, int K_in, const float* mask, int ldmask,
               const float* resid, int ldr, hipStream_t st, Drop dr = Drop(), Xf xf = Xf(), float alpha = 1.f);
 int lin_bwd_w(const float* dy, int ld_dy, const float* x, int ldx, float* dW, float* db, long long M, int N_out, int K_in, float alpha, float* sk,
-              size_t sk_floats, hipStream_t st, Drop dr = Drop(), Xf xf = Xf(), int accumulate = 0, int max_splits = 0);
+              size_t sk_floats, hipStream_t st, Drop dr = Drop(), Xf xf = Xf(), int accumulate = 0, int max_splits = 0, ReduceJob* defer = nullptr);
+int lin_bwd_w_sk_floats(long long M, int N_out, int K_in, size_t sk_floats, int max_splits, size_t* need);
 
 int pool_embed_launch(const float* lin, const float* cls, const float* pos, float* x0, int B, int K, int d, hipStream_t st);
 int pool_rows_launch(const float* in, float* out, int B, int K, int d, int mode, hipStream_t st);
@@ -227,6 +232,10 @@
 int layernorm_bwd_launch(const float* dy, const float* x, const float* mean, const float* rstd, const float* g, float* dx,
                          float* dgb, long long R, int F, int accumulate_dx, int accumulate_dgb, float* ws, size_t ws_floats, hipStream_t st);
 int colsum_launch(const float* X, long long ld, float* out, long long R, int F, int accumulate, float scale, float* ws, size_t ws_floats, hipStream_t st);
+int colsum_jobs(const float* X, long long ld, float* out, long long R, int F, int accumulate, float scale, float* ws, size_t ws_floats, ReduceJob* jobs,
+                size_t* ws_used);
+int layernorm_bwd_partials_launch(const float* dy, const float* x, const float* mean, const float* rstd, const float* g, float* dx, long long R, int F,
+                                  int accumulate_dx, float* ws, size_t ws_floats, int* nblk, hipStream_t st);
 int reduce_partials_launch(const float* part, int n, float* out, float scale, int accumulate, hipStream_t st);
 int mse_launch(const float* obs, const float* recon, float* drecon, float* out, int B, int C, int H, int W, float* ws, size_t ws_floats, hipStream_t st);
 int gumbel_softmax_launch(const float* raw, const float* e1, const float* e2, float* z, int* tokens, long long R, int V, float tau,
diff --git a/ocrl_amd/csrc/reduce_impl.h b/ocrl_amd/csrc/reduce_impl.h
--- /dev/null
+++ b/ocrl_amd/csrc/reduce_impl.h
@@ -0,0 +1,100 @@
+#pragma once
+#include "common.h"
+
+static __device__ __forceinline__ void splitk_reduce_body(const float* part, float* out, long long n4, int splits, long long stride, int accumulate,
+                                                          unsigned bx, float4* red) {
+    const int cl = threadIdx.x & 15, sl = threadIdx.x >> 4;
+    const long long i = (long long)bx * 16 + cl;
+    float4 s = make_float4(0.f, 0.f, 0.f, 0.f);
+    if (i < n4) {
+        int k = sl;
+        for (; k + 48 < splits; k += 64) {
+            const float4 v0 = *reinterpret_cast<const float4*>(part + (size_t)k * stride + i * 4);
+            const float4 v1 = *reinterpret_cast<const float4*>(part + (size_t)(k + 16) * stride + i * 4);
+            const float4 v2 = *reinterpret_cast<const float4*>(part + (size_t)(k + 32) * stride + i * 4);
+            const float4 v3 = *reinterpret_cast<const float4*>(part + (size_t)(k + 48) * stride + i * 4);
+            s.x += (v0.x + v1.x) + (v2.x + v3.x); s.y += (v0.y + v1.y) + (v2.y + v3.y);
+            s.z += (v0.z + v1.z) + (v2.z + v3.z); s.w += (v0.w + v1.w) + (v2.w + v3.w);
+        }
+        for (; k < splits; k += 16) {
+            const float4 v = *reinterpret_cast<const float4*>(part + (size_t)k * stride + i * 4);
+            s.x += v.x; s.y += v.y; s.z += v.z; s.w += v.w;
+        }
+    }
+    red[sl * 16 + cl] = s;
+    __syncthreads();
+    if (sl == 0 && i < n4) {
+        float4 t = accumulate ? *reinterpret_cast<const float4*>(out + i * 4) : make_float4(0.f, 0.f, 0.f, 0.f);
+#pragma unroll
+        for (int k = 0; k < 16; ++k) { t.x += red[k * 16 + cl].x; t.y += red[k * 16 + cl].y; t.z += red[k * 16 + cl].z; t.w += red[k * 16 + cl].w; }
+        *reinterpret_cast<float4*>(out + i * 4) = t;
+    }
+}
+
+static __device__ __forceinline__ void colsum_body(const float* X, long long ld, float* part, long long R, int F, long long rows_per_chunk, unsigned bx,
+                                                   unsigned by, float4* red4) {
+    float* red = reinterpret_cast<float*>(red4);
+    const int col = bx * 64 + (threadIdx.x & 63), rl = threadIdx.x >> 6;
+    const long long r0 = (long long)by * rows_per_chunk;
+    const long long r1 = min(R, r0 + rows_per_chunk);
+    float s = 0.f;
+    if (col < F)
+        for (long long r = r0 + rl; r < r1; r += 4) s += X[r * ld + col];
+    red[rl * 64 + (threadIdx.x & 63)] = s;
+    __syncthreads();
+    if (rl == 0 && col < F) part[(size_t)by * F + col] = red[threadIdx.x] + red[64 + threadIdx.x] + red[128 + threadIdx.x] + red[192 + threadIdx.x];
+}
+
+static __device__ __forceinline__ void colsum4_body(const float* X, long long ld, float* part, long long R, int F, long long rows_per_chunk, unsigned bx,
+                                                    float4* red) {
+    const int F4 = F >> 2, RL = 256 / F4;
+    const int c4 = threadIdx.x % F4, rl = threadIdx.x / F4;
+    const long long r0 = (long long)bx * rows_per_chunk;
+    const long long r1 = min(R, r0 + rows_per_chunk);
+    float4 s0 = make_float4(0.f, 0.f, 0.f, 0.f), s1 = s0, s2 = s0, s3 = s0;
+    if (rl < RL) {
+        const float* base = X + (size_t)c4 * 4;
+        long long r = r0 + rl;
+        for (; r + 3 * RL < r1; r += 4 * RL) {
+            const float4 a = *reinterpret_cast<const float4*>(base + r * ld), b = *reinterpret_cast<const float4*>(base + (r + RL) * ld);
+            const float4 c = *reinterpret_cast<const float4*>(base + (r + 2 * RL) * ld), d = *reinterpret_cast<const float4*>(base + (r + 3 * RL) * ld);
+            s0.x += a.x; s0.y += a.y; s0.z += a.z; s0.w += a.w;
+            s1.x += b.x; s1.y += b.y; s1.z += b.z; s1.w += b.w;
+            s2.x += c.x; s2.y += c.y; s2.z += c.z; s2.w += c.w;
+            s3.x += d.x; s3.y += d.y; s3.z += d.z; s3.w += d.w;
+        }
+        for (; r < r1; r += RL) {
+            const float4 a = *reinterpret_cast<const float4*>(base + r * ld);
+            s0.x += a.x; s0.y += a.y; s0.z += a.z; s0.w += a.w;
+        }
+    }
+    red[threadIdx.x] = make_float4(s0.x + s1.x + s2.x + s3.x, s0.y + s1.y + s2.y + s3.y, s0.z + s1.z + s2.z + s3.z, s0.w + s1.w + s2.w + s3.w);
+    __syncthreads();
+    if (threadIdx.x < F4) {
+        float4 t = red[threadIdx.x];
+        for (int k = 1; k < RL; ++k) { const float4 v = red[k * F4 + threadIdx.x]; t.x += v.x; t.y += v.y; t.z += v.z; t.w += v.w; }
+        *reinterpret_cast<float4*>(part + (size_t)bx * F + threadIdx.x * 4) = t;
+    }
+}
+
+static __device__ __forceinline__ void colsum_final_body(const float* part, float* out, int nchunk, int F, int accumulate, float scale, unsigned bx,
+                                                         float4* red4) {
+    float* red = reinterpret_cast<float*>(red4);
+    const int cl = threadIdx.x & 15, rl = threadIdx.x >> 4;
+    const int c = bx * 16 + cl;
+    float s0 = 0.f, s1 = 0.f;
+    if (c < F) {
+        int k = rl;
+        for (; k + 16 < nchunk; k += 32) { s0 += part[(size_t)k * F + c]; s1 += part[(size_t)(k + 16) * F + c]; }
+        if (k < nchunk) s0 += part[(size_t)k * F + c];
+    }
+    red[rl * 16 + cl] = s0 + s1;
+    __syncthreads();
+    if (rl == 0 && c < F) {
+        float t = 0.f;
+#pragma unroll
+        for (int k = 0; k < 16; ++k) t += red[k * 16 + cl];
+        t *= scale;
+        out[c] = accumulate ? out[c] + t : t;
+    }
+}
diff --git a/ocrl_amd/csrc/reduce_table.hip b/ocrl_amd/csrc/reduce_table.hip
--- /dev/null
+++ b/ocrl_amd/csrc/reduce_table.hip
@@ -0,0 +1,90 @@
+#include "common.h"
+#include "kernels.h"
+#include "reduce_impl.h"
+#include <vector>
+
+static __device__ __forceinline__ void reduce_job_run(const ReduceJob& j, unsigned w, float4* red) {
+    switch (j.kind) {
+        case OCRL_REDUCE_SPLITK: splitk_reduce_body(j.src, j.dst, j.cols >> 2, j.parts, j.part_stride, j.accumulate, w, red); break;
+        case OCRL_REDUCE_COLSUM: {
+            const unsigned cb = (unsigned)(j.cols + 63) >> 6;
+            colsum_body(j.src, j.ld, j.dst, j.rows, j.cols, j.part_stride, w % cb, w / cb, red);
+            break;
+        }
+        case OCRL_REDUCE_COLSUM4: colsum4_body(j.src, j.ld, j.dst, j.rows, j.cols, j.part_stride, w, red); break;
+        default: colsum_final_body(j.src, j.dst, j.parts, j.cols, j.accumulate, j.scale, w, red); break;
+    }
+}
+
+__global__ __launch_bounds__(256) void reduce_table_kernel(const ReduceJob* __restrict__ jobs, const int* __restrict__ prefix, int njobs) {
+    __shared__ float4 red[256];
+    int lo = 0, hi = njobs;
+    while (hi - lo > 1) {
+        const int mid = (lo + hi) >> 1;
+        if (prefix[mid] <= (int)blockIdx.x) lo = mid; else hi = mid;
+    }
+    const unsigned w = blockIdx.x - (unsigned)prefix[lo];
+    const int chain = jobs[lo].chain;
+    for (int c = 0; c <= chain; ++c) {
+        if (c) __syncthreads();
+        reduce_job_run(jobs[lo + c], w, red);
+    }
+}
+
+static long long job_workgroups(const ReduceJob& j) {
+    if (j.cols <= 0 || j.parts <= 0) return 0;
+    switch (j.kind) {
+        case OCRL_REDUCE_SPLITK: return cdiv((long long)(j.cols / 4), 16);
+        case OCRL_REDUCE_COLSUM: return (long long)cdiv(j.cols, 64) * j.parts;
+        case OCRL_REDUCE_COLSUM4: return j.parts;
+        default: return cdiv(j.cols, 16);
+    }
+}
+
+int reduce_table_prepare(ReduceJob* jobs, int njobs, int* prefix) {
+    long long total = 0;
+    std::vector<int> head(njobs, -1);
+    for (int i = 0; i < njobs; ++i) {
+        ReduceJob& j = jobs[i];
+        j.chain = 0;
+        OCRL_REQUIRE(j.kind >= OCRL_REDUCE_SPLITK && j.kind <= OCRL_REDUCE_COLSUM_FINAL, "reduce table: job %d has unknown kind %d", i, j.kind);
+        OCRL_REQUIRE(j.cols >= 0 && j.parts >= 0, "reduce table: job %d has negative cols / parts", i);
+        const long long wg = job_workgroups(j);
+        if (wg) {
+            OCRL_REQUIRE(j.src && j.dst, "reduce table: job %d has a null pointer", i);
+            if (j.kind == OCRL_REDUCE_SPLITK)
+                OCRL_REQUIRE(j.cols % 4 == 0 && j.part_stride % 4 == 0 && ((((uintptr_t)j.src) | ((uintptr_t)j.dst)) & 15) == 0 && j.scale == 1.f,
+                             "reduce table: split-k job %d needs cols, part_stride %% 4 == 0, 16-byte aligned buffers and scale 1", i);
+            if (j.kind == OCRL_REDUCE_COLSUM || j.kind == OCRL_REDUCE_COLSUM4)
+                OCRL_REQUIRE(j.rows >= 1 && j.part_stride >= 1 && (long long)j.parts * j.part_stride >= j.rows && j.ld >= j.cols && !j.accumulate && j.scale == 1.f,
+                             "reduce table: column-sum job %d: the chunks must cover the rows (no accumulate, scale 1, ld >= cols)", i);
+            if (j.kind == OCRL_REDUCE_COLSUM4)
+                OCRL_REQUIRE(j.cols % 4 == 0 && j.ld % 4 == 0 && j.cols >= 4 && j.cols <= 1024 && ((((uintptr_t)j.src) | ((uintptr_t)j.dst)) & 15) == 0,
+                             "reduce table: float4 column-sum job %d needs cols, ld %% 4 == 0, 4 <= cols <= 1024 and 16-byte aligned buffers", i);
+        }
+        prefix[i] = (int)total;
+        if (wg) {
+            int e = -1;
+            for (int k = i - 1; k >= 0 && e < 0; --k) if (head[k] >= 0 && jobs[k].dst == j.dst) e = k;
+            if (e >= 0) {
+                OCRL_REQUIRE(e == i - 1 && jobs[e].kind == j.kind && jobs[e].cols == j.cols && (j.kind == OCRL_REDUCE_SPLITK || j.kind == OCRL_REDUCE_COLSUM_FINAL),
+                             "reduce table: jobs %d and %d share a destination but are not adjacent jobs of one split-k / final kind and width", e, i);
+                head[i] = head[e];
+                jobs[head[e]].chain += 1;
+            } else {
+                head[i] = i;
+                total += wg;
+            }
+        }
+        OCRL_REQUIRE(total < (1ll << 31), "reduce table: too many workgroups");
+    }
+    prefix[njobs] = (int)total;
+    return 0;
+}
+
+int reduce_table_launch(const ReduceJob* jobs_dev, const int* prefix_dev, int njobs, int workgroups, hipStream_t st) {
+    if (njobs <= 0 || workgroups <= 0) return 0;
+    hipLaunchKernelGGL(reduce_table_kernel, dim3((unsigned)workgroups), dim3(256), 0, st, jobs_dev, prefix_dev, njobs);
+    OCRL_CHECK_LAUNCH("reduce_table");
+    return 0;
+}
diff --git a/ocrl_amd/csrc/slate_model.cpp b/ocrl_amd/csrc/slate_model.cpp
--- a/ocrl_amd/csrc/slate_model.cpp
+++ b/ocrl_amd/csrc/slate_model.cpp
@@ -227,6 +227,20 @@
         q.gbr[1] = carve(nullptr, BT * d); q.gbr[2] = carve(nullptr, BT * d);
     }
     scratch3_ = carve(nullptr, scratch_floats_);
+    {
+        size_t need = 0, n1 = 0;
+        const long long shapes[7][3] = {{(long long)BT, V, d}, {(long long)BT, d, 4 * d}, {(long long)BT, 4 * d, d}, {(long long)BT, d, d}, {(long long)BT, 3 * d, d},
+                                        {(long long)BK, d, d}, {(long long)BK, d, d}};
+        for (const auto& sh : shapes)
+            if (lin_bwd_w_sk_floats(sh[0], (int)sh[1], (int)sh[2], scratch_floats_, 0, &n1) == 0) need += n1;
+        need += 2 * (size_t)(d * d > 65536 ? d * d : 65536);
+        rd_arena_floats_ = need;
+        rd_arena_ = carve(nullptr, rd_arena_floats_);
+        rd_ln_slot_ = (size_t)(2048 + 256) * 2 * d;
+        rd_ln_ = carve(nullptr, rd_ln_slot_ * (3 * NB + 1));
+        rd_dev_ = reinterpret_cast<ReduceJob*>(carve(nullptr, (size_t)RD_MAX_JOBS * sizeof(ReduceJob) / 4));
+        rd_prefix_dev_ = reinterpret_cast<int*>(carve(nullptr, RD_MAX_JOBS + RD_MAX_LAUNCHES));
+    }
     gmem_ = carve(nullptr, BK * d); gck_ = carve(nullptr, BK * d); gcv_ = carve(nullptr, BK * d);
     gdA_ = carve(nullptr, BN * 64); gdB_ = carve(nullptr, BN * 64);
     }
@@ -263,6 +277,13 @@
                 if (dw_mode_ == 2) OCRL_HIP(hipStreamCreateWithFlags(&side2_, hipStreamNonBlocking));
             }
         }
+    }
+    {
+        const char* e = getenv("OCRL_REDUCE_DEFER");
+        rd_on_ = e ? atoi(e) != 0 : true;
+        rd_host_.assign(RD_MAX_JOBS, ReduceJob());
+        rd_prefix_host_.assign(RD_MAX_JOBS + RD_MAX_LAUNCHES, -1);
+        rd_stage1_.clear(); rd_final_.clear();
     }
     {
         const char* e = getenv("OCRL_XATTN");
@@ -671,6 +692,45 @@
     return 0;
 }
 
+int SlateModel::lin_bwd_w_deferred(const float* dy, int ld_dy, const float* x, int ldx, float* dW, float* db, long long M, int N_out, int K_in, hipStream_t st,
+                                   Xf xf) {
+    size_t need = 0;
+    RC(lin_bwd_w_sk_floats(M, N_out, K_in, scratch_floats_, 0, &need));
+    if (!need) return lin_bwd_w(dy, ld_dy, x, ldx, dW, db, M, N_out, K_in, 1.f, st, xf);
+    OCRL_REQUIRE(rd_used_ + need <= rd_arena_floats_, "deferred reductions: slab arena too small (%zu + %zu > %zu)", rd_used_, need, rd_arena_floats_);
+    ReduceJob j[2];
+    RC(::lin_bwd_w(dy, ld_dy, x, ldx, dW, db, M, N_out, K_in, 1.f, rd_arena_ + rd_used_, need, st, Drop(), xf, 0, 0, j));
+    OCRL_REQUIRE(j[0].parts > 1, "deferred reductions: the product did not split as planned");
+    rd_used_ += need;
+    rd_stage1_.push_back(j[0]);
+    if (j[1].parts) rd_stage1_.push_back(j[1]);
+    return 0;
+}
+
+int SlateModel::rd_flush(hipStream_t s) {
+    for (std::vector<ReduceJob>* list : {&rd_stage1_, &rd_final_}) {
+        const int n = (int)list->size();
+        if (!n) continue;
+        OCRL_REQUIRE(rd_cursor_ + n <= RD_MAX_JOBS && rd_pcursor_ + n + 1 <= RD_MAX_JOBS + RD_MAX_LAUNCHES, "deferred reductions: job table overflow");
+        std::vector<int> prefix(n + 1);
+        RC(reduce_table_prepare(list->data(), n, prefix.data()));
+        ReduceJob* hj = rd_host_.data() + rd_cursor_;
+        int* hp = rd_prefix_host_.data() + rd_pcursor_;
+        if (memcmp(hj, list->data(), (size_t)n * sizeof(ReduceJob)) != 0 || memcmp(hp, prefix.data(), (size_t)(n + 1) * sizeof(int)) != 0) {
+            OCRL_HIP(hipStreamSynchronize(s));
+            memcpy(hj, list->data(), (size_t)n * sizeof(ReduceJob));
+            memcpy(hp, prefix.data(), (size_t)(n + 1) * sizeof(int));
+            OCRL_HIP(hipMemcpyAsync(rd_dev_ + rd_cursor_, hj, (size_t)n * sizeof(ReduceJob), hipMemcpyHostToDevice, s));
+            OCRL_HIP(hipMemcpyAsync(rd_prefix_dev_ + rd_pcursor_, hp, (size_t)(n + 1) * sizeof(int), hipMemcpyHostToDevice, s));
+        }
+        RC(reduce_table_launch(rd_dev_ + rd_cursor_, rd_prefix_dev_ + rd_pcursor_, n, prefix[n], s));
+        rd_cursor_ += n; rd_pcursor_ += n + 1;
+        list->clear();
+    }
+    rd_used_ = 0;
+    return 0;
+}
+
 int SlateModel::bwd_decoder(hipStream_t st) {
     const int B = last_.B;
     const long long BT = (long long)B * T, BK = (long long)B * K;
@@ -689,9 +749,35 @@
     auto dw = [&](const float* dy, int ld_dy, const float* x, int ldx, float* dW, float* db, long long M, int N_out, int K_in, Xf xf = Xf()) -> int {
         float* keep = scratch_;
         if (dws) scratch_ = sw_scratch;
-        const int rc = lin_bwd_w(dy, ld_dy, x, ldx, dW, db, M, N_out, K_in, 1.f, sw, xf);
+        const int rc = rd_on_ ? lin_bwd_w_deferred(dy, ld_dy, x, ldx, dW, db, M, N_out, K_in, sw, xf) : lin_bwd_w(dy, ld_dy, x, ldx, dW, db, M, N_out, K_in, 1.f, sw, xf);
         scratch_ = keep;
         return rc;
+    };
+    rd_cursor_ = rd_pcursor_ = 0; rd_used_ = 0; rd_ln_next_ = 0;
+    rd_stage1_.clear(); rd_final_.clear();
+    auto ln_bwd = [&](const float* dy, const float* x, const float* mean, const float* rstd, const float* g, float* dx, float* dgb, int acc_dx) -> int {
+        if (!rd_on_) return layernorm_bwd_launch(dy, x, mean, rstd, g, dx, dgb, BT, d, acc_dx, 0, scratch_, scratch_floats_, st);
+        OCRL_REQUIRE(rd_ln_next_ < 3 * NB + 1, "deferred reductions: out of LayerNorm slots");
+        float* ws = rd_ln_ + rd_ln_slot_ * rd_ln_next_++;
+        int nblk = 0;
+        RC(layernorm_bwd_partials_launch(dy, x, mean, rstd, g, dx, BT, d, acc_dx, ws, scratch_floats_, &nblk, st));
+        const size_t need = (size_t)nblk * 2 * d;
+        ReduceJob j[2];
+        size_t used = 0;
+        RC(colsum_jobs(ws, 2 * d, dgb, nblk, 2 * d, 0, 1.f, ws + need, scratch_floats_ - need, j, &used));
+        OCRL_REQUIRE(need + used <= rd_ln_slot_, "deferred reductions: LayerNorm slot too small");
+        rd_stage1_.push_back(j[0]); rd_final_.push_back(j[1]);
+        return 0;
+    };
+    auto colsum_sw = [&](const float* X, long long ld, float* out, long long R, int F) -> int {
+        if (!rd_on_) return colsum_launch(X, ld, out, R, F, 0, 1.f, scratch_, scratch_floats_, sw);
+        ReduceJob j[2];
+        size_t used = 0;
+        OCRL_REQUIRE(rd_used_ <= rd_arena_floats_, "deferred reductions: slab arena overrun");
+        RC(colsum_jobs(X, ld, out, R, F, 0, 1.f, rd_arena_ + rd_used_, rd_arena_floats_ - rd_used_ < scratch_floats_ ? rd_arena_floats_ - rd_used_ : scratch_floats_, j, &used));
+        rd_used_ += (used + 3) & ~(size_t)3;
+        rd_stage1_.push_back(j[0]); rd_final_.push_back(j[1]);
+        return 0;
     };
     auto on_sw = [&](const std::function<int()>& body) -> int {
         float* keep = scratch_;
@@ -705,8 +791,7 @@
     RC(dw(pred_, V, lnf_, d, G("_out.weight"), nullptr, BT, V, d, ce));
     RC(lin_bwd_x(pred_, V, P("_out.weight"), gt1_, d, BT, V, d, nullptr, 0, nullptr, 0, st, Drop(), ce));
     const float* xlast = blk_[NB - 1].x3;
-    RC(layernorm_bwd_launch(gt1_, xlast, lnf_mean_, lnf_rstd_, P("_tfdec.layer_norm.weight"), gx_, G("_tfdec.layer_norm.weight"), BT, d, 0, 0,
-                            scratch_, scratch_floats_, st));
+    RC(ln_bwd(gt1_, xlast, lnf_mean_, lnf_rstd_, P("_tfdec.layer_norm.weight"), gx_, G("_tfdec.layer_norm.weight"), 0));
     RC(fill_launch(gmem_, BK * d, 0.f, st));
     for (int b = NB - 1; b >= 0; --b) {
         Blk& k = blk_[b];
@@ -726,8 +811,7 @@
         RC(dw(gd, d, k.f1, 4 * d, G(pre + "ffn.2.weight"), G(pre + "ffn.2.bias"), BT, d, 4 * d));
         RC(dw(q.gf1, 4 * d, k.ln3, d, G(pre + "ffn.0.weight"), G(pre + "ffn.0.bias"), BT, 4 * d, d));
         RC(lin_bwd_x(q.gf1, 4 * d, P(pre + "ffn.0.weight"), gt1_, d, BT, 4 * d, d, nullptr, 0, nullptr, 0, st));
-        RC(layernorm_bwd_launch(gt1_, k.x2, k.ln3_mean, k.ln3_rstd, P(pre + "ffn_layer_norm.weight"), gx_, G(pre + "ffn_layer_norm.weight"), BT, d, 1, 0,
-                                scratch_, scratch_floats_, st));
+        RC(ln_bwd(gt1_, k.x2, k.ln3_mean, k.ln3_rstd, P(pre + "ffn_layer_norm.weight"), gx_, G(pre + "ffn_layer_norm.weight"), 1));
         RC(drop_gx(site + 3, q.gbr[1]));
         const float* gd_co = gd;
         if (xattn_) {
@@ -772,8 +856,8 @@
                 go.B = k.cv; go.sB = (long long)K * d; go.sBi = dh;
                 go.C = xa_po_; go.sC = (long long)d * d; go.sCi = dh;
                 RC(gemm_launch(go, sw));
-                RC(colsum_launch(xa_pq_, (long long)d * d, G(pre + "encoder_decoder_attn.proj_q.weight"), B, d * d, 0, 1.f, scratch_, scratch_floats_, sw));
-                RC(colsum_launch(xa_po_, (long long)d * d, G(pre + "encoder_decoder_attn.proj_o.weight"), B, d * d, 0, 1.f, scratch_, scratch_floats_, sw));
+                RC(colsum_sw(xa_pq_, (long long)d * d, G(pre + "encoder_decoder_attn.proj_q.weight"), B, d * d));
+                RC(colsum_sw(xa_po_, (long long)d * d, G(pre + "encoder_decoder_attn.proj_o.weight"), B, d * d));
                 return 0;
             }));
         } else {
@@ -787,16 +871,21 @@
         {
             hipStream_t sx = xattn_ ? sw : st;
             auto body = [&]() -> int {
-                RC(lin_bwd_w(gck_, d, mem_, d, G(pre + "encoder_decoder_attn.proj_k.weight"), nullptr, BK, d, d, 1.f, sx));
-                RC(lin_bwd_w(gcv_, d, mem_, d, G(pre + "encoder_decoder_attn.proj_v.weight"), nullptr, BK, d, d, 1.f, sx));
+                if (rd_on_ && sx == sw) {
+                    RC(lin_bwd_w_deferred(gck_, d, mem_, d, G(pre + "encoder_decoder_attn.proj_k.weight"), nullptr, BK, d, d, sx, Xf()));
+                    RC(lin_bwd_w_deferred(gcv_, d, mem_, d, G(pre + "encoder_decoder_attn.proj_v.weight"), nullptr, BK, d, d, sx, Xf()));
+                } else {
+                    RC(lin_bwd_w(gck_, d, mem_, d, G(pre + "encoder_decoder_attn.proj_k.weight"), nullptr, BK, d, d, 1.f, sx));
+                    RC(lin_bwd_w(gcv_, d, mem_, d, G(pre + "encoder_decoder_attn.proj_v.weight"), nullptr, BK, d, d, 1.f, sx));
+                }
                 RC(lin_bwd_x(gck_, d, P(pre + "encoder_decoder_attn.proj_k.weight"), gmem_, d, BK, d, d, nullptr, 0, gmem_, d, sx));
                 RC(lin_bwd_x(gcv_, d, P(pre + "encoder_decoder_attn.proj_v.weight"), gmem_, d, BK, d, d, nullptr, 0, gmem_, d, sx));
                 return 0;
             };
             if (xattn_) RC(on_sw(body)); else RC(body());
         }
-        RC(layernorm_bwd_launch(gt1_, k.x1, k.ln2_mean, k.ln2_rstd, P(pre + "encoder_decoder_attn_layer_norm.weight"), gx_,
-                                G(pre + "encoder_decoder_attn_layer_norm.weight"), BT, d, 1, 0, scratch_, scratch_floats_, st));
+        RC(ln_bwd(gt1_, k.x1, k.ln2_mean, k.ln2_rstd, P(pre + "encoder_decoder_attn_layer_norm.weight"), gx_,
+                  G(pre + "encoder_decoder_attn_layer_norm.weight"), 1));
         RC(drop_gx(site + 1, q.gbr[2]));
         const float* gd_o = gd;
         RC(lin_bwd_x(gd, d, P(pre + "self_attn.proj_o.weight"), gt1_, d, BT, d, d, nullptr, 0, nullptr, 0, st));
@@ -813,12 +902,11 @@
         RC(lin_bwd_x(q.gqkv, 3 * d, P(pre + "self_attn.proj_q.weight"), gt1_, d, BT, 3 * d, d, nullptr, 0, nullptr, 0, st));
         if (b == 0) {
             RC(axpy_launch(gx_, gt1_, BT * d, 1.f, st));
-            RC(layernorm_bwd_launch(gt1_, xin, k.ln1_mean, k.ln1_rstd, P(pre + "self_attn_layer_norm.weight"), gx_,
-                                    G(pre + "self_attn_layer_norm.weight"), BT, d, 0, 0, scratch_, scratch_floats_, st));
+            RC(ln_bwd(gt1_, xin, k.ln1_mean, k.ln1_rstd, P(pre + "self_attn_layer_norm.weight"), gx_, G(pre + "self_attn_layer_norm.weight"), 0));
         } else {
-            RC(layernorm_bwd_launch(gt1_, xin, k.ln1_mean, k.ln1_rstd, P(pre + "self_attn_layer_norm.weight"), gx_,
-                                    G(pre + "self_attn_layer_norm.weight"), BT, d, 1, 0, scratch_, scratch_floats_, st));
-        }
+            RC(ln_bwd(gt1_, xin, k.ln1_mean, k.ln1_rstd, P(pre + "self_attn_layer_norm.weight"), gx_, G(pre + "self_attn_layer_norm.weight"), 1));
+        }
+        if (rd_on_ && b > 0) { RC(dw_sync()); RC(rd_flush(sw)); }
     }
     RC(embed_bwd_launch(gx_, tokens_, G("_dict.dictionary.weight"), B, T, V, d, p, last_.seed, scratch_, scratch_floats_, st));
     RC(fill_launch(G("_z_pos.pe"), (long long)(T + 1) * d, 0.f, st));
@@ -829,6 +917,7 @@
         OCRL_HIP(hipEventRecord(ev, sw));
         OCRL_HIP(hipStreamWaitEvent(st, ev, 0));
     }
+    if (rd_on_) { RC(dw_sync()); RC(rd_flush(sw)); }
     RC(lin_bwd_w(gmem_, d, slots_, D, G("_slotproj.weight"), nullptr, BK, d, D, 1.f, st));
     RC(lin_bwd_x(gmem_, d, P("_slotproj.weight"), gslots_, D, BK, d, D, nullptr, 0, nullptr, 0, st));
     return 0;
diff --git a/ocrl_amd/csrc/slate_model.h b/ocrl_amd/csrc/slate_model.h
--- a/ocrl_amd/csrc/slate_model.h
+++ b/ocrl_amd/csrc/slate_model.h
@@ -58,6 +58,7 @@
                   float alpha, hipStream_t st, Xf xf = Xf()) {
         return ::lin_bwd_w(dy, ld_dy, x, ldx, dW, db, M, N_out, K_in, alpha, scratch_, scratch_floats_, st, Drop(), xf);
     }
+    int lin_bwd_w_deferred(const float* dy, int ld_dy, const float* x, int ldx, float* dW, float* db, long long M, int N_out, int K_in, hipStream_t st, Xf xf);
     bool fused_heads() const { return !cfg.hard; }
     int conv_layer_fwd(const float* x, const float* pack, const float* bias, float* y, int Bn, int Hh, int Ww, int KS, int CIN, int relu,
                        const float* posmap, const float* mask, hipStream_t st);
@@ -138,6 +139,20 @@
     hipEvent_t ev_dw_[8] = {nullptr, nullptr, nullptr, nullptr, nullptr, nullptr, nullptr, nullptr};
     hipEvent_t ev_join2_ = nullptr;
     int ev_dw_next_ = 0;
+    enum { RD_MAX_JOBS = 1024, RD_MAX_LAUNCHES = 64 };
+    bool rd_on_ = true;
+    float* rd_arena_ = nullptr;
+    size_t rd_arena_floats_ = 0, rd_used_ = 0;
+    float* rd_ln_ = nullptr;
+    size_t rd_ln_slot_ = 0;
+    int rd_ln_next_ = 0;
+    ReduceJob* rd_dev_ = nullptr;
+    int* rd_prefix_dev_ = nullptr;
+    std::vector<ReduceJob> rd_host_;
+    std::vector<int> rd_prefix_host_;
+    int rd_cursor_ = 0, rd_pcursor_ = 0;
+    std::vector<ReduceJob> rd_stage1_, rd_final_;
+    int rd_flush(hipStream_t s);
     float *attn_delta_;
     float *lnf_, *lnf_mean_, *lnf_rstd_, *pred_;
     float *gqkv_;
```

Result: no change. 1703, median of 2 (-0.0%).
